# l-tamas/Fiasco

Hardware: AMD Instinct MI355X
Metric: grayscale frames/sec encoded (higher is better)
Workload: dtype f32

## Files before the change

fiasco_amd/__init__.py:

```python
import ctypes
import os
import subprocess

_HERE = os.path.dirname(os.path.abspath(__file__))
LIB_PATH = os.path.join(_HERE, "libfiasco_amd.so")
CSRC = os.path.join(_HERE, "csrc")

FIASCO_NO_VERBOSITY, FIASCO_SOME_VERBOSITY, FIASCO_ULTIMATE_VERBOSITY = 0, 1, 2
FIASCO_TILING_SPIRAL_ASC, FIASCO_TILING_SPIRAL_DSC = 0, 1
FIASCO_TILING_VARIANCE_ASC, FIASCO_TILING_VARIANCE_DSC = 2, 3
FIASCO_RPF_RANGE_0_75, FIASCO_RPF_RANGE_1_00, FIASCO_RPF_RANGE_1_50, FIASCO_RPF_RANGE_2_00 = 0, 1, 2, 3
FIASCO_PROGRESS_NONE, FIASCO_PROGRESS_BAR, FIASCO_PROGRESS_PERCENT = 0, 1, 2

EXPORTED_SYMBOLS = [
    "fiasco_get_error_message", "fiasco_set_verbosity", "fiasco_get_verbosity", "fiasco_coder",
    "fiasco_c_options_new", "fiasco_c_options_delete", "fiasco_c_options_set_smoothing",
    "fiasco_c_options_set_frame_pattern", "fiasco_c_options_set_tiling",
    "fiasco_c_options_set_basisfile", "fiasco_c_options_set_chroma_quality",
    "fiasco_c_options_set_optimizations", "fiasco_c_options_set_prediction",
    "fiasco_c_options_set_video_param", "fiasco_c_options_set_quantization",
    "fiasco_c_options_set_progress_meter", "fiasco_c_options_set_comment",
    "fiasco_c_options_set_title", "fiasco_calloc", "open_file", "fiasco_amd_set_limits",
    "fiasco_amd_get_limits", "fiasco_amd_encode_batch", "fiasco_amd_free",
    "fiasco_amd_get_stats", "fiasco_amd_reset_stats", "fiasco_amd_spec_workgroups", "fiasco_amd_core_name", "fiasco_amd_rccl_gather", "fiasco_amd_set_device",
    "fiasco_amd_batch_stage", "fiasco_amd_batch_encode", "fiasco_amd_batch_free",
    "fiasco_amd_batch_submit", "fiasco_amd_batch_collect", "fiasco_amd_batch_stats", "fiasco_amd_batch_decode_psnr", "fiasco_amd_batch_decode_psnr_all", "fiasco_amd_coop_workgroups", "fiasco_amd_share_of", "fiasco_amd_spec_append_helpers", "fiasco_amd_batch_decode_plane", "fiasco_amd_c_options_set_models",
    "fiasco_amd_release_memory", "fiasco_amd_batch_upload", "fiasco_amd_set_devices", "fiasco_amd_device_count",
    "fiasco_amd_selftest_log2", "fiasco_amd_selftest_log2_patched",
    "fiasco_amd_selftest_log2_max_ulp",
    "fiasco_amd_seq_open", "fiasco_amd_seq_free", "fiasco_amd_seq_gops", "fiasco_amd_seq_frames",
    "fiasco_amd_seq_gop_of", "fiasco_amd_seq_ycol_size", "fiasco_amd_seq_initial_level",
    "fiasco_amd_seq_search", "fiasco_amd_seq_gop_result", "fiasco_amd_seq_ycol", "fiasco_amd_seq_write",
    "fiasco_amd_seq_probe",
    "fiasco_amd_batch_stage_device", "fiasco_amd_batch_upload_device", "fiasco_amd_batch_input_planes",
    "fiasco_amd_batch_decode_device", "fiasco_amd_planes_to_pixels_device",
]

FIASCO_AMD_GRAY8, FIASCO_AMD_RGB8_INTERLEAVED, FIASCO_AMD_RGB8_PLANAR = 0, 1, 2


class DeviceFrame(ctypes.Structure):
    _fields_ = [("data", ctypes.c_void_p), ("pitch", ctypes.c_size_t), ("plane_stride", ctypes.c_size_t),
                ("width", ctypes.c_uint), ("height", ctypes.c_uint), ("layout", ctypes.c_int)]


class DeviceTarget(ctypes.Structure):
    _fields_ = [("data", ctypes.c_void_p), ("pitch", ctypes.c_size_t), ("plane_stride", ctypes.c_size_t),
                ("width", ctypes.c_uint), ("height", ctypes.c_uint), ("layout", ctypes.c_int)]


class Stats(ctypes.Structure):
    _fields_ = [("kernel_ms", ctypes.c_double), ("launches", ctypes.c_ulonglong),
                ("frames", ctypes.c_ulonglong), ("bytes_mp", ctypes.c_ulonglong),
                ("bytes_img", ctypes.c_ulonglong), ("bytes_gram", ctypes.c_ulonglong),
                ("n_mp", ctypes.c_ulonglong), ("n_steps", ctypes.c_ulonglong),
                ("n_blocks", ctypes.c_ulonglong), ("n_appends", ctypes.c_ulonglong),
                ("n_fulleval", ctypes.c_ulonglong), ("t_init", ctypes.c_ulonglong),
                ("t_approx", ctypes.c_ulonglong), ("t_ipis", ctypes.c_ulonglong),
                ("t_append", ctypes.c_ulonglong), ("t_serial", ctypes.c_ulonglong),
                ("t_total", ctypes.c_ulonglong), ("t_mpA", ctypes.c_ulonglong),
                ("t_mpB", ctypes.c_ulonglong), ("n_blockevals", ctypes.c_ulonglong),
                ("dbg", ctypes.c_ulonglong * 8), ("states_sum", ctypes.c_ulonglong),
                ("states_max", ctypes.c_ulonglong), ("reencodes", ctypes.c_ulonglong),
                ("frames_by_build", ctypes.c_ulonglong * 5),
                ("spec_frames", ctypes.c_ulonglong), ("spec_tasks", ctypes.c_ulonglong),
                ("spec_confirmed", ctypes.c_ulonglong), ("spec_wrong", ctypes.c_ulonglong),
                ("spec_timeout", ctypes.c_ulonglong), ("spec_inline", ctypes.c_ulonglong),
                ("spec_wait", ctypes.c_ulonglong), ("spec_tab_used", ctypes.c_ulonglong),
                ("spec_tab_missed", ctypes.c_ulonglong), ("spec_adopted", ctypes.c_ulonglong),
                ("decoder_frames", ctypes.c_ulonglong), ("decoder_bytes", ctypes.c_ulonglong),
                ("decoder_us", ctypes.c_ulonglong), ("coop_frames", ctypes.c_ulonglong),
                ("coop_workgroups", ctypes.c_ulonglong),
                ("spec_app_rows", ctypes.c_ulonglong), ("spec_app_wait", ctypes.c_ulonglong)]


def build(verbose=False):
    out = None if verbose else subprocess.DEVNULL
    subprocess.check_call(["make", "-C", CSRC], stdout=out)
    if not os.path.exists(LIB_PATH):
        raise RuntimeError("build did not produce %s" % LIB_PATH)


class FiascoError(RuntimeError):
    pass


class Library:

    def __init__(self, path=LIB_PATH):
        if not os.path.exists(path):
            raise FiascoError("%s is missing: run fiasco_amd.build() (there is no fallback)" % path)
        self.path = path
        L = self.L = ctypes.CDLL(path)
        c = ctypes
        L.fiasco_get_error_message.restype = c.c_char_p
        L.fiasco_set_verbosity.argtypes = [c.c_int]
        L.fiasco_get_verbosity.restype = c.c_int
        L.fiasco_c_options_new.restype = c.c_void_p
        L.fiasco_c_options_delete.argtypes = [c.c_void_p]
        L.fiasco_coder.argtypes = [c.POINTER(c.c_char_p), c.c_char_p, c.c_float, c.c_void_p]
        L.fiasco_coder.restype = c.c_int
        L.fiasco_amd_c_options_set_models.argtypes = [c.c_void_p, c.c_char_p, c.c_char_p, c.c_char_p, c.c_char_p]
        L.fiasco_amd_c_options_set_models.restype = c.c_int
        for name, args in [
            ("set_smoothing", [c.c_int]), ("set_frame_pattern", [c.c_char_p]),
            ("set_tiling", [c.c_int, c.c_uint]), ("set_basisfile", [c.c_char_p]),
            ("set_chroma_quality", [c.c_float, c.c_uint]),
            ("set_optimizations", [c.c_uint] * 5), ("set_prediction", [c.c_int, c.c_uint, c.c_uint]),
            ("set_video_param", [c.c_uint, c.c_int, c.c_int, c.c_int]),
            ("set_quantization", [c.c_uint, c.c_int, c.c_uint, c.c_int]),
            ("set_progress_meter", [c.c_int]), ("set_comment", [c.c_char_p]),
            ("set_title", [c.c_char_p]),
        ]:
            fn = getattr(L, "fiasco_c_options_" + name)
            fn.argtypes = [c.c_void_p] + args
            fn.restype = c.c_int
        L.fiasco_amd_set_limits.argtypes = [c.c_uint, c.c_uint]
        L.fiasco_amd_set_limits.restype = c.c_int
        L.fiasco_amd_get_limits.argtypes = [c.POINTER(c.c_uint), c.POINTER(c.c_uint)]
        L.fiasco_amd_encode_batch.argtypes = [c.c_uint, c.POINTER(c.c_char_p), c.POINTER(c.c_size_t),
                                              c.c_float, c.c_void_p, c.POINTER(c.c_void_p),
                                              c.POINTER(c.c_size_t)]
        L.fiasco_amd_encode_batch.restype = c.c_int
        L.fiasco_amd_free.argtypes = [c.c_void_p]
        L.fiasco_amd_core_name.restype = c.c_char_p
        if hasattr(L, "fiasco_amd_get_stats"):
            L.fiasco_amd_get_stats.argtypes = [c.POINTER(Stats)]

    def error_message(self):
        return self.L.fiasco_get_error_message().decode("latin-1")

    def core_name(self):
        return self.L.fiasco_amd_core_name().decode()

    def set_verbosity(self, level):
        self.L.fiasco_set_verbosity(level)

    def set_limits(self, max_states, max_level):
        if not self.L.fiasco_amd_set_limits(max_states, max_level):
            raise FiascoError(self.error_message())

    def get_limits(self):
        a, b = ctypes.c_uint(), ctypes.c_uint()
        self.L.fiasco_amd_get_limits(ctypes.byref(a), ctypes.byref(b))
        return a.value, b.value

    def set_devices(self, ids):
        arr = (ctypes.c_int * max(len(ids), 1))(*ids)
        self.L.fiasco_amd_set_devices.argtypes = [ctypes.POINTER(ctypes.c_int), ctypes.c_int]
        if not self.L.fiasco_amd_set_devices(arr, len(ids)):
            raise FiascoError(self.error_message())

    def device_count(self):
        return self.L.fiasco_amd_device_count()

    def set_device(self, device):
# ... 450 lines not shown
```

fiasco_amd/csrc/hip/core_hip.cpp:

```cpp
#include <hip/hip_runtime.h>
#include <stdio.h>
#include <stdlib.h>
#include <string.h>
#include <stddef.h>
#include <pthread.h>
#include <algorithm>
#include <utility>
#include <vector>
#include "fa_host.h"
#include "frame_coder.h"
#include "libfiasco_amd_hip.h"

extern "C" const char *fa_knob(const char *name)
{
    const char *d = getenv("FIASCO_AMD_DEBUG");
    return d && *d && strcmp(d, "0") != 0 ? getenv(name) : nullptr;
}
static long long knob_int(const char *name, long long d)
{
    const char *e = fa_knob(name);
    return e ? atoll(e) : d;
}


// ... 1338 lines not shown
    }
    const char *const host = pinned;
    const int16_t *tree = (const int16_t *) host;
    const int16_t *into = (const int16_t *) (host + (L.into - L.tree));
    const float *weight = (const float *) (host + (L.weight - L.tree));
    const float *fin = (const float *) (host + (L.final_d - L.tree));
    const uint8_t *los = (const uint8_t *) (host + (L.level_of_state - L.tree));
    const uint8_t *dt = (const uint8_t *) (host + (L.domain_type - L.tree));
    const uint16_t *xs = (const uint16_t *) (host + (L.x - L.tree));
    const uint16_t *ys = (const uint16_t *) (host + (L.y - L.tree));
    const uint8_t *ycol = (const uint8_t *) (host + (L.ycol - L.tree));
    const int16_t *mv = (const int16_t *) (host + (L.mv - L.tree));
    const bool inter = job->frame_type != FA_I_FRAME;
    for (unsigned s = 0; s < w->basis_states; s++) w->level_of_state[s] = 0xff;
    fa_wfa_remove_states(w, w->basis_states);
    for (unsigned s = w->basis_states; s < ns; s++) {
        w->final_distribution[s] = fin[s];
        w->domain_type[s] = dt[s];
        w->level_of_state[s] = los[s];
        w->delta_state[s] = 0;
        for (int l = 0; l < 2; l++) {
            FA_TREE(w, s, l) = tree[(size_t) l * P + s];
            w->x[s * 2 + l] = xs[(size_t) l * P + s];
            w->y[s * 2 + l] = ys[(size_t) l * P + s];
            w->y_state[s * 2 + l] = FA_RANGE;
            w->y_column[s * 2 + l] = F.color ? ycol[(size_t) l * P + s] : 0;
            w->prediction[s * 2 + l] = 0;
            if (inter) {
                fa_mv *m = &w->mv[s * 2 + l];
                m->type = mv[(size_t) (0 * 2 + l) * P + s]; m->fx = mv[(size_t) (1 * 2 + l) * P + s];
                m->fy = mv[(size_t) (2 * 2 + l) * P + s]; m->bx = mv[(size_t) (3 * 2 + l) * P + s];
                m->by = mv[(size_t) (4 * 2 + l) * P + s];
            }
            for (int e = 0; e < 6; e++) {
                FA_INTO(w, s, l, e) = into[(size_t) (l * 6 + e) * P + s];
                FA_WEIGHT(w, s, l, e) = weight[(size_t) (l * 6 + e) * P + s];
                if (FA_INTO(w, s, l, e) == FA_NO_EDGE) break;
            }
        }
    }
    if (F.color)
        for (unsigned s = 0; s < w->cap && s < (unsigned) P; s++)
            for (int l = 0; l < 2; l++) w->y_column[s * 2 + l] = ycol[(size_t) l * P + s];
    w->states = ns;
    w->root_state = (unsigned) F.root_state;
    job->stats[0].costs = F.costs; job->stats[0].err = F.err;
    job->stats[0].tree_bits = F.tree_bits; job->stats[0].matrix_bits = F.matrix_bits;
    job->stats[0].weights_bits = F.weights_bits;
    if (F.color) {
        for (int b = 0; b < 2; b++) {
            job->stats[b + 1].costs = F.c_costs[b]; job->stats[b + 1].err = F.c_err[b];
            job->stats[b + 1].tree_bits = F.c_tree_bits[b];
            job->stats[b + 1].matrix_bits = F.c_matrix_bits[b];
            job->stats[b + 1].weights_bits = F.c_weights_bits[b];
        }
        int ycb = FA_TREE(w, ns - 1, 0), crs = FA_TREE(w, ns - 1, 1);
        int roots[2] = { FA_TREE(w, ycb, 1), FA_TREE(w, crs, 0) };
        int yroot = FA_TREE(w, ycb, 0);
        std::vector<std::pair<int, int>> stack;
        for (int b = 0; b < 2; b++) {
            stack.push_back(std::make_pair(roots[b], yroot));
            while (!stack.empty()) {
                std::pair<int, int> t = stack.back();
                stack.pop_back();
                int s = t.first, y = t.second;
                if (s == FA_RANGE || (unsigned) s < w->basis_states) continue;
                for (int l = 0; l < 2; l++) {
                    int ny = y != FA_RANGE ? FA_TREE(w, y, l) : FA_RANGE;
                    w->y_state[s * 2 + l] = (int16_t) ny;
                    stack.push_back(std::make_pair((int) FA_TREE(w, s, l), ny));
                }
            }
        }
    }
    job->lc_min_level_out = (unsigned) F.lc_min_out;
    job->status = 1;
    g_stats.frames += 1;
    g_stats.bytes_mp += F.bytes_mp; g_stats.bytes_img += F.bytes_img; g_stats.bytes_gram += F.bytes_gram;
    g_stats.n_mp += F.n_mp; g_stats.n_steps += F.n_steps; g_stats.n_blocks += F.n_blocks;
    g_stats.n_appends += F.n_appends; g_stats.n_fulleval += F.n_fulleval;
    g_stats.t_init += F.t_init; g_stats.t_approx += F.t_approx; g_stats.t_ipis += F.t_ipis;
    g_stats.t_append += F.t_append; g_stats.t_serial += F.t_serial; g_stats.t_total += F.t_total;
    g_stats.t_mpA += F.t_mpA; g_stats.t_mpB += F.t_mpB; g_stats.n_blockevals += F.n_blockevals;
    for (int k = 0; k < 8; k++) g_stats.dbg[k] += F.dbg[k];
    g_stats.states_sum += ns;
    if (ns > g_stats.states_max) g_stats.states_max = ns;
    cap_hint_put(job, F.ystates_out, F.states);
    if (fa_knob("FIASCO_AMD_CAP_TRACE"))
        fprintf(stderr, "capacity: frame type %d used %d table states of %d, %d states of %d; %.3f s on the device\n", job->frame_type,
                F.ystates_out, fs.P, F.states, fs.PA, (double) F.t_total / 1e8);
    return 1;
}

static bool queue_resources(Staged *S, size_t frames)
{
    if (!grow_buffer(S->d_ring, S->ring_n, 5 * frames)) return false;
    if (!S->d_queue && hipMalloc((void **) &S->d_queue, 2 * 5 * sizeof(unsigned)) != hipSuccess) {
        S->d_queue = nullptr; (void) hipGetLastError(); return false;
    }
    if (!S->ptrmask_ready) {
        const size_t words = FC_DESC_WORDS, mwords = (words + 31) / 32;
        std::vector<unsigned> mask(mwords, 0u);
        FrameSlot a = S->slots[S->lender0], b = S->slots[S->lender0];
        const fa_job *job = &S->jobs[a.job];
        b.base = a.base + (1u << 24);
        fill_frame(a, job); fill_frame(b, job);
        const unsigned long long *wa = (const unsigned long long *) &a.F, *wb = (const unsigned long long *) &b.F;
        for (size_t w = 0; w < sizeof(DevFrame) / 8; w++)
            if (wa[w] != wb[w]) mask[w >> 5] |= 1u << (w & 31);
        const size_t wp = offsetof(DevFrame, pack_src) / 8;
        mask[wp >> 5] |= 1u << (wp & 31);
        if (!S->d_ptrmask && hipMalloc((void **) &S->d_ptrmask, mwords * sizeof(unsigned)) != hipSuccess) {
            S->d_ptrmask = nullptr; (void) hipGetLastError(); return false;
        }
        if (hipMemcpy(S->d_ptrmask, mask.data(), mwords * sizeof(unsigned), hipMemcpyHostToDevice) != hipSuccess) return false;
        S->ptrmask_ready = true;
    }
    return true;
}

struct WaveGroups { size_t n[N_BUILDS], lend[N_BUILDS], borrow[N_BUILDS]; };

static bool order_batch(Staged *S, WaveGroups &g)
{
    std::vector<size_t> &batch = S->batch;
    batch.clear();
    for (size_t k = 0; k < S->slots.size(); k++)
        if (S->slots[k].staged && !S->slots[k].done) batch.push_back(k);
    if (batch.empty()) return false;
    memset(&g, 0, sizeof g);
    const bool few = batch.size() <= (size_t) S->ncu && !fa_knob("FIASCO_AMD_NO_WIDE");
    std::vector<int> key(S->slots.size());
    for (size_t k : batch) {
        const FrameSlot &fs = S->slots[k];
        const Build b = build_of(S, fs, few);
        const int part = fs.borrow ? 1 : S->borrowers && queue_eligible(S, fs) && queue_layout(S, fs) ? 0 : 2;
        key[k] = 3 * b + part;
        g.n[b]++;
        if (part == 0) g.lend[b]++; else if (part == 1) g.borrow[b]++;
        if (k_build[b].stats_slot >= 0) g_stats.frames_by_build[k_build[b].stats_slot]++; else g_stats.spec_frames++;
    }
    std::stable_sort(batch.begin(), batch.end(), [&](size_t a, size_t b) { return key[a] < key[b]; });
    return true;
}

static void place_packs(Staged *S)
{
    const std::vector<size_t> &batch = S->batch;
    std::vector<DevFrame> &hf = S->hf;
    hf.resize(batch.size());
    S->pack_off.assign(batch.size(), 0);
    size_t need = 0;
    for (size_t b = 0; b < batch.size(); b++) {
        const FrameSlot &fs = S->slots[batch[b]];
        hf[b] = fs.F;
        hf[b].pack_src = fs.F.slab_base + fs.L.tree;
        hf[b].pack_bytes = (unsigned) (fs.L.pool_states - fs.L.tree);
        S->pack_off[b] = need;
        need += align_up(fs.L.pool_states - fs.L.tree, 256);
    }
    S->pack_need = need;
    S->parity ^= 1;
    char *&pack = S->d_pack[S->parity];
    (void) grow_buffer(pack, S->d_pack_bytes[S->parity], need);
    if (!S->cstream && hipStreamCreateWithFlags(&S->cstream, hipStreamNonBlocking) != hipSuccess) {
        S->cstream = nullptr; (void) hipGetLastError();
// ... 254 lines not shown
    if (S->packed) {
        need = S->pack_need;
        for (size_t b = 0; b < batch.size(); b++) if (hf[b].status == FC_OK) off[b] = S->pack_off[b];
    } else
        for (size_t b = 0; b < batch.size(); b++)
            if (hf[b].status == FC_OK) {
                const Layout &L = S->slots[batch[b]].L;
                off[b] = need;
                need += align_up(L.pool_states - L.tree, 256);
            }
    if (S->copy_pending) { (void) hipStreamSynchronize(S->cstream); S->copy_pending = false; }
    (void) grow_buffer(S->pinned, S->pinned_bytes, need, true);
    if (S->pinned && S->packed) {
        if (hipMemcpyAsync(S->pinned, S->d_pack[S->parity], need, hipMemcpyDeviceToHost, S->cstream) == hipSuccess)
            S->copy_pending = true;
        else {
            (void) hipGetLastError();
            off.assign(batch.size(), (size_t) -1);
        }
    } else if (S->pinned) {
        for (size_t b = 0; b < batch.size(); b++)
            if (off[b] != (size_t) -1) {
                const FrameSlot &fs = S->slots[batch[b]];
                if (hipMemcpyAsync(S->pinned + off[b], fs.base + fs.L.tree, fs.L.pool_states - fs.L.tree,
                                   hipMemcpyDeviceToHost, S->stream) != hipSuccess)
                    off[b] = (size_t) -1;
            }
        (void) hipStreamSynchronize(S->stream);
    }
    return off;
}

static void frame_outcome(Staged *S, size_t b, size_t off)
{
    FrameSlot &fs = S->slots[S->batch[b]];
    fa_job *job = &S->jobs[fs.job];
    const int st = S->hf[b].status;
    void *tr_keep = fs.F.trace;
    fs.F = S->hf[b];
    fs.F.trace = (FcTrace *) tr_keep; fs.F.trace_cap = 0;
    if (fs.ext_pix) fs.F.pix16 = fs.ext_pix;
    const size_t cap = align_up(job->cp.limit_states, 64);
    if (st == FC_ERR_CAPACITY && ((size_t) fs.P < cap || (size_t) fs.PA < cap || fs.spec)) {
        g_stats.reencodes += 1;
        size_t np = align_up((size_t) fs.P + (size_t) fs.P / 2, 64);
        size_t npa = align_up((size_t) fs.PA + (size_t) fs.PA / 2, 64);
        if ((size_t) fs.P >= cap || np >= cap) fs.spec = false;
        if (np > 3072 && S->specG > 1 && (size_t) S->specG * S->n > (size_t) S->ncu) fs.spec = false;
        if (fs.base) slab_release(fs.base, fs.bytes);
        if (fs.borrow) { fs.borrow = false; S->borrowers--; }
        fs.base = nullptr; fs.staged = false;
        fs.P = (int) (np > cap ? cap : np);
        fs.PA = (int) (npa > cap ? cap : npa);
        if (fs.PA < fs.P) fs.PA = fs.P;
        if (fs.P > 12 * 1024) fs.spec = false;
        if (!stage_slot(S, fs)) fs.done = true;
        return;
    }
    if (st == FC_ERR_COOP && fs.spec && !S->no_app) {
        S->no_app = true;
        return;
    }
    if (st == FC_ERR_COOP && !S->no_coop_done) {
        S->no_coop = true;
        return;
    }
    if (st == FC_ERR_QUEUE && fs.borrow) {
        fs.borrow = false; S->borrowers--;
        fs.base = nullptr; fs.staged = false;
        if (!stage_slot(S, fs)) fs.done = true;
        return;
    }
    fs.done = true;
    if (st == FC_OK) {
        if (S->pinned && off != (size_t) -1) S->to_unpack.push_back(std::make_pair(S->batch[b], off));
        else S->good += collect(S, fs, nullptr);
        return;
    }
    const char *msg = "device coder failed";
    if (st == FC_ERR_STATES || st == FC_ERR_CAPACITY) msg = "Maximum number of states reached!";
    else if (st == FC_ERR_NOROOT) msg = "No root state generated!";
    else if (st == FC_ERR_QUEUE) msg = "device coder: frame queue gave no slab";
    else if (st == FC_ERR_COOP) msg = "device coder: the helper workgroups of the frame did not answer";
    else if (st == FC_ERR_INTERNAL) msg = "device coder: frame exceeds a built-in capacity (recursion depth, snapshot stack or 16384 states)";
    if (st > FC_ERR_QUEUE) snprintf(job->errmsg, sizeof job->errmsg, "%s (status %d)", msg, st);
    else snprintf(job->errmsg, sizeof job->errmsg, "%s", msg);
}

static void complete_wave(Staged *S)
{
    if (!download_wave(S)) {
        const char *why = hipGetErrorString(hipGetLastError());
        for (size_t b = 0; b < S->batch.size(); b++) {
            FrameSlot &fs = S->slots[S->batch[b]];
            snprintf(S->jobs[fs.job].errmsg, sizeof S->jobs[fs.job].errmsg, "HIP error: %s", why);
            fs.done = true;
        }
        S->broken = true;
        return;
    }
    const std::vector<size_t> off = fetch_automata(S);
    for (size_t b = 0; b < S->batch.size(); b++) frame_outcome(S, b, off[b]);
    (void) hipStreamSynchronize(S->stream);
}

static void flush_unpack(Staged *S)
{
    if (S->copy_pending) { (void) hipStreamSynchronize(S->cstream); S->copy_pending = false; }
    for (size_t i = 0; i < S->to_unpack.size(); i++)
        S->good += collect(S, S->slots[S->to_unpack[i].first], S->pinned + S->to_unpack[i].second);
    S->to_unpack.clear();
}

static int core1_submit(void *h)
{
    Staged *S = (Staged *) h;
    if (!S || !S->ok) return 0;
    if (S->inflight) return 1;
    for (size_t k = 0; k < S->slots.size(); k++) {
        S->slots[k].done = false;
        S->slots[k].src = S->jobs[S->slots[k].job].image;
    }
    S->good = 0; S->broken = false;
    if (S->up_pending) {
        (void) hipStreamWaitEvent(S->stream, S->ev_up, 0);
        for (size_t k = 0; k < S->slots.size(); k++) {
            FrameSlot &fs = S->slots[k];
            if (fs.ext_next) { fs.ext_pix = fs.ext_next; fs.F.pix16 = fs.ext_pix; }
        }
        S->up_parity ^= 1;
        S->up_pending = false;
    }
    S->inflight = launch_wave(S);
    return 1;
}

static int core1_finish2(void *h, int resubmit)
{
    Staged *S = (Staged *) h;
    if (!S || !S->ok) return 0;
    if (!S->inflight) { core1_submit(h); }
    for (size_t k = 0; k < S->slots.size(); k++) S->jobs[S->slots[k].job].status = 0;
    for (;;) {
        if (S->inflight) { complete_wave(S); S->inflight = false; if (S->broken) break; }
        {
            bool more = false;
            for (size_t k = 0; k < S->slots.size(); k++) if (!S->slots[k].done) more = true;
            if (more) flush_unpack(S);
        }
        if (launch_wave(S)) { S->inflight = true; continue; }
        bool any = false, pending = false;
        for (size_t k = 0; k < S->slots.size(); k++) {
            FrameSlot &fs = S->slots[k];
            if (!fs.staged && !fs.done && !S->jobs[fs.job].errmsg[0]) pending = true;
        }
        if (!pending) break;
        for (size_t k = 0; k < S->slots.size(); k++) {
            FrameSlot &fs = S->slots[k];
            if (fs.done && fs.base) { slab_release(fs.base, fs.bytes); fs.base = nullptr; fs.staged = false; }
        }
        for (size_t k = 0; k < S->slots.size(); k++) {
            FrameSlot &fs = S->slots[k];
            if (fs.staged || fs.done || S->jobs[fs.job].errmsg[0]) continue;
            if (stage_slot(S, fs)) any = true; else if (!fs.rejected) break;
        }
        if (!any) break;
// ... 511 lines not shown
```

fiasco_amd/csrc/hip/fc_config.inc:

```

#ifndef FC_VARIANT_WIDE
#define FC_VARIANT_WIDE 0
#endif
#if FC_VARIANT_WIDE
#ifndef FC_WIDE_B
#define FC_WIDE_B 512
#endif
#define B       FC_WIDE_B
#if defined(FC_VARIANT_BIG) && FC_VARIANT_BIG
#define FC_KREG 12
#elif !defined(FC_KREG)
#define FC_KREG (9216 / FC_WIDE_B)
#endif
#else
#define B       FC_BLOCK
#define FC_KREG 12
#endif
#ifndef FC_VARIANT_BIG
#define FC_VARIANT_BIG 0
#endif
#if FC_HM && !(FC_VARIANT_BIG && FC_VARIANT_WIDE)
#error "FC_HM is a variant of the 512-thread big build"
#endif
#if FC_GM && !FC_HM
#error "FC_GM is a variant of the FC_HM build"
#endif
#if FC_VARIANT_BIG
#if FC_GM
#define FC_KERNEL    fiasco_frame_kernel_big_gm
#define FC_LAUNCH    fc_launch_big_gm
#define FC_OCCUPANCY fc_occupancy_big_gm
#elif FC_HM
#define FC_KERNEL    fiasco_frame_kernel_big_hm
#define FC_LAUNCH    fc_launch_big_hm
#define FC_OCCUPANCY fc_occupancy_big_hm
#elif FC_VARIANT_WIDE
#define FC_KERNEL    fiasco_frame_kernel_big_wide
#define FC_LAUNCH    fc_launch_big_wide
#define FC_OCCUPANCY fc_occupancy_big_wide
#else
#define FC_KERNEL    fiasco_frame_kernel_big
#define FC_LAUNCH    fc_launch_big
#define FC_OCCUPANCY fc_occupancy_big
#endif
#define FC_PIXELS    4096
#define FC_NIP       4
#define FC_CLMAX     2048
#define FC_WG_PER_CU (FC_VARIANT_WIDE ? 1 : 2)
#else
#if FC_VARIANT_WIDE
#if defined(FC_SPEC) && FC_SPEC
#define FC_KERNEL    fiasco_frame_kernel_spec_wide
#define FC_LAUNCH    fc_launch_spec_wide
#define FC_OCCUPANCY fc_occupancy_spec_wide
#define FC_SPEC_SLOT_BYTES fc_spec_slot_bytes_wide
#elif defined(FC_GRAM_TRI) && FC_GRAM_TRI
#define FC_KERNEL    fiasco_frame_kernel_wide_tri
#define FC_LAUNCH    fc_launch_wide_tri
#define FC_OCCUPANCY fc_occupancy_wide_tri
#else
#define FC_KERNEL    fiasco_frame_kernel_wide
#define FC_LAUNCH    fc_launch_wide
#define FC_OCCUPANCY fc_occupancy_wide
#endif
#elif defined(FC_SPEC) && FC_SPEC
#define FC_KERNEL    fiasco_frame_kernel_spec
#define FC_LAUNCH    fc_launch_spec
#define FC_OCCUPANCY fc_occupancy_spec
#define FC_SPEC_SLOT_BYTES fc_spec_slot_bytes
#else
#define FC_KERNEL    fiasco_frame_kernel
#define FC_LAUNCH    fc_launch
#define FC_OCCUPANCY fc_occupancy
#endif
#define FC_PIXELS    1024
#define FC_NIP       2
#define FC_CLMAX     768
#ifndef FC_WG_PER_CU
#define FC_WG_PER_CU (FC_VARIANT_WIDE ? 1 : 4)
#endif
#endif
#ifndef FC_SPEC
#define FC_SPEC 0
#endif
#define SPEC_THR 1.2f
#define FC_D5T (!FC_VARIANT_BIG)
#if FC_D5T
#define D5_AT(P, NA, a, s) ((unsigned) (s) * (unsigned) (NA) + (unsigned) ((a) & 1) * ((unsigned) (NA) >> 1) + ((unsigned) (a) >> 1))
#else
#define D5_AT(P, NA, a, s) ((unsigned) (a) * (unsigned) (P) + (unsigned) (s))
#endif
#define FC_PRIO_ROTATE (!FC_VARIANT_BIG && !FC_VARIANT_WIDE && !FC_SPEC)
#define FC_PRIO_SHIFT 20
#define MAXED   FC_MAXED
#define FC_MAXE (FC_NIP + 1)
#define NOEDGE  (-1)
#define RANGE_  (-1)
#define MAXCOSTS 1e20f
#define BIGF    3.0e38f
#define MIN_NORM 2e-3f

enum { OP_DONE = 0, OP_INIT_RANGE, OP_APPROX, OP_IPIS_INCR, OP_APPEND, OP_NOP, OP_CHROMA,
       OP_PRED_SETUP, OP_PRED_FINISH, OP_NORMS, OP_MC_SEARCH, OP_SPEC_CKPT };
enum { PH_ENTER = 0, PH_AFTER_INIT, PH_AFTER_LC, PH_CHILD, PH_CHILD2, PH_CHILD_RET, PH_DECIDE,
       PH_AFTER_APPEND, PH_PRED_BEGIN, PH_PRED_RECURSE, PH_PRED_RET, PH_PRED_DONE, PH_PRED_MC2, PH_PRED_GO,
       PH_SPEC_END };
enum { MV_NONE = 0, MV_FORWARD = 1, MV_BACKWARD = 2, MV_INTERPOLATED = 3 };
#ifdef FC_DUP_OP
#define FC_DUP(o, call) do { if ((o) == FC_DUP_OP) { __syncthreads(); call; } } while (0)
#else
#define FC_DUP(o, call) do { } while (0)
#endif
#if FC_VARIANT_BIG
#define FC_DEPTH FC_MAXDEPTH_BIG
#elif FC_VARIANT_WIDE
#define FC_DEPTH FC_MAXDEPTH
#else
#define FC_DEPTH FC_MAXDEPTH_NARROW
#endif
```

fiasco_amd/csrc/hip/fc_lds.inc:

```

#define RANGE_E (FC_MAXE + 1)
struct __attribute__((aligned(16))) Range {
    int   x, y, image, address, level, tree;
    float weight[RANGE_E];
    short into[RANGE_E];
    float err, tree_bits, matrix_bits, weights_bits;
#if FC_VARIANT_BIG
    float nd_tree_bits, nd_weights_bits, mv_tree_bits, mv_coord_bits;
    int   prediction;
    short mv[5];
#endif
};

struct Pool {
    short count[MAXED + 1];
    unsigned short total, n, max_domains, y_index;
    short d0_index;
    unsigned short d0_yindex, d0_n;
};

struct __attribute__((aligned(16))) SFrame {
    Range rg, lrange, rrange, child[2];
    Pool  pool0, pool_lc;
    float max_costs, lincomb, subdiv, ret, price;
// ... 19 lines not shown
    short indices[MAXED + 1], into[MAXED + 1];
    float weight[MAXED];
    unsigned symp;
    float matrix_bits, weights_bits, err, costs, min_costs;
    float sel_ipdo[MAXED][MAXED];
    float norm_ov[MAXED + 1], ipio[MAXED + 1];
    short psorted[MAXED + 1];
    int   np;
    float wb_dc, wb_nd, norm, ab, price;
    int   y_state, ypos;
#if FC_VARIANT_BIG
    const float *numrow;
    short excl[MAXED + 1];
#endif
#if FC_GM
    short kq[MAXED + 1];
#endif
    float s1_pre[MAXED], s1_sfx[MAXED], s1_z0, s1_zy;
    int   s1_last[MAXED], s1_k[MAXED], s1_thr[MAXED];
    unsigned s1_cd, s1_has;
};

struct __attribute__((aligned(16))) CoeffBuf {
    short tot[16];
    short cnt[FC_VARIANT_BIG ? FC_MAXCOEFF_BIG : FC_MAXCOEFF];
};
#if FC_VARIANT_BIG
#define SNAP_POOL16 880
#define SNAP_TM_WORDS 2392
#else
#define SNAP_POOL16 (FC_VARIANT_WIDE ? FC_SNAP16_WIDE : FC_SNAP16_NARROW)
#define SNAP_TM_WORDS (FC_VARIANT_WIDE ? FC_SNAPTM_WIDE : FC_SNAPTM_NARROW)
#endif
#if FC_VARIANT_BIG || FC_VARIANT_WIDE
#define NBLOCKMIN   256
#else
#define NBLOCKMIN   64
#endif
#define TM_WORDS    (4 * 26 + 8)

struct RoundBox {
    float m2[2];
    int   state;
    int   idx;
    float cost, mbits, wbits, err, f[MAXED];
    float num, den, ip[MAXED - 1];
    unsigned evals, blockevals;
    unsigned symp;
};
#define SYMP_NONE 0u
#define SYMP_HAS(p, k) ((k) < 3 && (((p) >> (10 * (k))) & 1023u) != 0u)
#define SYMP_GET(p, k) ((int) (((p) >> (10 * (k))) & 1023u) - 2)
#define SYMP_PUT(sym, k) ((unsigned) ((sym) + 2) << (10 * (k)))

struct Sh {
    RoundBox rb;
    SFrame   st[FC_DEPTH];
    int      sp;
    int      op, a0, a1, a2, a3;
#if FC_VARIANT_BIG
    unsigned coopW, coop_seq;
    int      coopD, coop_minsub;
    unsigned long long coop_ticks;
#endif
    Pool     pool;
    CoeffBuf cb;
#if FC_VARIANT_BIG
    Pool     dpool;
    CoeffBuf dcb;
    struct { int rpf_mant, dc_mant, sy, dcs; float rpf_range, dc_range; int half_nd, half_dc; } dq;
    int      nslot;
    uint4   *snap_tm_p;
    int      pred_active, pred_lo, pred_rec;
    struct { int type, fx, fy, bx, by; float bits, tree_bits; } mc;
    unsigned long long mcred[B / 64];
    unsigned pred_saved[FC_MAXSAVE / 32];
#endif
    uint4    snap_pool[SNAP_POOL16];
    uint4   *snap;
    int      n16;
    __attribute__((aligned(16))) unsigned tm[TM_WORDS];
    __attribute__((aligned(16))) unsigned snap_tm[SNAP_TM_WORDS];
    float    m0tab[12];
    double   lgdc[FC_MAXSYM], lglv[FC_MAXSYM], lglv_m1;
    float    Ltab[MAXED + 1];
    float    Q0, Q1;
    float    tb[2];
    MPState  mp;
#if FC_VARIANT_BIG
    MPState  mp_keep;
    int      apx_stage, apx_it, apx_more;
#endif
    float    blockmin[NBLOCKMIN];
    __attribute__((aligned(16))) float pixels[FC_PIXELS];
    float    norms[FC_PIXELS / 32];
    unsigned long long tk[16];
    struct {
        unsigned long long bytes_mp, bytes_img, bytes_gram, n_mp, n_steps, n_blocks, n_appends,
                           n_fulleval, n_blockevals, t_mpA, t_mpB;
    } cnt;
#ifdef FC_SERIAL_PROFILE
    unsigned long long tk_ph[8], ph_t0, tk_init[2], tk_apx[4];
    int      ph_prev;
#endif
    int      band, lc_min, tree_band[3], ystates, after_chroma;
    short    dl[64];
#if !FC_SPEC
    short    cl[FC_CLMAX];
    int      cln;
#endif
    unsigned long long red[B / 64];
    int      gs_idx[2][MAXED + 1], gs_n[2], gs_c[2], gs_raw_idx[2][MAXED + 1];
    float    gs_raw_w[2][MAXED + 1];
    float    gs_w[2][MAXED + 1];
    struct {
        int lc_max, width, height, limit_states, PA, P, ML; float price, chroma_decrease;
        float *gram, *diag, *ipis; int16_t *pos; unsigned gram_ls;
        float *gcol;
        float *d5, *d4;
        const unsigned *l2_keys; const double *l2_vals; unsigned l2_mask;
        int max_elements, rpf_mant, dc_mant, sy, dcs, gl0, images_level, lc_min_opt, trace_on;
        int snap_b1;
        int16_t *at_tree, *at_into, *at_pool; float *at_weight, *at_final; uint8_t *at_los, *at_dtype, *at_ycol;
        uint16_t *at_x, *at_y; int color;
        float rpf_range, dc_range;
        int half_nd, half_dc;
    } par;
#if FC_GM
    struct { int pk[2], ck[2], qa; float base, kept; double lg1; int16_t *gq; int P; } gm;
#endif
    int      states;
    int      flim;
    int      failed;
#if FC_SPEC
    int      gap_lo, gap_hi, gap_shift;
    unsigned deadmask;
    int      cap;
    int      blk;
    int      tab_shared;
    int      tab_from;
    struct SpecLocal {
        FcSpecCtl *ctl;
        char     *slots;
        int       role, on;
        int       mode;
        int       T;
        int       chroma_tabs;
        char     *tabs;
        unsigned  rb_s[32];
        unsigned  blkof[FC_SPEC_W];
        unsigned  sk[FC_SPEC_W];
        unsigned long long n_tab_used, n_tab_missed, n_adopted;
        int       floor;
        unsigned  head, commit;
        unsigned  spec_mask;
        int       nospec;
        unsigned  epoch;
        int       verdict, abort, busy;
        unsigned  ops;
        float     mlc, lin[FC_SPEC_W];
        unsigned  nlc;
        float     learn;
        unsigned long long n_tasks, n_confirmed, n_wrong, n_timeout, n_inline, t_wait;
        unsigned  app_H, app_min, app_seq, app_off;
        unsigned long long n_app_dealt, t_app_wait;
    } sl;
#endif
};
#if FC_GM
#define GM_QAC(k)   ((k) == FC_PK_ADAPTIVE || (k) == FC_PK_BASIS)
#define GM_RLE(k)   ((k) == FC_PK_RLE || (k) == FC_PK_RLE_NO_CHROMA)
#define GQ_CUR(sh, set)          ((sh).gm.gq + (size_t) ((sh).gm.qa ^ (set)) * (sh).gm.P)
#define GQ_SNAP(sh, depth, slot) ((sh).gm.gq + (size_t) (2 + (depth) * 5 + (slot)) * (sh).gm.P)
#endif
#if FC_SPEC
#define DEAD(sh, s) ((unsigned) ((int) (s) - (sh).gap_lo) < (unsigned) ((sh).gap_hi - (sh).gap_lo))
#else
#define DEAD(sh, s) false
#endif
```

fiasco_amd/csrc/hip/fc_serial.inc:

```


__device__ float tree_bits_dev(const Sh &sh, int ML, int child, int level, int which)
{
    const unsigned *counts = sh.tm + which * 2 * ML;
    float prob = counts[level] / (float) counts[ML + level];
    return child ? (float) -log2((double) prob) : (float) -log2((double) (1 - prob));
}

__device__ void tree_update_dev(Sh &sh, int ML, int child, int level, int which)
{
    unsigned *counts = sh.tm + which * 2 * ML;
    if (child) counts[level]++;
    counts[ML + level]++;
}

__device__ __forceinline__ void copy16(uint4 *dst, const uint4 *src, int n)
{
    int i = 0;
    for (; i + 8 <= n; i += 8) {
        uint4 t0 = src[i], t1 = src[i + 1], t2 = src[i + 2], t3 = src[i + 3];
        uint4 t4 = src[i + 4], t5 = src[i + 5], t6 = src[i + 6], t7 = src[i + 7];
        dst[i] = t0; dst[i + 1] = t1; dst[i + 2] = t2; dst[i + 3] = t3;
        dst[i + 4] = t4; dst[i + 5] = t5; dst[i + 6] = t6; dst[i + 7] = t7;
    }
// ... 405 lines not shown
                snap_save(F, sh, sp, 0);
                tm_save(sh, sp, ML);
#if FC_GM
                fr.rn0 = sh.dpool.n;
                gq_save(sh, 0, sp, 0);
#endif
#if FC_VARIANT_BIG
                if (sh.nslot == 5 && !fr.delta) {
                    fr.dpool0 = sh.dpool; snap_save_d(sh, sp, 2);
#if FC_GM
                    gq_save(sh, 1, sp, 2);
#endif
                }
#endif
            }
            fr.states = sh.states;
            for (int l = 0; l < 2; l++)
                fr.ny[l] = (sh.band && fr.y_state != RANGE_) ? (int) TREE(F, fr.y_state, l) : RANGE_;
            phase = PH_AFTER_LC;
            if (rg.level <= sh.par.lc_max) {
                fr.lrange = rg;
                fr.lrange.tree = RANGE_;
#if FC_VARIANT_BIG
                fr.lrange.tree_bits = tree_bits_dev(sh, ML, 0, rg.level, 0);
#endif
                fr.lrange.matrix_bits = 0;
                fr.lrange.weights_bits = 0;
#if FC_VARIANT_BIG
                fr.lrange.nd_tree_bits = 0; fr.lrange.nd_weights_bits = 0; fr.lrange.prediction = 0;
                fr.lrange.mv_tree_bits = fr.try_pred == 2 ? 1.0f : 0.0f;
                fr.lrange.mv_coord_bits = 0;
#endif
                sh.op = OP_APPROX;
                return 0;
            }
            fr.lincomb = MAXCOSTS;
            break;
        }
        case PH_AFTER_LC: {
            Range &rg = fr.rg;
            if (fr.leaf) {
                fr.subdiv = MAXCOSTS;
                phase = PH_DECIDE;
                break;
            }
            if (!fr.coop) {
#if FC_VARIANT_BIG
                fr.pool_lc = sh.pool;
                snap_save(F, sh, sp, 1);
#if FC_GM
                gq_save(sh, 0, sp, 1);
#endif
                sh.pool = fr.pool0;
                snap_load(F, sh, sp, 0);
#if FC_GM
                gq_load(sh, 0, sp, 0);
                if (fr.delta) sh.dpool.n = (unsigned short) fr.rn0;
#endif
#else
                fr.pool_lc = sh.pool;
#endif
            }
#if FC_SPEC
            if (fr.ckpt == 3) {
                fr.subdiv = MAXCOSTS;
                phase = PH_DECIDE;
                break;
            }
#endif
            if (rg.level > sh.lc_min) {
                Range z;
                z.x = z.y = z.image = z.address = z.level = 0; z.tree = 0;
                for (int i = 0; i < RANGE_E; i++) { z.weight[i] = 0; z.into[i] = 0; }
                z.err = z.tree_bits = z.matrix_bits = z.weights_bits = 0;
#if FC_VARIANT_BIG
                z.nd_tree_bits = z.nd_weights_bits = z.mv_tree_bits = z.mv_coord_bits = 0; z.prediction = 0;
                for (int i = 0; i < 5; i++) z.mv[i] = 0;
#endif
                fr.child[0] = z; fr.child[1] = z;
                fr.rrange = rg;
#if FC_VARIANT_BIG
                fr.rrange.tree_bits = tree_bits_dev(sh, ML, 1, rg.level, 0);
#else
                fr.rrange.tree_bits = rg.level <= sh.par.lc_max ? sh.tb[1] : tree_bits_dev(sh, ML, 1, rg.level, 0);
#endif
                fr.rrange.matrix_bits = 0;
                fr.rrange.weights_bits = 0;
                fr.rrange.err = 0;
#if FC_VARIANT_BIG
                fr.rrange.mv_tree_bits = fr.try_pred == 2 ? 1.0f : 0.0f;
                fr.rrange.mv_coord_bits = 0;
                fr.rrange.nd_tree_bits = fr.try_pred == 1 ? tree_bits_dev(sh, ML, 1, rg.level, 1) : 0.0f;
                fr.rrange.nd_weights_bits = 0;
                fr.rrange.prediction = 0;
                fr.subdiv = (fr.rrange.tree_bits + fr.rrange.weights_bits + fr.rrange.matrix_bits
                             + fr.rrange.mv_tree_bits + fr.rrange.mv_coord_bits + fr.rrange.nd_tree_bits
                             + fr.rrange.nd_weights_bits) * fr.price;
#else
                fr.subdiv = (fr.rrange.tree_bits + fr.rrange.weights_bits + fr.rrange.matrix_bits) * fr.price;
#endif
                fr.label = 0;
                phase = PH_CHILD;
            } else {
                fr.subdiv = MAXCOSTS;
                phase = PH_DECIDE;
            }
            break;
        }
        case PH_CHILD: {
            const Range &rr = fr.rrange;
            const int label = fr.label;
            Range &ch = fr.child[label];
            ch.image = rr.image * 2 + label + 1;
            ch.address = rr.address * 2 + label;
            ch.level = rr.level - 1;
            ch.x = (rr.level & 1) ? rr.x : rr.x + label * (int) width_of_level(rr.level - 1);
            ch.y = (rr.level & 1) ? rr.y + label * (int) height_of_level(rr.level - 1) : rr.y;
            phase = PH_CHILD2;
            if (label && rr.level <= sh.par.lc_max && sh.states > fr.states && !sh.band) {
                sh.op = OP_IPIS_INCR; sh.a0 = ch.image; sh.a1 = ch.address; sh.a2 = ch.level;
                sh.a3 = fr.states;
                return 0;
            }
            break;
        }
        case PH_CHILD2: {
            float lim = fr.lincomb > fr.max_costs ? fr.max_costs : fr.lincomb;
            float remaining = lim - fr.subdiv;
            phase = PH_CHILD_RET;
            fr.ret = 0;
            if (remaining > 0) {
                if (sp + 1 >= FC_DEPTH) { sh.failed = FC_ERR_INTERNAL; break; }
                SFrame &cf = sh.st[sp + 1];
                cf.rg = fr.child[fr.label];
                cf.y_state = fr.ny[fr.label];
                cf.max_costs = remaining;
                cf.phase = PH_ENTER;
#if FC_SPEC
                cf.ckpt = 0;
#endif
#if FC_VARIANT_BIG
                cf.pred = fr.pred; cf.delta = fr.delta;
#endif
                fr.phase = phase; sp++; phase = PH_ENTER;
                break;
            }
            fr.ret = -1;
            break;
        }
        case PH_CHILD_RET: {
            const int label = fr.label;
            float lim = fr.lincomb > fr.max_costs ? fr.max_costs : fr.lincomb;
#if FC_VARIANT_BIG
            if (fr.try_pred == 2 && !fr.norm_done) {
                const Range &c0 = fr.child[label];
                sh.op = OP_NORMS; sh.a0 = fr.rg.level; sh.a1 = fr.norm_first;
                sh.a2 = (fr.ret < 0 && c0.level >= F.p_min) ? c0.level : -1;
                sh.a3 = c0.x | (c0.y << 16);
                fr.norm_first = 0; fr.norm_done = 1;
                return 0;
            }
            fr.norm_done = 0;
#endif
            if (fr.ret >= 0) fr.subdiv += fr.ret;
            if (fr.subdiv >= lim) {
                fr.subdiv = MAXCOSTS;
                phase = PH_DECIDE;
// ... 295 lines not shown
```

fiasco_amd/csrc/hip/frame_coder.h:

```cpp
#ifndef FRAME_CODER_H
#define FRAME_CODER_H
#include <stdint.h>

#define FC_MAXED    5
#define FC_BLOCK    256
#define FC_MAXDEPTH 22
#define FC_MAXDEPTH_BIG 32
#define FC_MAXDEPTH_NARROW 18
#define FC_SNAP16_NARROW 480
#define FC_SNAP16_WIDE   840
#define FC_SNAPTM_NARROW 988
#define FC_SNAPTM_WIDE   1092
#define FC_MAXSAVE  512
#define FC_MAXCOEFF 224
#ifndef FC_HM
#define FC_HM 0
#endif
#ifndef FC_GM
#define FC_GM 0
#endif
enum { FC_PK_ADAPTIVE = 0, FC_PK_CONSTANT = 1, FC_PK_BASIS = 2, FC_PK_UNIFORM = 3, FC_PK_RLE = 4, FC_PK_RLE_NO_CHROMA = 5 };
enum { FC_CK_ADAPTIVE = 0, FC_CK_UNIFORM = 1 };
#define FC_GQ_SLOTS (2 + FC_MAXDEPTH_BIG * 5)
#define FC_MAXCOEFF_BIG_STD 640
#define FC_MAXSYM_STD   64
#define FC_MAXCOEFF_HM  5120
#define FC_MAXSYM_HM    512
#define FC_MAXCOEFF_BIG (FC_HM ? FC_MAXCOEFF_HM : FC_MAXCOEFF_BIG_STD)
#define FC_MAXSYM       (FC_HM ? FC_MAXSYM_HM : FC_MAXSYM_STD)
#define FC_N16(coeffs)  ((32 + 2 * (coeffs) + 15) / 16)
#define FC_N16MAX       FC_N16(FC_MAXCOEFF_BIG)
#define FC_MAXBASIS 16
#define FC_BX_BYTES (64 * 1024)
#ifndef FC_TRI_HOT
#define FC_TRI_HOT  8
#endif

enum { FC_OK = 1, FC_ERR_STATES = 2, FC_ERR_CAPACITY = 3, FC_ERR_NOROOT = 4, FC_ERR_INTERNAL = 5,
       FC_ERR_QUEUE = 6,
       FC_ERR_COOP = 7 };
struct FcCoop {
    unsigned seq;
    unsigned done;
    unsigned quit;
    unsigned depth;
    int      level, from, to;
    int      minsub;
    float   *ipis, *d5, *d4;
    unsigned long long done_ticks;
};
#define FC_COOP_HDR 128
#define FC_COOP_WAIT_TICKS 3000000000ull
#define FC_COOP_DONE_TICKS 500000000ull
#define FC_QUEUE_WAIT_TICKS 60000000000ull

struct FcTrace;
typedef struct DevFrame {
    float    price;
    int      lc_min, lc_max, images_level, max_elements;
    int      maxe_live;
    int      gl0;
    int      second_domain_block;
    int      check_underflow, check_overflow, full_search;
    int      level, width, height;
    int      pool_max, limit_states, ML;
    int      rpf_mant, dc_mant;
    float    rpf_range, dc_range;
    int      P;
    unsigned gram_ls;
    int      PA;
    int      color;
    int      chroma_sparse;
    int      chroma_cl_cap;
    int      chroma_max;
    float    chroma_decrease;
    unsigned long long plane;
    int      NL, NS, NA, NI;
    int      coeff_size, coeff_nt, dcs, sy;
    int      basis_states;
    int16_t  b_tree[FC_MAXBASIS][2];
    int16_t  b_into[FC_MAXBASIS][2][6];
    float    b_weight[FC_MAXBASIS][2][6];
    float    b_final[FC_MAXBASIS];
    uint8_t  b_dtype[FC_MAXBASIS];
    const int *bx;
    int      gm_pool[2], gm_coeff[2];
    int16_t *gq;
    const double *lginv;
    const int16_t *pix16;
    float   *gram, *diag, *ipis, *d5, *img, *imgT, *norms;
    float   *gcol;
    float   *d4, *imgT4;
    float   *num, *den, *est, *ipdo;
    uint8_t *used;
    int16_t *tree, *into;
    float   *weight, *final_d;
    uint8_t *level_of_state, *domain_type;
    uint16_t *x, *y;
    uint8_t *ycol;
    const uint8_t *ycol0;
    void    *snap_hbm;
    int      pred_root;
    int      pred_on;
    int      frame_type;
    int      p_min, p_max;
    int      d_rpf_mant, d_dc_mant;
    float    d_rpf_range, d_dc_range;
    int      d_coeff_size, d_dcs, d_sy;
    float   *ipis_alt, *d5_alt, *d4_alt;
    float   *pix_save;
    float   *sv_gram;
    float   *sv_img;
    struct FcSavedRow *sv_auto;
    int      max_save;
    const int16_t *past, *future;
    float   *mc_fwd, *mc_bwd;
    int16_t *mv;
    int16_t *pix_chroma;
    int      search_range;
    int16_t *pool_states;
    int16_t *pos;
    int     *hits;
    const void *pack_src;
    void    *pack_dst;
    unsigned pack_bytes;
    const unsigned *l2_keys;
    const double   *l2_vals;
    unsigned        l2_mask;
    int      status;
    int      states, root_state;
    FcCoop  *coop;
    int      ystates_out;
    float    costs, err, tree_bits, matrix_bits, weights_bits;
    float    c_costs[2], c_err[2], c_tree_bits[2], c_matrix_bits[2], c_weights_bits[2];
    int      lc_min_out;
    unsigned long long bytes_mp, bytes_img, bytes_gram;
    unsigned long long n_mp, n_steps, n_blocks, n_appends, n_fulleval;
    unsigned long long t_init, t_approx, t_ipis, t_append, t_serial, t_total;
    unsigned long long t_mpA, t_mpB, n_blockevals;
    unsigned long long dbg[8];
    struct FcTrace *trace;
    int      trace_cap, trace_n;
    char    *slab_base;
    unsigned long long slab_bytes;
    struct FcSpecCtl *spec;
    int      spec_role, spec_G;
    int      spec_tb;
    int      spec_cap;
    int      spec_T;
} DevFrame;

#define FC_DESC_WORDS ((sizeof(DevFrame) + 7) / 8)

#define FC_SPEC_W      16
#define FC_SPEC_TEMPS  16
#define FC_SPEC_MAXG   8
#define FC_SPEC_R      24
typedef struct FcSpecCtl {
    unsigned next;
    unsigned epoch;
    unsigned done;
    unsigned committed;
    unsigned adopting;
    unsigned busy;
    unsigned slot_bytes;
    unsigned slot_seq[FC_SPEC_W];
    unsigned verdict[FC_SPEC_W];
    unsigned long long n_tasks, n_confirmed, n_wrong, n_timeout, n_inline, t_wait;
    unsigned long long n_tab_used, n_tab_missed;
    unsigned long long n_adopted;
    unsigned s_pub;
    unsigned tab_free;
    unsigned blk_cur;
    unsigned chroma_ready, tab_next, ystates;
    unsigned n_tabs;
    unsigned n_blocks;
    unsigned tab_stride;
    unsigned tab_wait;
    unsigned long long off_blocks, off_tabs;
    unsigned tab_seq[FC_SPEC_R];
    unsigned tab_s[FC_SPEC_R];
    unsigned tab_epoch[FC_SPEC_R];
    unsigned app_H;
    unsigned app_min;
    unsigned app_wait;
    unsigned app_seq;
    unsigned app_done;
    unsigned app_off;
    unsigned app_dbg;
    int      app_s, app_flim;
    int      app_n[2], app_c[2], app_idx[2][FC_MAXED + 1];
    float    app_w[2][FC_MAXED + 1];
    unsigned long long n_app_dealt, t_app_wait;
} FcSpecCtl;

typedef struct FcSavedRow {
    int16_t  tree[2], into[2][6];
    float    weight[2][6];
    float    final_d;
    uint16_t x[2], y[2];
    int16_t  pos;
    int16_t  mv[2][5];
    uint8_t  level, dtype, ycol[2], tables;
} FcSavedRow;

typedef struct FcTrace {
    int   seq, level, image, D, states, nedges;
    float cost, err, mbits, wbits;
    short into[6];
    float w[5];
} FcTrace;

#endif
```

fiasco_amd/csrc/hip/frame_coder.hip:

```cpp
#include <hip/hip_runtime.h>
#include <stdint.h>
#include <math.h>
#include "frame_coder.h"

#include "fc_config.inc"
#include "fc_lds.inc"
#include "fc_access.inc"
#include "fc_tables.inc"
#include "fc_append.inc"
#include "fc_predict.inc"
#include "fc_models.inc"
#include "mp_device.inc"
#include "fc_serial.inc"
#include "fc_spec.inc"

__device__ void basis_init(DevFrame &F, Sh &sh)
{
    const int nb = F.basis_states, il = F.images_level;
    for (int s = 0; s < nb; s++) {
        F.img[(size_t) s * F.NI] = F.final_d[s];
        if (il == 0) F.imgT[s] = F.final_d[s];
    }
    for (int l = 1; l <= il; l++)
        for (int s = 0; s < nb; s++)
            for (int i = 0; i < (1 << l); i++) {
                float v = image_elem(F, s, l, i);
                F.img[(size_t) s * F.NI + (1 << l) - 1 + i] = v;
                if (l == il) F.imgT[(size_t) i * F.P + s] = v;
#if FC_VARIANT_BIG
                if (l == il - 1 && F.gl0 < il) F.imgT4[(size_t) i * F.P + s] = v;
#endif
            }
    for (int q = 0; q < F.NL; q++)
        for (int s1 = 0; s1 < nb; s1++)
            for (int s2 = 0; s2 <= s1; s2++) {
                if (!F.domain_type[s2]) continue;
#if FC_VARIANT_BIG
                if (F.gl0 < il) {
                    gram_store(F, q, s1, s2, q == 0 ? gram_dot4(F, s1, s2) : q == 1 ? gram_dot(F, s1, s2)
                                                                   : gram_entry(F, q, s1, s2));
                    continue;
                }
#endif
                gram_store(F, q, s1, s2, q == 0 ? gram_dot(F, s1, s2) : gram_entry(F, q, s1, s2));
            }
    sh.states = nb;
}

#if FC_VARIANT_BIG
__device__ void basis_init_bx(DevFrame &F, Sh &sh)
{
    const int tid = threadIdx.x, il = F.images_level;
    const BxView V = bx_view(F);
    const int nb = V.nb;
    for (int s = tid; s < nb; s += B) {
        F.img[(size_t) s * F.NI] = F.final_d[s];
        if (il == 0) F.imgT[s] = F.final_d[s];
    }
    __syncthreads();
    for (int l = 1; l <= il; l++) {
        for (int k = tid; k < (nb << l); k += B) {
            const int s = k >> l, i = k & ((1 << l) - 1);
            const float v = image_elem_bx(F, V, s, l, i);
            F.img[(size_t) s * F.NI + (1 << l) - 1 + i] = v;
            if (l == il) F.imgT[(size_t) i * F.P + s] = v;
            if (l == il - 1 && F.gl0 < il) F.imgT4[(size_t) i * F.P + s] = v;
        }
        __syncthreads();
    }
    for (int q = 0; q < F.NL; q++) {
        for (int k = tid; k < nb * nb; k += B) {
            const int s1 = k / nb, s2 = k - s1 * nb;
            if (s2 > s1 || !F.domain_type[s2]) continue;
            float v;
            if (F.gl0 < il) v = q == 0 ? gram_dot4(F, s1, s2) : q == 1 ? gram_dot(F, s1, s2) : gram_entry_bx(F, V, q, s1, s2);
            else v = q == 0 ? gram_dot(F, s1, s2) : gram_entry_bx(F, V, q, s1, s2);
            gram_store(F, q, s1, s2, v);
        }
        __syncthreads();
    }
}
#endif

#if FC_SPEC
#define SPEC_STRIDE ((unsigned) ((sizeof(Sh) + 255) / 256 * 256))
#define SPEC_SLOTS(ctl) ((char *) (ctl) + (sizeof(FcSpecCtl) + 255) / 256 * 256)
#endif

__global__ void __launch_bounds__(B, FC_WG_PER_CU)
#if FC_SPEC
FC_KERNEL(DevFrame *frames, DevFrame *vframes, unsigned G, unsigned n, unsigned H)
#else
FC_KERNEL(DevFrame *frames, unsigned nlend, unsigned long long *ring, unsigned *ctr, const unsigned *ptrmask,
          unsigned long long queue_wait_ticks, unsigned coopW)
#endif
{
#if FC_SPEC
    constexpr unsigned FC_LDS_EXTRA = sizeof(Sh::SpecLocal) + 64;
#else
    constexpr unsigned FC_LDS_EXTRA = 64;
#endif
    static_assert(sizeof(Sh) + FC_LDS_EXTRA <= (160u * 1024u) / FC_WG_PER_CU, "Sh outgrows the LDS share of a workgroup of this build");
    __shared__ Sh sh;
#if FC_SPEC
    __shared__ Sh::SpecLocal sl_keep;
    __shared__ unsigned task_seq, spec_slot, spec_used, spec_vid;
    __shared__ int task_go, spec_act, spec_bad;
    if (threadIdx.x == 0) spec_bad = 0;
    if (blockIdx.x >= n * G) {
        const unsigned k = blockIdx.x - n * G;
        spec_append_helper(frames[k / H], sh, k % H, H);
        return;
    }
    const unsigned role = blockIdx.x % G;
    DevFrame &F = role ? vframes[(blockIdx.x / G) * (G - 1) + role - 1] : frames[blockIdx.x / G];
    unsigned long long *const ring = nullptr;
#elif FC_VARIANT_BIG
    const unsigned cW = coopW > 1 ? coopW : 1;
    unsigned fidx = blockIdx.x, member = 0;
    if (cW > 1) {
        fidx = (blockIdx.x / (8 * cW)) * 8 + blockIdx.x % 8;
        member = (blockIdx.x / 8) % cW;
        if (fidx >= nlend) return;
    }
    DevFrame &F = frames[fidx];
    if (member) { coop_helper(F, sh, member, cW); return; }
    if (threadIdx.x == 0) {
        sh.coopW = F.coop ? cW : 1; sh.coop_seq = 0;
        sh.coopD = cW > 1 && F.coop ? (int) F.coop->depth : 0; sh.coop_minsub = cW > 1 && F.coop ? F.coop->minsub : 0;
        sh.coop_ticks = cW > 1 && F.coop ? F.coop->done_ticks : 0;
    }
#else
    DevFrame &F = frames[blockIdx.x];
#endif
    const int tid = threadIdx.x;

#if !FC_SPEC
    if (ring && blockIdx.x >= nlend) {
        __shared__ unsigned long long got;
        if (tid == 0) {
            const unsigned t = atomicAdd(&ctr[0], 1u);
            unsigned long long b;
            const unsigned long long t_give_up = wall_clock64() + queue_wait_ticks;
            while ((b = __hip_atomic_load(&ring[t], __ATOMIC_ACQUIRE, __HIP_MEMORY_SCOPE_AGENT)) == 0) {
                if (wall_clock64() > t_give_up) break;
                __builtin_amdgcn_s_sleep(32);
            }
            got = b;
        }
        __syncthreads();
        if (got == 0) {
            if (tid == 0) { F.status = FC_ERR_QUEUE; F.states = 0; }
            return;
        }
        {
            unsigned long long *d = (unsigned long long *) &F;
            const unsigned long long lo = (unsigned long long) F.slab_base, span = F.slab_bytes;
            const unsigned long long delta = got - lo;
            unsigned long long v[(FC_DESC_WORDS + B - 1) / B];
#pragma unroll
            for (unsigned k = 0; k < (FC_DESC_WORDS + B - 1) / B; k++) {
                const unsigned w = k * B + tid;
                v[k] = w < FC_DESC_WORDS ? d[w] : 0;
            }
            __syncthreads();
#pragma unroll
            for (unsigned k = 0; k < (FC_DESC_WORDS + B - 1) / B; k++) {
                const unsigned w = k * B + tid;
                if (w < FC_DESC_WORDS && ((ptrmask[w >> 5] >> (w & 31)) & 1u) && v[k] - lo < span) d[w] = v[k] + delta;
            }
        }
        __threadfence();
        __syncthreads();
        __builtin_amdgcn_s_dcache_inv();
    }
#endif

#if FC_SPEC
    if (tid == 0) {
        Sh::SpecLocal &sl = sh.sl;
        sh.gap_lo = sh.gap_hi = 0; sh.gap_shift = 0; sh.deadmask = 0;
        sh.cap = F.spec ? F.spec_cap : F.P;
        sl.ctl = F.spec; sl.slots = F.spec ? SPEC_SLOTS(F.spec) : nullptr;
        sl.role = (int) role; sl.on = F.spec != nullptr && G > 1;
        sl.mode = role == 0 && sl.on ? 1 : 0;
        sl.T = F.spec_T; sl.tabs = F.spec ? (char *) F.spec + F.spec->off_tabs : nullptr;
        sl.chroma_tabs = 0;
        sl.n_tab_used = sl.n_tab_missed = sl.n_adopted = 0;
        sl.app_H = role == 0 && F.spec && G > 1 ? F.spec->app_H : 0u; sl.app_min = F.spec ? F.spec->app_min : 0u;
        sl.app_seq = 0; sl.app_off = 0; sl.n_app_dealt = sl.t_app_wait = 0;
        for (int k = 0; k < 32; k++) sl.rb_s[k] = 0;
        sh.blk = 0; sh.tab_shared = 0; sh.tab_from = 0;
        sl.floor = 0; sl.head = sl.commit = 0; sl.spec_mask = 0; sl.nospec = 0; sl.epoch = 0;
        sl.verdict = 0; sl.abort = 0; sl.ops = 0; sl.mlc = 0.0f; sl.nlc = 0; sl.learn = 0.0f;
        sl.n_tasks = sl.n_confirmed = sl.n_wrong = sl.n_timeout = sl.n_inline = sl.t_wait = 0;
        sl_keep = sl;
    }
    if (role == 0) {
#endif
    if (tid < 10 && tid >= 1)
        sh.m0tab[tid] = (float) -log2((double) (1 - 1 / (float) (1 << tid)));
    if (tid == 0) {
        const int ML = F.ML;
        static const unsigned c0[22] = {20,17,15,10,5,4,3,2,1,1,1,1,1,1,1,1,1,1,1,1,1,1};
        static const unsigned c1[22] = {1,1,1,1,1,1,1,1,1,2,3,5,10,15,20,25,30,35,60,60,60,60};
        sh.failed = 0;
        sh.cnt.bytes_mp = sh.cnt.bytes_img = sh.cnt.bytes_gram = 0;
        sh.cnt.n_mp = sh.cnt.n_steps = sh.cnt.n_blocks = sh.cnt.n_appends = sh.cnt.n_fulleval = 0;
        sh.cnt.t_mpA = sh.cnt.t_mpB = sh.cnt.n_blockevals = 0;
        F.trace_n = 0;
        for (int k = 0; k < 8; k++) F.dbg[k] = 0;
#ifdef FC_LATENCY_PROBE
        {
            volatile float *a = F.est;
            for (int k = 0; k < 64; k++) a[k] = (float) ((k * 7 + 3) & 63);
            __builtin_amdgcn_s_waitcnt(0);
            unsigned long long c0 = __builtin_readcyclecounter();
            int idx = 0;
            for (int k = 0; k < 64; k++) idx = (int) a[idx];
            unsigned long long c1 = __builtin_readcyclecounter();
            F.dbg[5] = (c1 - c0) / 64 + (idx & 0);
            c0 = __builtin_readcyclecounter();
            for (int k = 0; k < 64; k++) { a[64] = (float) k; idx += (int) a[64]; }
            c1 = __builtin_readcyclecounter();
            F.dbg[6] = (c1 - c0) / 64 + (idx & 0);
        }
#endif
#if FC_VARIANT_BIG
        if (F.bx) {
            const BxView V = bx_view(F);
            for (int s = 0; s < V.nb; s++) {
                F.final_d[s] = V.final_d[s];
                F.domain_type[s] = (uint8_t) V.dtype[s];
                F.level_of_state[s] = 0xff;
                for (int l = 0; l < 2; l++) { TREE(F, s, l) = RANGE_; INTO(F, s, l, 0) = NOEDGE; }
            }
        } else
#endif
        for (int s = 0; s < F.basis_states; s++) {
            F.final_d[s] = F.b_final[s];
            F.domain_type[s] = F.b_dtype[s];
            F.level_of_state[s] = 0xff;
            for (int l = 0; l < 2; l++) {
                TREE(F, s, l) = F.b_tree[s][l];
                for (int e = 0; e < 6; e++) {
                    INTO(F, s, l, e) = F.b_into[s][l][e];
                    WEIGHT(F, s, l, e) = F.b_weight[s][l][e];
                    if (F.b_into[s][l][e] == NOEDGE) break;
                }
            }
        }
        for (int w = 0; w < 2; w++)
            for (int l = 0; l < ML; l++) {
                int k = l < 22 ? l : 21;
                sh.tm[w * 2 * ML + l] = c1[k];
                sh.tm[w * 2 * ML + ML + l] = c0[k] + c1[k];
            }
        for (int i = 4 * ML; i < TM_WORDS; i++) sh.tm[i] = 0;
        Pool &m = sh.pool;
        m.total = 0;
        for (int i = 0; i <= MAXED; i++) { m.count[i] = 1; m.total++; }
        m.n = 0; m.max_domains = (unsigned short) F.pool_max; m.y_index = 0;
        m.d0_index = 0; m.d0_yindex = 0; m.d0_n = 0;
#if FC_GM
        sh.gm.pk[0] = F.gm_pool[0]; sh.gm.pk[1] = F.pred_on ? F.gm_pool[1] : FC_PK_CONSTANT;
        sh.gm.ck[0] = F.gm_coeff[0]; sh.gm.ck[1] = F.gm_coeff[1];
        sh.gm.qa = 0; sh.gm.gq = F.gq; sh.gm.P = F.P;
        sh.gm.base = sh.gm.kept = 0.0f; sh.gm.lg1 = 0.0;
        sh.dpool = m;
        for (int set = 0; set < 2; set++) {
            Pool &pm = set ? sh.dpool : sh.pool;
            const int k = sh.gm.pk[set];
            int maxd = F.pool_max ? F.pool_max : 1;
            if (k == FC_PK_BASIS) maxd = F.basis_states;
            if (k == FC_PK_UNIFORM || k == FC_PK_CONSTANT) maxd = 0xffff;
            pm.max_domains = (unsigned short) maxd;
            if (!GM_RLE(k)) { pm.total = 0; for (int i = 0; i <= MAXED; i++) pm.count[i] = 0; }
        }
        for (int s = 0; s < F.basis_states; s++) {
            F.pos[s] = -1;
            if (F.domain_type[s] & 2) gm_offer(F, sh, s);
        }
        if ((F.domain_type[0] & 2) && F.pos[0] < 0) { F.pos[0] = 0; F.pool_states[0] = 0; }
        if (sh.gm.pk[0] == FC_PK_CONSTANT) sh.pool.n = 1;
        if (sh.gm.pk[1] == FC_PK_CONSTANT) sh.dpool.n = 0;
#else
        for (int s = 0; s < F.basis_states; s++) {
            F.pos[s] = -1;
            if ((F.domain_type[s] & 2) && m.n < m.max_domains) {
                F.pos[s] = (short) m.n;
                F.pool_states[m.n++] = (short) s;
                if (s == 0) m.d0_n = 1;
            }
        }
#endif
        sh.n16 = (32 + 2 * F.coeff_size + 15) / 16;
#if FC_VARIANT_BIG
        if (F.pred_on && (32 + 2 * F.d_coeff_size + 15) / 16 > sh.n16) sh.n16 = (32 + 2 * F.d_coeff_size + 15) / 16;
        sh.nslot = F.pred_on ? 5 : 2;
        sh.snap = (F.pred_on || (F.level - F.lc_min + 3) * 2 * sh.n16 > SNAP_POOL16) && F.snap_hbm
                  ? (uint4 *) F.snap_hbm : sh.snap_pool;
        sh.snap_tm_p = F.pred_on && F.snap_hbm ? (uint4 *) F.snap_hbm + FC_DEPTH * 5 * FC_N16MAX : (uint4 *) sh.snap_tm;
        sh.pred_active = 0; sh.pred_lo = sh.pred_rec = 0;
#endif
        {
            const int depth_need = F.level - F.lc_min + 2
#if FC_VARIANT_BIG
                                   + (F.pred_on ? F.p_max - F.lc_min + 2 : 0)
#endif
                                   ;
#if FC_VARIANT_BIG
            const bool snap_lds = sh.snap == &sh.snap_pool[0];
            const bool tm_lds = (const void *) sh.snap_tm_p == (const void *) &sh.snap_tm[0];
#else
            const bool snap_lds = true, tm_lds = true;
#endif
#if FC_VARIANT_BIG
            const int snap_need = (F.level - F.lc_min + 3) * 2 * sh.n16;
#else
            const int snap_need = (F.level - F.lc_min + 3 + F.lc_max - F.lc_min) * sh.n16;
            sh.par.snap_b1 = (F.level - F.lc_min + 3) - (F.level - F.lc_max);
#endif
            if ((snap_lds && snap_need > SNAP_POOL16)
                || (tm_lds && (F.level - F.lc_min + 3) * 4 * TM_N16(ML) > SNAP_TM_WORDS) || F.coeff_nt > 16
                || (F.P + 63) / 64 > NBLOCKMIN
                || depth_need > FC_DEPTH
                || F.max_elements > FC_MAXE
                || (!FC_VARIANT_BIG && F.pred_on))
                sh.failed = FC_ERR_INTERNAL;
        }
        for (int i = 0; i < (FC_VARIANT_BIG ? FC_MAXCOEFF_BIG : FC_MAXCOEFF); i++) sh.cb.cnt[i] = 0;
        for (int i = 0; i < 16; i++) sh.cb.tot[i] = 0;
        for (int i = 0; i < F.coeff_size; i++) sh.cb.cnt[i] = 1;
        sh.cb.tot[0] = (short) F.dcs;
        for (int i = 1; i < F.coeff_nt; i++) sh.cb.tot[i] = (short) F.sy;
#if FC_VARIANT_BIG
        for (int i = 0; i < FC_MAXCOEFF_BIG; i++) sh.dcb.cnt[i] = 0;
        for (int i = 0; i < 16; i++) sh.dcb.tot[i] = 0;
        for (int i = 0; i < F.d_coeff_size; i++) sh.dcb.cnt[i] = 1;
        sh.dcb.tot[0] = (short) F.d_dcs;
        for (int i = 1; i < F.coeff_nt; i++) sh.dcb.tot[i] = (short) F.d_sy;
#if !FC_GM
        sh.dpool = sh.pool;
#endif
        sh.dq.rpf_mant = F.d_rpf_mant; sh.dq.dc_mant = F.d_dc_mant; sh.dq.sy = F.d_sy; sh.dq.dcs = F.d_dcs;
        sh.dq.rpf_range = F.d_rpf_range; sh.dq.dc_range = F.d_dc_range;
        sh.dq.half_nd = rtob_dev(0.5f, F.d_rpf_mant, F.d_rpf_range); sh.dq.half_dc = rtob_dev(0.5f, F.d_dc_mant, F.d_dc_range);
        if (F.pred_on && F.d_coeff_size > FC_MAXCOEFF_BIG) sh.failed = FC_ERR_INTERNAL;
#endif
#if FC_VARIANT_BIG
        if (F.bx) sh.states = F.basis_states;
        else
#else
        if (F.bx) sh.failed = FC_ERR_INTERNAL;
#endif
        basis_init(F, sh);
        sh.flim = 0;
        sh.par.lc_max = F.lc_max; sh.par.width = F.width; sh.par.height = F.height;
        sh.par.limit_states = F.limit_states; sh.par.PA = F.PA; sh.par.P = F.P; sh.par.ML = F.ML;
        sh.par.price = F.price; sh.par.chroma_decrease = F.chroma_decrease;
        sh.par.gram = F.gram; sh.par.gram_ls = F.gram_ls; sh.par.diag = F.diag; sh.par.ipis = F.ipis; sh.par.pos = F.pos;
        sh.par.gcol = F.gcol;
        sh.par.d5 = F.d5; sh.par.d4 = F.d4;
        sh.par.at_tree = F.tree; sh.par.at_into = F.into; sh.par.at_pool = F.pool_states; sh.par.at_weight = F.weight;
        sh.par.at_final = F.final_d; sh.par.at_los = F.level_of_state; sh.par.at_dtype = F.domain_type;
        sh.par.at_ycol = F.ycol; sh.par.at_x = F.x; sh.par.at_y = F.y; sh.par.color = F.color;
        sh.par.l2_keys = F.l2_keys; sh.par.l2_vals = F.l2_vals; sh.par.l2_mask = F.l2_mask;
        sh.par.max_elements = F.max_elements; sh.par.rpf_mant = F.rpf_mant; sh.par.dc_mant = F.dc_mant;
        sh.par.sy = F.sy; sh.par.dcs = F.dcs; sh.par.gl0 = F.gl0; sh.par.images_level = F.images_level;
        sh.par.lc_min_opt = F.lc_min; sh.par.trace_on = F.trace != nullptr;
        sh.par.rpf_range = F.rpf_range; sh.par.dc_range = F.dc_range;
        sh.par.half_nd = rtob_dev(0.5f, F.rpf_mant, F.rpf_range); sh.par.half_dc = rtob_dev(0.5f, F.dc_mant, F.dc_range);
        sh.band = 0; sh.lc_min = F.lc_min; sh.after_chroma = 0; sh.ystates = 0;
        push_root(F, sh, RANGE_);
        sh.op = OP_NOP;
    }
    if (F.color)
        for (int i = tid; i < 2 * F.PA; i += B) F.ycol[i] = F.ycol0 ? F.ycol0[i] : (uint8_t) 0;
#if FC_VARIANT_BIG
    if (F.bx) { __syncthreads(); basis_init_bx(F, sh); }
#endif
#if FC_SPEC
    }
#endif
    unsigned long long *tk = sh.tk;
    if (tid == 0) for (int k = 0; k < 16; k++) tk[k] = 0;
#ifdef FC_SERIAL_PROFILE
    if (tid == 0) { for (int k = 0; k < 8; k++) sh.tk_ph[k] = 0; sh.ph_prev = 0; sh.ph_t0 = 0; sh.tk_init[0] = sh.tk_init[1] = 0; for (int k = 0; k < 4; k++) sh.tk_apx[k] = 0; }
#endif
    unsigned long long t_begin = wall_clock64();
#if FC_SPEC
    const unsigned T = F.spec ? (unsigned) F.spec_T : 0u;
    if (role == 0 && F.spec && G > 1) {
        __threadfence();
        __syncthreads();
        if (tid == 0) __hip_atomic_store(&F.spec->s_pub, (unsigned) sh.states, __ATOMIC_RELEASE, __HIP_MEMORY_SCOPE_AGENT);
    }
    if (role >= 1 && role <= T) { spec_worker(F, sh, role, T, false); return; }
    for (;;) {
    if (role) {
        FcSpecCtl *const c = F.spec;
        __syncthreads();
        if (tid == 0) {
            unsigned t = atomicAdd(&c->next, 1u);
            int go = 1;
            for (;;) {
                const unsigned q = __hip_atomic_load(&c->slot_seq[t % FC_SPEC_W], __ATOMIC_RELAXED, __HIP_MEMORY_SCOPE_AGENT);
                if (q == t + 1) { take_acquire(); break; }
                if (q > t + 1) { t = atomicAdd(&c->next, 1u); continue; }
                if (__hip_atomic_load(&c->done, __ATOMIC_RELAXED, __HIP_MEMORY_SCOPE_AGENT)) { go = 0; break; }
                if (__hip_atomic_load(&c->chroma_ready, __ATOMIC_RELAXED, __HIP_MEMORY_SCOPE_AGENT)) { take_acquire(); go = 2; break; }
                __builtin_amdgcn_s_sleep(32);
            }
            task_seq = t; task_go = go;
        }
        __syncthreads();
        if (task_go != 1) break;
        {
            const uint4 *src = (const uint4 *) (SPEC_SLOTS(c) + (size_t) (task_seq % FC_SPEC_W) * SPEC_STRIDE);
            for (unsigned i = tid; i < sizeof(Sh) / 16; i += B) ((uint4 *) &sh)[i] = src[i];
        }
        __syncthreads();
        if (tid == 0) {
            const unsigned task_epoch = sh.sl.epoch;
            bool valid = __hip_atomic_load(&c->slot_seq[task_seq % FC_SPEC_W], __ATOMIC_ACQUIRE, __HIP_MEMORY_SCOPE_AGENT) == task_seq + 1
                         && __hip_atomic_load(&c->epoch, __ATOMIC_ACQUIRE, __HIP_MEMORY_SCOPE_AGENT) == task_epoch;
            sh.sl = sl_keep;
            sh.sl.epoch = task_epoch;
            const int S0 = sh.states, TB = F.spec_tb;
            if (valid && (S0 > TB || sh.sp < 0 || sh.sp >= FC_DEPTH)) valid = false;
            sh.sl.floor = sh.sp; sh.sl.verdict = 2; sh.sl.abort = valid ? 0 : 1; sh.sl.ops = 0; sh.sl.busy = 0;
            sh.sl.mode = 2 + sh.sp;
            if (sh.sp > 0) sh.st[sh.sp - 1].phase = PH_SPEC_END;
            sh.gap_lo = S0; sh.gap_hi = TB; sh.gap_shift = TB - S0; sh.states = TB; sh.cap = TB + FC_SPEC_TEMPS;
            unsigned dm = 0;
            for (int k = 0; k < 32; k++) if (k * B >= S0 && (k + 1) * B <= TB) dm |= 1u << k;
            sh.deadmask = dm;
            sh.par.at_pool = F.pool_states;
            sh.par.trace_on = 0;
            sh.par.color = 0;
            for (int k = 0; k < FC_SPEC_TEMPS; k++) F.level_of_state[TB + k] = 0;
            sh.op = valid ? OP_NOP : OP_DONE;
            if (valid) {
                atomicAdd(&c->busy, 1u);
                SPEC_DEKKER_FENCE();
                if (__hip_atomic_load(&c->epoch, __ATOMIC_ACQUIRE, __HIP_MEMORY_SCOPE_AGENT) != task_epoch) {
                    atomicSub(&c->busy, 1u); valid = false; sh.sl.abort = 1; sh.op = OP_DONE;
                } else sh.sl.busy = 1;
            }
            if (valid && !sh.tab_shared) {
                const Range &rg = sh.st[sh.sp].rg;
                sh.par.ipis = F.ipis; sh.par.d5 = F.d5;
                sh.op = OP_INIT_RANGE; sh.a0 = rg.x; sh.a1 = rg.y; sh.a2 = -1;
            }
        }
    }
#endif
    for (;;) {
        __syncthreads();
        const int op = sh.op;
        if (op == OP_DONE) break;
        unsigned long long t0 = wall_clock64();
#if FC_PRIO_ROTATE
        {
            const unsigned pr = ((unsigned) (t0 >> FC_PRIO_SHIFT) + (blockIdx.x >> 8)) & 3u;
            if (pr == 0) __builtin_amdgcn_s_setprio(0);
            else if (pr == 1) __builtin_amdgcn_s_setprio(1);
            else if (pr == 2) __builtin_amdgcn_s_setprio(2);
            else __builtin_amdgcn_s_setprio(3);
        }
#endif
        switch (op) {
#if FC_SPEC
        case OP_SPEC_CKPT: {
            FcSpecCtl *const c = sh.sl.ctl;
            if (tid == 0) {
                int act = 0;
                const int back = spec_poll(sh, sh.a0 == 2);
                if (back) {
                    act = (back & 0x100) ? 3 : 2; spec_slot = (unsigned) ((back & 0xff) - 1);
                    spec_used = (unsigned) (back >> 16) & 63u; spec_vid = (unsigned) (back >> 24) & 7u;
                    if (act == 3) {
                        __builtin_amdgcn_fence(__ATOMIC_ACQUIRE, "agent");
                        const Sh *im = (const Sh *) (sh.sl.slots + (size_t) (FC_SPEC_W + spec_vid) * SPEC_STRIDE);
                        const int TB = im->gap_hi, S0 = im->gap_lo, m = im->states - TB;
                        int bad = 0;
                        if (S0 != (int) sh.sl.sk[spec_slot]) bad |= 1;
                        if (TB < F.spec_cap || TB + FC_SPEC_TEMPS > F.P || ((TB - F.spec_cap) % FC_SPEC_TEMPS)) bad |= 2;
                        if (m < 0 || m > FC_SPEC_TEMPS || m > (int) spec_used) bad |= 4;
                        if (im->sp < 1 || im->sp >= FC_DEPTH) bad |= 8;
                        if (im->sl.epoch != sh.sl.epoch) bad |= 16;
                        if (S0 + m > F.spec_cap) bad |= 32;
                        if (im->sl.verdict != 3 || im->failed) bad |= 64;
                        if (bad) { spec_bad |= bad; act = 2; }
                    }
                }
                else if (sh.a0 == 1) {
                    SFrame &fr = sh.st[sh.sp];
                    if (!sh.sl.nospec && fr.rg.level > sh.lc_min) { fr.ckpt = 2; act = 1; }
                } else if (sh.par.color && !sh.band && !sh.after_chroma) spec_luminance_done(sh);
                else { sh.sl.on = 0; sh.sl.mode = 0; }
                spec_act = act;
            }
            __syncthreads();
            if (spec_act == 1) {
                const unsigned seq = sh.sl.head, slot = seq % FC_SPEC_W;
                if (tid == 0) __hip_atomic_store(&c->slot_seq[slot], 0u, __ATOMIC_RELAXED, __HIP_MEMORY_SCOPE_AGENT);
                WAVE_DRAIN();
                __syncthreads();
                uint4 *dst = (uint4 *) (sh.sl.slots + (size_t) slot * SPEC_STRIDE);
                for (unsigned i = tid; i < sizeof(Sh) / 16; i += B) dst[i] = ((const uint4 *) &sh)[i];
                WAVE_DRAIN();
                __syncthreads();
                if (tid == 0) {
                    publish_release();
                    __hip_atomic_store(&c->s_pub, (unsigned) sh.states, __ATOMIC_RELAXED, __HIP_MEMORY_SCOPE_AGENT);
                    __hip_atomic_store(&c->slot_seq[slot], seq + 1, __ATOMIC_RELAXED, __HIP_MEMORY_SCOPE_AGENT);
                    sh.sl.head = seq + 1; sh.sl.spec_mask &= ~(1u << slot); sh.sl.n_tasks++;
                    sh.sl.blkof[slot] = (unsigned) (sh.blk - 1);
                    sh.sl.sk[slot] = (unsigned) sh.states;
                }
            } else if (spec_act == 3) {
                if (tid == 0) sl_keep = sh.sl;
                __builtin_amdgcn_fence(__ATOMIC_ACQUIRE, "agent");
                __syncthreads();
                const uint4 *src = (const uint4 *) (sl_keep.slots + (size_t) (FC_SPEC_W + spec_vid) * SPEC_STRIDE);
                for (unsigned i = tid; i < sizeof(Sh) / 16; i += B) ((uint4 *) &sh)[i] = src[i];
                __syncthreads();
                const int TB = sh.gap_hi, S0 = sh.gap_lo, m = sh.states - TB, shift = TB - S0;
                __syncthreads();
                if (tid == 0) {
                    sh.sl = sl_keep;
                    sh.sl.nospec = 0;
                    sh.sl.commit = sh.sl.head;
                    sh.sl.rb_s[sh.sl.epoch % 32u] = (unsigned) S0;
                    __hip_atomic_store(&c->s_pub, (unsigned) S0, __ATOMIC_RELEASE, __HIP_MEMORY_SCOPE_AGENT);
                    __hip_atomic_store(&c->adopting, 1u, __ATOMIC_RELEASE, __HIP_MEMORY_SCOPE_AGENT);
                    sh.sl.epoch++;
                    __hip_atomic_store(&c->epoch, sh.sl.epoch, __ATOMIC_RELEASE, __HIP_MEMORY_SCOPE_AGENT);
                    SPEC_DEKKER_FENCE();
                    while (__hip_atomic_load(&c->busy, __ATOMIC_ACQUIRE, __HIP_MEMORY_SCOPE_AGENT)) __builtin_amdgcn_s_sleep(8);
                    sh.sl.n_adopted++;
                    sh.gap_lo = sh.gap_hi = sh.gap_shift = 0; sh.deadmask = 0;
                    sh.cap = F.spec_cap;
                    sh.states = S0 + m;
                    sh.par.at_pool = F.pool_states; sh.par.color = F.color; sh.par.trace_on = 0;
                    if (!sh.tab_shared) { sh.par.ipis = F.ipis; sh.par.d5 = F.d5; }
                    sh.st[sh.sp - 1].phase = PH_CHILD_RET;
                    SFrame &fr = sh.st[sh.sp];
                    fr.states = S0;
                    for (int l = 0; l < 2; l++) {
                        Range &ch = fr.child[l];
                        if (ch.tree >= TB) ch.tree -= shift;
                        for (int e = 0; e < RANGE_E; e++) if (ch.into[e] >= TB) ch.into[e] = (short) (ch.into[e] - shift);
                    }
                    if (F.color) {
                        GLOBAL_AS uint8_t *yc = (GLOBAL_AS uint8_t *) F.ycol;
                        for (unsigned j = 0; j < spec_used; j++) { yc[S0 + j] = 0; yc[(unsigned) F.PA + S0 + j] = 0; }
                    }
                }
                __syncthreads();
                __builtin_amdgcn_fence(__ATOMIC_ACQUIRE, "agent");
                for (int j = 0; j < m; j++) {
                    const int sid = TB + j, did = S0 + j;
                    if (tid < 2) {
                        const int l = tid;
                        const int t = TREE(F, sid, l);
                        TREE(F, did, l) = (short) (t >= TB ? t - shift : t);
                        for (int e = 0; e < 6; e++) {
                            const int d = INTO(F, sid, l, e);
                            INTO(F, did, l, e) = (short) (d >= TB ? d - shift : d);
                            WEIGHT(F, did, l, e) = WEIGHT(F, sid, l, e);
                        }
                        F.x[l * F.PA + did] = F.x[l * F.PA + sid]; F.y[l * F.PA + did] = F.y[l * F.PA + sid];
                    } else if (tid == 2) {
                        F.final_d[did] = F.final_d[sid]; F.level_of_state[did] = F.level_of_state[sid];
                        F.domain_type[did] = F.domain_type[sid];
                        const short p = F.pos[sid];
                        F.pos[did] = p;
                        if (p >= 0) F.pool_states[p] = (short) did;
                    }
                    if (!F.domain_type[sid]) continue;
                    for (int i = tid; i < F.NI; i += B) F.img[(size_t) did * F.NI + i] = F.img[(size_t) sid * F.NI + i];
                    if (tid < 32) F.imgT[(size_t) tid * F.P + did] = F.imgT[(size_t) tid * F.P + sid];
                    for (int q = 0; q < F.NL; q++) {
                        const float *Gs = GRAM(F, q) + GROW(sid, F.P);
                        float *Gd = GRAM(F, q) + GROW(did, F.P);
                        for (int t = tid; t < S0; t += B) Gd[t] = Gs[t];
                        if (tid <= j) Gd[S0 + tid] = Gs[TB + tid];
                        if (tid == 0) F.diag[(size_t) q * F.P + did] = F.diag[(size_t) q * F.P + sid];
                    }
                }
                __threadfence();
                __syncthreads();
                if (tid == 0)
                    __hip_atomic_store(&c->adopting, 0u, __ATOMIC_RELEASE, __HIP_MEMORY_SCOPE_AGENT);
            } else if (spec_act == 2) {
                const unsigned slot = spec_slot;
                if (tid == 0) sl_keep = sh.sl;
                __builtin_amdgcn_fence(__ATOMIC_ACQUIRE, "agent");
                __syncthreads();
                const uint4 *src = (const uint4 *) (sl_keep.slots + (size_t) slot * SPEC_STRIDE);
                for (unsigned i = tid; i < sizeof(Sh) / 16; i += B) ((uint4 *) &sh)[i] = src[i];
                __syncthreads();
                if (tid == 0) {
                    sh.sl = sl_keep;
                    sh.sl.nospec = 1;
                    sh.sl.commit = sh.sl.head;
                    sh.sl.rb_s[sh.sl.epoch % 32u] = (unsigned) sh.states;
                    __hip_atomic_store(&c->s_pub, (unsigned) sh.states, __ATOMIC_RELEASE, __HIP_MEMORY_SCOPE_AGENT);
                    sh.sl.epoch++;
                    __hip_atomic_store(&c->epoch, sh.sl.epoch, __ATOMIC_RELEASE, __HIP_MEMORY_SCOPE_AGENT);
                    SPEC_DEKKER_FENCE();
                    while (__hip_atomic_load(&c->busy, __ATOMIC_ACQUIRE, __HIP_MEMORY_SCOPE_AGENT)) __builtin_amdgcn_s_sleep(8);
                }
                __syncthreads();
                if (!sh.tab_shared) op_init_range(F, sh, sh.st[sh.sp].rg.x, sh.st[sh.sp].rg.y, 0);
                if (tid == 0 && sh.sl.n_timeout >= 3) { sh.sl.on = 0; sh.sl.mode = 0; }
            }
            break;
        }
#endif
#if FC_SPEC
        case OP_INIT_RANGE:
            if (((sh.sl.on && sh.sl.T > 0) || sh.sl.chroma_tabs) && sh.sl.role == 0 && sh.a2 >= 0) spec_tables(F, sh, sh.a2);
            else if (tid == 0) { sh.tab_from = 0; if (sh.sl.role == 0) { sh.par.ipis = F.ipis; sh.par.d5 = F.d5; sh.tab_shared = 0; } }
            __syncthreads();
            op_init_range(F, sh, sh.a0, sh.a1, sh.tab_from);
            break;
#else
        case OP_INIT_RANGE: op_init_range(F, sh, sh.a0, sh.a1, 0); FC_DUP(OP_INIT_RANGE, op_init_range(F, sh, sh.a0, sh.a1, 0)); break;
#endif
        case OP_APPROX:     op_approx(F, sh); break;
        case OP_IPIS_INCR:  op_ipis(F, sh, sh.a0, sh.a1, sh.a2, sh.a3); FC_DUP(OP_IPIS_INCR, op_ipis(F, sh, sh.a0, sh.a1, sh.a2, sh.a3)); break;
        case OP_APPEND:     op_append(F, sh, sh.a0); FC_DUP(OP_APPEND, op_append(F, sh, sh.a0)); break;
        case OP_CHROMA:
            op_chroma_pool(F, sh);
#if FC_SPEC
            if (sh.sl.chroma_tabs) {
                __threadfence();
                __syncthreads();
                if (tid == 0) {
                    FcSpecCtl *c = sh.sl.ctl;
                    c->ystates = (unsigned) sh.ystates;
                    __hip_atomic_store(&c->chroma_ready, 1u, __ATOMIC_RELEASE, __HIP_MEMORY_SCOPE_AGENT);
                }
            }
#endif
            break;
#if FC_VARIANT_BIG
        case OP_PRED_SETUP:  op_pred_setup(F, sh, sh.a0, sh.a1); break;
        case OP_PRED_FINISH: op_pred_finish(F, sh, sh.a0); break;
        case OP_NORMS:       op_norms(F, sh, sh.a0, sh.a1, sh.a2, sh.a3); break;
        case OP_MC_SEARCH:   op_mc_search(F, sh, sh.a0, sh.a1, sh.a2); break;
#endif
        default: break;
        }
        __syncthreads();
#if FC_SPEC
        if (tid == 0 && role && (++sh.sl.ops & 1u) == 0
            && __hip_atomic_load(&F.spec->epoch, __ATOMIC_RELAXED, __HIP_MEMORY_SCOPE_AGENT) != sh.sl.epoch) {
            sh.sl.abort = 1; sh.op = OP_DONE;
        } else
#endif
        if (tid == 0) {
            unsigned long long t1 = wall_clock64();
            tk[op] += t1 - t0;
#ifdef FC_SERIAL_PROFILE
            sh.ph_t0 = t1;
#endif
            serial_advance(F, sh);
#ifdef FC_SERIAL_PROFILE
            { unsigned long long t = wall_clock64(); sh.tk_ph[sh.ph_prev] += t - sh.ph_t0; }
#endif
            tk[0] += wall_clock64() - t1;
        }
    }
#if FC_SPEC
    if (!role) break;
    __syncthreads();
    if (tid == 0 && !sh.sl.abort
        && __hip_atomic_load(&F.spec->epoch, __ATOMIC_ACQUIRE, __HIP_MEMORY_SCOPE_AGENT) != sh.sl.epoch) sh.sl.abort = 1;
    __syncthreads();
    if (!sh.sl.abort && sh.sl.verdict == 3) {
        uint4 *dst = (uint4 *) (SPEC_SLOTS(F.spec) + (size_t) (FC_SPEC_W + (role - T - 1)) * SPEC_STRIDE);
        for (unsigned i = tid; i < sizeof(Sh) / 16; i += B) dst[i] = ((const uint4 *) &sh)[i];
        __threadfence();
        __syncthreads();
    }
    if (tid == 0) {
        if (!sh.sl.abort) {
            unsigned used = 0;
            while (used < FC_SPEC_TEMPS && F.level_of_state[sh.gap_hi + (int) used] != 0) used++;
            __hip_atomic_store(&F.spec->verdict[task_seq % FC_SPEC_W],
                               ((task_seq + 1) << 11) | ((role - T - 1) << 8) | (used << 2) | (unsigned) sh.sl.verdict,
                               __ATOMIC_RELEASE, __HIP_MEMORY_SCOPE_AGENT);
        }
        if (sh.sl.busy) { __threadfence(); atomicSub(&F.spec->busy, 1u); }
        if (!sh.sl.abort && sh.sl.verdict == 3) {
            while (__hip_atomic_load(&F.spec->epoch, __ATOMIC_ACQUIRE, __HIP_MEMORY_SCOPE_AGENT) == sh.sl.epoch
                   && __hip_atomic_load(&F.spec->committed, __ATOMIC_ACQUIRE, __HIP_MEMORY_SCOPE_AGENT) <= task_seq
                   && !__hip_atomic_load(&F.spec->done, __ATOMIC_ACQUIRE, __HIP_MEMORY_SCOPE_AGENT))
                __builtin_amdgcn_s_sleep(16);
            while (__hip_atomic_load(&F.spec->adopting, __ATOMIC_ACQUIRE, __HIP_MEMORY_SCOPE_AGENT)) __builtin_amdgcn_s_sleep(16);
        }
    }
    }
    if (role) {
        if (task_go == 2) spec_worker(F, sh, role, T, true);
        return;
    }
    if (tid == 0 && sh.sl.ctl && G > 1) {
        FcSpecCtl *const c = sh.sl.ctl;
        __hip_atomic_store(&c->epoch, sh.sl.epoch + 1, __ATOMIC_RELEASE, __HIP_MEMORY_SCOPE_AGENT);
        __hip_atomic_store(&c->done, 1u, __ATOMIC_RELEASE, __HIP_MEMORY_SCOPE_AGENT);
        c->n_tasks = sh.sl.n_tasks; c->n_confirmed = sh.sl.n_confirmed; c->n_wrong = sh.sl.n_wrong;
        c->n_timeout = sh.sl.n_timeout; c->n_inline = sh.sl.n_inline; c->t_wait = sh.sl.t_wait;
        c->n_tab_used = sh.sl.n_tab_used; c->n_tab_missed = sh.sl.n_tab_missed; c->n_adopted = sh.sl.n_adopted;
        c->n_app_dealt = sh.sl.n_app_dealt; c->t_app_wait = sh.sl.t_app_wait;
    }
#endif
    if (tid == 0) {
        F.t_serial = tk[0]; F.t_init = tk[OP_INIT_RANGE]; F.t_approx = tk[OP_APPROX];
        F.t_ipis = tk[OP_IPIS_INCR]; F.t_append = tk[OP_APPEND];
        F.t_total = wall_clock64() - t_begin;
        F.bytes_mp = sh.cnt.bytes_mp; F.bytes_img = sh.cnt.bytes_img; F.bytes_gram = sh.cnt.bytes_gram;
        F.n_mp = sh.cnt.n_mp; F.n_steps = sh.cnt.n_steps; F.n_blocks = sh.cnt.n_blocks;
        F.n_appends = sh.cnt.n_appends; F.n_fulleval = sh.cnt.n_fulleval;
        F.n_blockevals = sh.cnt.n_blockevals; F.t_mpA = sh.cnt.t_mpA; F.t_mpB = sh.cnt.t_mpB;
#if FC_VARIANT_BIG && !defined(FC_SERIAL_PROFILE)
        F.dbg[2] = tk[OP_CHROMA]; F.dbg[3] = tk[OP_PRED_SETUP]; F.dbg[4] = tk[OP_PRED_FINISH];
        F.dbg[5] = tk[OP_NORMS]; F.dbg[6] = tk[OP_MC_SEARCH];
#endif
#ifdef FC_SERIAL_PROFILE
        for (int k = 0; k < 8; k++) F.dbg[k] = sh.tk_ph[k];
        F.dbg[0] = sh.tk_init[0]; F.dbg[7] = sh.tk_init[1];
        F.dbg[3] = sh.tk_apx[0]; F.dbg[4] = sh.tk_apx[1]; F.dbg[5] = sh.tk_apx[2]; F.dbg[2] = sh.tk_apx[3];
#endif
    }
#if FC_SPEC && !defined(FC_SERIAL_PROFILE)
    if (tid == 0) { F.dbg[0] = tk[OP_SPEC_CKPT]; F.dbg[1] = 0; }
#endif
    if (tid == 0) {
#if FC_VARIANT_BIG && !FC_SPEC
        if (sh.coopW > 1 && F.coop) __hip_atomic_store(&F.coop->quit, 1u, __ATOMIC_RELAXED, __HIP_MEMORY_SCOPE_AGENT);
#endif
        F.states = sh.states;
        F.ystates_out = sh.band ? sh.ystates : sh.states;
        F.lc_min_out = sh.lc_min;
        F.status = sh.failed ? sh.failed : FC_OK;
#if FC_SPEC
        if (spec_bad) F.status = 128 + spec_bad;
#endif
    }
    if (F.pack_dst) {
        const uint4 *src = (const uint4 *) F.pack_src;
        uint4 *dst = (uint4 *) F.pack_dst;
        const unsigned n16 = F.pack_bytes / 16;
        for (unsigned i = tid; i < n16; i += B) dst[i] = src[i];
    }
#if !FC_SPEC
    if (ring) {
        __threadfence();
        __syncthreads();
        if (tid == 0) {
            const unsigned i = atomicAdd(&ctr[1], 1u);
            __hip_atomic_store(&ring[i], (unsigned long long) F.slab_base, __ATOMIC_RELEASE, __HIP_MEMORY_SCOPE_AGENT);
        }
    }
#endif
}

extern "C" int FC_OCCUPANCY(void)
{
    const int by_lds = (int) (163840 / sizeof(Sh));
    return by_lds < FC_WG_PER_CU ? (by_lds < 1 ? 1 : by_lds) : FC_WG_PER_CU;
}

#if FC_SPEC
extern "C" void FC_LAUNCH(DevFrame *d_frames, DevFrame *d_vframes, unsigned n, unsigned G, unsigned H, hipStream_t stream)
{
    hipLaunchKernelGGL(FC_KERNEL, dim3(n * (G + H)), dim3(B), 0, stream, d_frames, d_vframes, G, n, H);
}
extern "C" unsigned FC_SPEC_SLOT_BYTES(void) { return SPEC_STRIDE; }
#if !FC_VARIANT_WIDE
extern "C" unsigned fc_spec_ctl_bytes(void) { return (unsigned) ((sizeof(FcSpecCtl) + 255) / 256 * 256); }
#endif
#else
extern "C" void FC_LAUNCH(DevFrame *d_frames, unsigned n, unsigned nlend, unsigned long long *ring, unsigned *ctr,
                          const unsigned *ptrmask, unsigned long long queue_wait_ticks, unsigned coopW, hipStream_t stream)
{
    const unsigned grid = coopW > 1 ? (n + 7) / 8 * 8 * coopW : n;
    hipLaunchKernelGGL(FC_KERNEL, dim3(grid), dim3(B), 0, stream, d_frames, nlend, ring, ctr, ptrmask, queue_wait_ticks, coopW);
}
#endif
```

fiasco_amd/csrc/hip/mp_device.inc:

```

struct StepCtx {
    int      np;
    int      p[MAXED - 1];
    float    pre[MAXED];
    int      last[MAXED], k[MAXED], thr[MAXED];
    unsigned cd, has;
    float    sfx[MAXED - 1];
    float    z0, zy;
    int      ypos;
    float    wb_dc, wb_nd;
    float    ab, price, err;
    unsigned N;
};

__device__ __forceinline__ int   uni(int v)      { return __builtin_amdgcn_readfirstlane(v); }
__device__ __forceinline__ float unif(float v)   { return __int_as_float(__builtin_amdgcn_readfirstlane(__float_as_int(v))); }

__device__ __forceinline__ void load_step_ctx(const MPState &mp, StepCtx &c)
{
    c.np = uni(mp.np);
#pragma unroll
    for (int i = 0; i < MAXED - 1; i++) { c.p[i] = uni(mp.psorted[i]); c.sfx[i] = unif(mp.s1_sfx[i]); }
#pragma unroll
    for (int i = 0; i < MAXED; i++) {
// ... 194 lines not shown
#endif
        ev.m_bits = bits;
    }
    nov[NN] = den; ipio[NN] = num;
#pragma unroll
    for (int k = 0; k <= NN; k++)
#pragma unroll
        for (int l = 0; l <= NN; l++)
            if (l > k) r[k] += ipd[l][k] * r[l] / nov[k];
    float m_err = mp.norm;
#pragma unroll
    for (int k = 0; k <= NN; k++) m_err += r[k] * r[k] * nov[k] - 2 * r[k] * ipio[k];
    ev.m_err = m_err;
    ev.costs = (ev.m_bits + ev.w_bits + mp.ab) * mp.price + m_err;
#pragma unroll
    for (int k = 0; k < MAXED; k++) ev.f[k] = k <= NN ? f[k] : 0.0f;
}

template <int MAXN>
__device__ __forceinline__ void full_eval(const DevFrame &F, const Sh &sh, const MPState &mp, const double *lglv,
                                          int n, int d, int state,
                                          float num, float den, float ip0, float ip1, float ip2,
                                          float ip3, Eval &ev)
{
    if (n == 0) full_eval_n<0>(F, sh, mp, lglv, d, state, num, den, ip0, ip1, ip2, ip3, ev);
    else if (n == 1 && MAXN >= 1) full_eval_n<(MAXN >= 1 ? 1 : 0)>(F, sh, mp, lglv, d, state, num, den, ip0, ip1, ip2, ip3, ev);
    else if (n == 2 && MAXN >= 2) full_eval_n<(MAXN >= 2 ? 2 : 0)>(F, sh, mp, lglv, d, state, num, den, ip0, ip1, ip2, ip3, ev);
    else if (n == 3 && MAXN >= 3) full_eval_n<(MAXN >= 3 ? 3 : 0)>(F, sh, mp, lglv, d, state, num, den, ip0, ip1, ip2, ip3, ev);
    else if (MAXN >= 4) full_eval_n<(MAXN >= 4 ? 4 : 0)>(F, sh, mp, lglv, d, state, num, den, ip0, ip1, ip2, ip3, ev);
}

#if FC_HM
__device__ __noinline__ void mp_tables(const DevFrame &F, Sh &sh, int level, int y)
{
    const int tid = threadIdx.x;
    const int ctx = level - sh.par.lc_min_opt, dcs = sh.par.dcs, sy = sh.par.sy;
    const int nrole = dcs + sy + MAXED + 2;
    for (int t = tid; t < nrole; t += B) {
        const int r = t - dcs - sy;
        int ci, ti = 0;
        const bool coeff = r <= 0;
        if (t < dcs) ci = t;
        else if (r < 0) { ci = dcs + ctx * sy + t - dcs; ti = ctx + 1; }
        else if (r == 0) { ci = dcs + ctx * sy - 1; ti = ctx + 1; }
        else ci = r - 1;
        const float num = coeff ? (float) sh.cb.cnt[ci] : (float) sh.pool.count[ci];
        const float den = coeff ? (float) sh.cb.tot[ti] : (float) sh.pool.total;
        const double lg = log2((double) (num / den));
        if (t < dcs) sh.lgdc[t] = lg;
        else if (r < 0) sh.lglv[t - dcs] = lg;
        else if (r == 0) sh.lglv_m1 = lg;
        else sh.Ltab[ci] = (float) -lg;
    }
    __syncthreads();
    if (tid == 0) {
        const Pool &m = sh.pool;
        float q0 = 0, q1;
        if (m.d0_n && y != 0) q0 += sh.m0tab[qac_shift(m.d0_index)];
        if (y >= 0) q0 += sh.m0tab[qac_shift(m.d0_yindex)];
        q1 = q0;
        if (y == 0) { q1 -= sh.m0tab[qac_shift(m.d0_yindex)]; q1 += (float) qac_shift(m.d0_yindex); }
        else        { q1 -= sh.m0tab[qac_shift(m.d0_index)];  q1 += (float) qac_shift(m.d0_index); }
        sh.Q0 = q0; sh.Q1 = q1;
#if FC_GM
        {
            const int k = sh.gm.pk[0];
            sh.gm.base = 0.0f;
            if (GM_QAC(k)) {
                const int16_t *q = GQ_CUR(sh, 0), *list = F.pool_states;
                float bits = 0;
                for (int e = 0; e < (int) m.n; e++)
                    if (list[e] != y) bits += gm_m0(sh, q[e]);
                if (y >= 0) bits += gm_m0(sh, m.y_index);
                sh.gm.base = bits;
            } else if (k == FC_PK_UNIFORM) {
                const unsigned nn = m.n;
                sh.gm.base = (float) ((double) (0u - nn) * log2_host(sh, (float) (nn - 1) / (float) nn));
                sh.gm.lg1 = F.lginv[nn];
            }
        }
#endif
    }
}
#else
__device__ __noinline__ void mp_tables(const DevFrame &F, Sh &sh, int level, int y)
{
    const int tid = threadIdx.x;
    const int ctx = level - sh.par.lc_min_opt, dcs = sh.par.dcs, sy = sh.par.sy;
    const int om = 64 + sy + 12 <= 128 ? 64 + sy : 128;
    const int sl = (om + 12 <= 128 && B > 128) ? 128 : om + 11;
    if (tid == sl) {
        const Pool &m = sh.pool;
        float q0 = 0, q1;
        if (m.d0_n && y != 0) q0 += sh.m0tab[qac_shift(m.d0_index)];
        if (y >= 0) q0 += sh.m0tab[qac_shift(m.d0_yindex)];
        q1 = q0;
        if (y == 0) { q1 -= sh.m0tab[qac_shift(m.d0_yindex)]; q1 += (float) qac_shift(m.d0_yindex); }
        else        { q1 -= sh.m0tab[qac_shift(m.d0_index)];  q1 += (float) qac_shift(m.d0_index); }
        sh.Q0 = q0; sh.Q1 = q1;
#if !FC_VARIANT_BIG
        if (!sh.band) {
            MPState &mp = sh.mp;
            const unsigned N = (unsigned) sh.pool.n;
            mp.s1_last[0] = 1;
            const unsigned mv = N - 2u;
            if (mv != 0) {
                const unsigned kk = 31u - (unsigned) __clz((int) (mv + 1));
                const unsigned r = (mv + 1) - (1u << kk);
                mp.s1_cd = 1u; mp.s1_k[0] = (int) kk; mp.s1_thr[0] = (int) (mv + 1 - 2 * r);
            } else {
                mp.s1_cd = 0u; mp.s1_k[0] = 0; mp.s1_thr[0] = 0;
            }
            mp.s1_has = 0u;
            mp.np = 0;
        }
#endif
    }
    if (tid < om + 12) {
        int ci = 0, ti = 0, role = 0;
        const int r = tid - om;
        if (tid < dcs) { role = 1; ci = tid; ti = 0; }
        else if (tid >= 64 && tid < 64 + sy) { role = 1; ci = dcs + ctx * sy + tid - 64; ti = ctx + 1; }
        else if (r == 6) {
            role = 1; ci = dcs + ctx * sy - 1; ti = ctx + 1;
        }
        else if (r >= 0 && r < MAXED + 1) { role = 2; ci = r; }
#if !FC_VARIANT_BIG
        else if (r == 7 || r == 8) role = 3;
        else if (r == 9 && !sh.band) {
            role = 1; ci = dcs + ctx * sy + sh.par.half_nd; ti = ctx + 1;
        } else if (r == 10 && !sh.band) {
            role = 1; ci = sh.par.half_dc; ti = 0;
        }
#endif
        float num = 1.0f, den = 1.0f;
        if (role == 1)      { num = (float) sh.cb.cnt[ci]; den = (float) sh.cb.tot[ti]; }
        else if (role == 2) { num = (float) sh.pool.count[ci]; den = (float) sh.pool.total; }
#if !FC_VARIANT_BIG
        else if (role == 3) {
            const unsigned *counts = sh.tm;
            num = (float) counts[level]; den = (float) counts[sh.par.ML + level];
        }
#endif
        float p = num / den;
#if !FC_VARIANT_BIG
        if (r == 7) p = 1 - p;
#endif
        const double lg = log2((double) p);
        if (role == 1) {
            if (tid < dcs) sh.lgdc[tid] = lg;
            else if (r == 6) sh.lglv_m1 = lg;
#if !FC_VARIANT_BIG
            else if (r == 9) sh.mp.wb_nd = sub_log2(sh, 0.0f, lg, ci, ti);
            else if (r == 10) sh.mp.wb_dc = sub_log2(sh, 0.0f, lg, ci, ti);
#endif
            else sh.lglv[tid - 64] = lg;
        } else if (role == 2) sh.Ltab[ci] = (float) -lg;
#if !FC_VARIANT_BIG
        else if (role == 3) sh.tb[r - 7] = (float) -lg;
#endif
    }
}

#endif

__device__ void mp_step_prepare(const DevFrame &F, Sh &sh, MPState &mp, const double *lglv, double lglv_m1)
{
    float wb = 0;
    int np = 0;
    for (int k = 0; k < mp.n; k++)
        if (mp.weight[k] != 0) {
            const bool have = SYMP_HAS(mp.symp, k);
            if (mp.into[k]) {
                const int sym = have ? SYMP_GET(mp.symp, k) : rtob_dev(mp.weight[k], sh.par.rpf_mant, sh.par.rpf_range);
                {
                    const int ctx = mp.level - sh.par.lc_min_opt;
                    wb = sub_log2(sh, wb, sym >= 0 ? lglv[sym] : lglv_m1, sh.par.dcs + ctx * sh.par.sy + sym, ctx + 1);
                }
            }
            else {
                const int sym = have ? SYMP_GET(mp.symp, k) : rtob_dev(mp.weight[k], sh.par.dc_mant, sh.par.dc_range);
                wb = sym >= 0 ? sub_log2(sh, wb, sh.lgdc[sym], sym, 0)
                              : (float) ((double) wb + (double) INFINITY);
            }
            if (mp.indices[k] == mp.ypos) continue;
            int j = np++;
            while (j > 0 && mp.psorted[j - 1] > mp.indices[k]) { mp.psorted[j] = mp.psorted[j - 1]; j--; }
            mp.psorted[j] = mp.indices[k];
        }
    mp.np = np;
    {
        const unsigned N = (unsigned) mp.N;
        const short *p = mp.psorted;
        const bool p0zero = np > 0 && p[0] == 0;
        float e[MAXED];
        bool  ev[MAXED];
        for (int j = 0; j < np; j++) {
            if (j == 0) {
                ev[0] = p[0] != 0 && (N - 2) != 0;
                e[0] = ev[0] ? (float) bits_bin_code((unsigned) p[0] - 1, N - 2) : 0.0f;
            } else {
                ev[j] = (unsigned) p[j - 1] != N - 2;
                e[j] = ev[j] ? (float) bits_bin_code((unsigned) (p[j] - p[j - 1] - 1), N - 2 - (unsigned) p[j - 1]) : 0.0f;
            }
        }
        float b = sh.Ltab[np + 1];
        b += p0zero ? sh.Q1 : sh.Q0;
        unsigned cd = 0, has = 0;
        for (int i = 0; i <= np; i++) {
            mp.s1_pre[i] = b;
            unsigned last = i == 0 ? 1u : (unsigned) p[i - 1] + 1;
            unsigned mv = N - 1 - last;
            mp.s1_last[i] = (int) last;
            if (mv != 0) {
                unsigned kk = 31u - (unsigned) __clz((int) (mv + 1));
                unsigned r = (mv + 1) - (1u << kk);
                cd |= 1u << i;
                mp.s1_k[i] = (int) kk; mp.s1_thr[i] = (int) (mv + 1 - 2 * r);
            } else {
                mp.s1_k[i] = 0; mp.s1_thr[i] = 0;
            }
            if (i < np && ev[i]) b += e[i];
        }
        for (int j = 1; j < np; j++) { mp.s1_sfx[j] = e[j]; if (ev[j]) has |= 1u << j; }
        mp.s1_cd = cd; mp.s1_has = has;
        b = sh.Ltab[np + 1]; b += sh.Q1;
        for (int j = 0; j < np; j++) if (ev[j]) b += e[j];
        mp.s1_z0 = b;
        b = sh.Ltab[np]; b += p0zero ? sh.Q1 : sh.Q0;
        for (int j = 0; j < np; j++) if (ev[j]) b += e[j];
        mp.s1_zy = b;
    }
    {
        const int ctx = mp.level - sh.par.lc_min_opt;
        const int s_nd = sh.par.half_nd, s_dc = sh.par.half_dc;
        mp.wb_nd = sub_log2(sh, wb, lglv[s_nd], sh.par.dcs + ctx * sh.par.sy + s_nd, ctx + 1);
        mp.wb_dc = sub_log2(sh, wb, sh.lgdc[s_dc], s_dc, 0);
    }
#if FC_GM
    {
        const int k = sh.gm.pk[0];
        float b = sh.gm.base;
        if (GM_QAC(k)) {
// ... 15 lines not shown
            mp.wb_dc = w; mp.wb_dc += (float) (sh.par.dc_mant + 1);
        }
    }
#endif
#if FC_VARIANT_BIG
    mp.min_costs = F.full_search ? MAXCOSTS : mp.costs;
#else
    mp.min_costs = mp.costs;
#endif
}

__device__ void models_update(const DevFrame &F, Sh &sh, const short *indices, const short *into,
                              const float *weight, int level, int y, unsigned symp = SYMP_NONE)
{
    Pool &m = sh.pool;
    int state_0 = 0, state_y = 0, edge = 0;
#if FC_GM
    if (GM_QAC(sh.gm.pk[0])) {
        int16_t *q = GQ_CUR(sh, 0);
        const int16_t *list = F.pool_states;
        int used_y = 0, y_is_domain = y >= 0 && F.pos[y] >= 0 && F.pos[y] < (int) m.n;
        short nv[MAXED + 1], np_[MAXED + 1];
        int nu = 0;
        for (int e = 0; indices[e] != NOEDGE; e++) {
            const int p = indices[e];
            if (into[e] == y && y >= 0) {
                if (y_is_domain) { np_[nu] = (short) p; nv[nu] = q[p]; nu++; }
                m.y_index >>= 1;
                used_y = 1;
            } else { np_[nu] = (short) p; nv[nu] = (short) (q[p] >> 1); nu++; }
        }
        (void) list;
        for (int i = 0; i < ((int) m.n + 7) / 8; i++) {
            uint4 v = ((uint4 *) q)[i];
            unsigned *w = (unsigned *) &v;
            for (int j = 0; j < 4; j++) {
                unsigned lo = (w[j] & 0xffffu) + 1, hi = (w[j] >> 16) + 1;
                if (lo > 1020) lo = 1020;
                if (hi > 1020) hi = 1020;
                w[j] = lo | (hi << 16);
            }
            ((uint4 *) q)[i] = v;
        }
        for (int i = 0; i < nu; i++) q[np_[i]] = nv[i] > 1020 ? (short) 1020 : nv[i];
        if (y >= 0 && !used_y) m.y_index++;
        if (m.y_index > 1020) m.y_index = 1020;
    } else if (!GM_RLE(sh.gm.pk[0])) {
    } else {
#endif
    for (; indices[edge] != NOEDGE; edge++) {
        if (into[edge] == 0) state_0 = 1;
        else if (into[edge] == y) state_y = 1;
    }
    m.count[edge]++;
    m.total++;
    {
        int used_y = 0, y_is_domain = 0;
        if (m.d0_n) { m.d0_index++; if (y == 0) y_is_domain = 1; }
        if (state_0) {
            if (y == 0) { if (y_is_domain) m.d0_index--; m.d0_yindex >>= 1; used_y = 1; }
            else { m.d0_index--; m.d0_index >>= 1; }
        }
        if (y >= 0 && !used_y) m.d0_yindex++;
        if (m.d0_n && m.d0_index > 1020) m.d0_index = 1020;
        if (m.d0_yindex > 1020) m.d0_yindex = 1020;
    }
    if (state_y) m.y_index >>= 1; else m.y_index++;
    if (m.y_index > 1020) m.y_index = 1020;
#if FC_GM
    }
    if (sh.gm.ck[0] == FC_CK_UNIFORM) return;
#endif
    int ctx = level - sh.par.lc_min_opt;
    for (int e = 0; into[e] != NOEDGE; e++) {
        const bool have = SYMP_HAS(symp, e);
        if (into[e]) {
            sh.cb.cnt[sh.par.dcs + ctx * sh.par.sy + (have ? SYMP_GET(symp, e) : rtob_dev(weight[e], sh.par.rpf_mant, sh.par.rpf_range))]++;
            sh.cb.tot[ctx + 1]++;
        } else {
            sh.cb.cnt[have ? SYMP_GET(symp, e) : rtob_dev(weight[e], sh.par.dc_mant, sh.par.dc_range)]++;
            sh.cb.tot[0]++;
        }
    }
}

__device__ __forceinline__ float wave_min_l63(float v)
{
    asm volatile(
        "s_nop 1\n\t"
        "v_min_f32_dpp %0, %0, %0 row_shr:1 row_mask:0xf bank_mask:0xf\n\t"
        "s_nop 1\n\t"
        "v_min_f32_dpp %0, %0, %0 row_shr:2 row_mask:0xf bank_mask:0xf\n\t"
        "s_nop 1\n\t"
        "v_min_f32_dpp %0, %0, %0 row_shr:4 row_mask:0xf bank_mask:0xf\n\t"
        "s_nop 1\n\t"
        "v_min_f32_dpp %0, %0, %0 row_shr:8 row_mask:0xf bank_mask:0xf\n\t"
        "s_nop 1\n\t"
        "v_min_f32_dpp %0, %0, %0 row_bcast:15 row_mask:0xa bank_mask:0xf\n\t"
        "s_nop 1\n\t"
        "v_min_f32_dpp %0, %0, %0 row_bcast:31 row_mask:0xc bank_mask:0xf\n\t"
        "s_nop 1"
        : "+v"(v));
    return v;
}

__device__ __forceinline__ void wave_min4_l63(float &a, float &b, float &c, float &d)
{
#define MIN4_STEP(ctl)                                                     \
        "v_min_f32_dpp %0, %0, %0 " ctl "\n\t"                             \
        "v_min_f32_dpp %1, %1, %1 " ctl "\n\t"                             \
        "v_min_f32_dpp %2, %2, %2 " ctl "\n\t"                             \
        "v_min_f32_dpp %3, %3, %3 " ctl "\n\t"
    asm volatile(
        "s_nop 1\n\t"
        MIN4_STEP("row_shr:1 row_mask:0xf bank_mask:0xf")
        MIN4_STEP("row_shr:2 row_mask:0xf bank_mask:0xf")
        MIN4_STEP("row_shr:4 row_mask:0xf bank_mask:0xf")
        MIN4_STEP("row_shr:8 row_mask:0xf bank_mask:0xf")
        MIN4_STEP("row_bcast:15 row_mask:0xa bank_mask:0xf")
        MIN4_STEP("row_bcast:31 row_mask:0xc bank_mask:0xf")
        "s_nop 1"
        : "+v"(a), "+v"(b), "+v"(c), "+v"(d));
#undef MIN4_STEP
}

__device__ __forceinline__ float wave_min(float v)
{
    return __int_as_float(__builtin_amdgcn_readlane(__float_as_int(wave_min_l63(v)), 63));
}

#if FC_VARIANT_BIG
#define MP_NUMROW(F, mp)    ((mp).numrow)
__device__ __forceinline__ bool mp_excluded(const MPState &mp, int pos)
{
    bool x = false;
    bool live = true;
#pragma unroll
    for (int i = 0; i < MAXED; i++) {
        live = live && mp.excl[i] != NOEDGE;
        x = x || (live && mp.excl[i] == pos);
    }
    return x;
}
#define MP_EXCLUDED(mp, pos) mp_excluded(mp, pos)
#else
#define MP_NUMROW(F, mp)    (sh.par.ipis + (size_t) (mp).image * sh.par.P)
#define MP_EXCLUDED(mp, pos) false
#endif

__device__ __forceinline__ void lds_barrier()
{
    asm volatile("s_waitcnt lgkmcnt(0)\n\ts_barrier" ::: "memory");
}

#include "mp_reg.inc"

__device__ __noinline__ void mp_steps_global(DevFrame &F, Sh &sh, int q, float size)
{
    const int tid = threadIdx.x, lane = tid & 63, wave = tid >> 6, P = F.P;
    MPState &mp = sh.mp;
    const int S = sh.states;
    const int nblk = (S + 63) >> 6;
    constexpr int U = 4;
    unsigned long long tA = 0, tB = 0, tmark = wall_clock64();
    unsigned blockevals = 0;
    for (;;) {
// ... 22 lines not shown
                    dd[u] = base + u * B + tid;
                    ps[u] = dd[u] < S && !DEAD(sh, dd[u]) ? (int) F.pos[dd[u]] : -1;
                    in[u] = ps[u] >= 0;
                    us[u] = (in[u] && n) ? F.used[dd[u]] != 0 : !in[u];
                }
                if (n == 0) {
#pragma unroll
                    for (int u = 0; u < U; u++) {
                        den[u] = in[u] ? diag[dd[u]] : 1.0f;
                        num[u] = in[u] ? numrow[dd[u]] : 0.0f;
                    }
#pragma unroll
                    for (int u = 0; u < U; u++) {
                        if (!in[u]) continue;
                        bool uu = den[u] / size < MIN_NORM;
                        if (!uu) uu = fabsf(num[u]) < MIN_NORM;
                        if (MP_EXCLUDED(mp, ps[u])) uu = true;
                        us[u] = uu;
                        F.num[dd[u]] = num[u]; F.den[dd[u]] = den[u]; F.used[dd[u]] = uu;
                    }
                } else {
#pragma unroll
                    for (int u = 0; u < U; u++) {
                        bool on = !us[u];
                        num[u] = on ? F.num[dd[u]] : 0.0f;
                        den[u] = on ? F.den[dd[u]] : 1.0f;
                        g[u] = on ? gram_load(Gq, P, mp.row_state, dd[u], flim) : 0.0f;
#pragma unroll
                        for (int k = 0; k < MAXED - 1; k++)
                            ip[u][k] = (on && k < nv) ? F.ipdo[(size_t) k * P + dd[u]] : 0.0f;
                    }
#pragma unroll
                    for (int u = 0; u < U; u++) {
                        if (us[u]) continue;
                        float t = g[u];
#pragma unroll
                        for (int k = 0; k < MAXED - 1; k++)
                            if (k < nv) t -= ip[u][k] / novk[k] * selk[k];
                        F.ipdo[(size_t) nv * P + dd[u]] = t;
                        den[u] -= t * t / nov_nv;
                        num[u] -= ipio_nv / nov_nv * t;
                        if (den[u] / size < MIN_NORM) { us[u] = true; F.used[dd[u]] = 1; }
                        F.num[dd[u]] = num[u]; F.den[dd[u]] = den[u];
                    }
                }
#pragma unroll
                for (int u = 0; u < U; u++) {
                    e[u] = BIGF;
                    if (in[u] && !us[u]) e[u] = stage1<MAXED - 1>(ctx, ps[u], dd[u], num[u], den[u]);
                    if (dd[u] < S) F.est[dd[u]] = e[u];
                    float bm = wave_min(e[u]);
                    int blk = ((base + u * B) >> 6) + wave;
                    if (lane == 0 && blk < NBLOCKMIN) sh.blockmin[blk] = bm;
                }
            }
        }
        __syncthreads();
        if (tid == 0) { unsigned long long t = wall_clock64(); tA += t - tmark; tmark = t; }
        if (wave == 0) {
            float m = mp.min_costs;
            unsigned evals = 0;
            int b_state = -1;
            float b_cost = 0, b_mbits = 0, b_wbits = 0, b_err = 0, b_f[MAXED];
#pragma unroll
            for (int k = 0; k < MAXED; k++) b_f[k] = 0;
            for (int bb = 0; bb < nblk; bb += 64) {
                float bm = (bb + lane < nblk) ? sh.blockmin[bb + lane] : BIGF;
                int lastb = -1;
                for (;;) {
                    unsigned long long mask = __ballot(bm < m && lane > lastb);
                    if (!mask) break;
                    int jb = __ffsll((long long) mask) - 1;
                    lastb = jb;
                    int d = ((bb + jb) << 6) + lane;
                    float e = (d < S) ? F.est[d] : BIGF;
                    bool pass = e < m;
                    Eval ev;
                    ev.costs = BIGF; ev.m_bits = ev.w_bits = ev.m_err = 0;
#pragma unroll
                    for (int k = 0; k < MAXED; k++) ev.f[k] = 0;
                    if (pass) {
                        float i0 = n > 0 ? F.ipdo[d] : 0.0f, i1 = n > 1 ? F.ipdo[(size_t) P + d] : 0.0f;
                        float i2 = n > 2 ? F.ipdo[(size_t) 2 * P + d] : 0.0f, i3 = n > 3 ? F.ipdo[(size_t) 3 * P + d] : 0.0f;
                        full_eval<MAXED - 1>(F, sh, mp, sh.lglv, n, F.pos[d], d, F.num[d], F.den[d], i0, i1, i2, i3, ev);
                    }
                    evals += (unsigned) __popcll(__ballot(pass));
                    blockevals++;
                    int last = -1, win = -1;
                    for (;;) {
                        unsigned long long ok = __ballot(pass && lane > last && e < m && ev.costs < m);
                        if (!ok) break;
                        int j = __ffsll((long long) ok) - 1;
                        last = j; win = j;
                        m = __shfl(ev.costs, j);
                    }
                    if (win >= 0) {
                        b_state = ((bb + jb) << 6) + win;
                        b_cost = __shfl(ev.costs, win); b_mbits = __shfl(ev.m_bits, win);
                        b_wbits = __shfl(ev.w_bits, win); b_err = __shfl(ev.m_err, win);
#pragma unroll
                        for (int k = 0; k < MAXED; k++) b_f[k] = __shfl(ev.f[k], win);
                    }
                }
            }
            if (lane == 0) {
                sh.cnt.n_fulleval += evals;
                int index = b_state >= 0 ? (int) F.pos[b_state] : -1;
                if (index >= 0) {
                    if (b_cost < mp.costs) {
                        mp.costs = b_cost; mp.err = b_err;
                        mp.matrix_bits = b_mbits; mp.weights_bits = b_wbits;
#pragma unroll
                        for (int k = 0; k < MAXED; k++) if (k <= n) mp.weight[k] = b_f[k];
                        mp.symp = SYMP_NONE;
                        mp.best_n = n + 1;
                    }
                    mp.indices[n] = (short) index;
                    mp.into[n] = (short) b_state;
                    F.used[b_state] = 1;
                    mp.norm_ov[n] = F.den[b_state];
                    mp.ipio[n] = F.num[b_state];
#pragma unroll
                    for (int k = 0; k < MAXED - 1; k++)
                        if (k < n) mp.sel_ipdo[n][k] = F.ipdo[(size_t) k * P + b_state];
                    mp.row_state = b_state;
                    mp.n = n + 1;
                    if (mp.n < F.max_elements) mp_step_prepare(F, sh, mp, sh.lglv, sh.lglv_m1);
                }
                mp.index = index;
            }
        }
        __syncthreads();
        if (tid == 0) { unsigned long long t = wall_clock64(); tB += t - tmark; tmark = t; }
        if (!(mp.n < F.max_elements && mp.index >= 0)) break;
    }
    if (tid == 0) { sh.cnt.t_mpA += tA; sh.cnt.t_mpB += tB; sh.cnt.n_blockevals += blockevals; }
}

#if FC_VARIANT_BIG
__device__ __noinline__ void mp_steps_list_global(DevFrame &F, Sh &sh, int q, float size, int D)
{
    const int tid = threadIdx.x, lane = tid & 63, wave = tid >> 6, P = F.P;
    MPState &mp = sh.mp;
    const int16_t *const list = F.pool_states;
    const int nblk = (D + 63) >> 6;
    unsigned blockevals = 0;
    for (;;) {
        const int n = mp.n;
        {
            const float *Gq = GRAM(F, q);
            const int flim = sh.flim;
            const float *diag = F.diag + (size_t) q * P;
            const float *numrow = MP_NUMROW(F, mp);
            const int nv = n - 1;
            StepCtx ctx;
            load_step_ctx(mp, ctx);
            for (int base = 0; base < nblk * 64; base += B) {
                const int c = base + tid;
                const bool in = c < D;
                const int st = in ? (int) list[c] : 0;
                bool us = in ? (n ? F.used[c] != 0 : false) : true;
                float num = 0.0f, den = 1.0f;
                if (in && n == 0) {
                    den = diag[st]; num = numrow[st];
                    bool uu = den / size < MIN_NORM;
                    if (!uu) uu = fabsf(num) < MIN_NORM;
                    if (MP_EXCLUDED(mp, c)) uu = true;
                    us = uu;
                    F.num[c] = num; F.den[c] = den; F.used[c] = uu;
                } else if (!us) {
                    num = F.num[c]; den = F.den[c];
                    float t = gram_load(Gq, P, mp.row_state, st, flim);
                    for (int k = 0; k < MAXED - 1; k++)
                        if (k < nv) t -= F.ipdo[(size_t) k * P + c] / mp.norm_ov[k] * mp.sel_ipdo[nv][k];
                    F.ipdo[(size_t) nv * P + c] = t;
                    den -= t * t / mp.norm_ov[nv];
                    num -= mp.ipio[nv] / mp.norm_ov[nv] * t;
                    if (den / size < MIN_NORM) { us = true; F.used[c] = 1; }
                    F.num[c] = num; F.den[c] = den;
                }
                float e = BIGF;
#if FC_GM
                if (in && !us && !GM_RLE(sh.gm.pk[0])) {
                    const int pk = sh.gm.pk[0];
                    float bits = sh.gm.kept;
                    if (GM_QAC(pk)) {
                        const int qi = c == mp.ypos ? (int) sh.pool.y_index : (int) GQ_CUR(sh, 0)[c < (int) sh.pool.n ? c : 0];
                        bits -= gm_m0(sh, qi); bits += gm_m1(qi);
                    } else if (pk == FC_PK_UNIFORM) bits = (float) ((double) bits - sh.gm.lg1);
                    else bits = 0;
                    const float wbits = st ? ctx.wb_nd : ctx.wb_dc;
                    e = (bits + wbits + ctx.ab) * ctx.price + ctx.err - num * num / den;
                } else
#endif
                if (in && !us) e = stage1<MAXED - 1>(ctx, c, st, num, den);
                if (in) F.est[c] = e;
                const float bm = wave_min(e);
                const int blk = (base >> 6) + wave;
                if (lane == 0 && blk < NBLOCKMIN) sh.blockmin[blk] = bm;
            }
        }
        __syncthreads();
        if (wave == 0) {
            float m = mp.min_costs;
            unsigned evals = 0;
            int b_idx = -1;
            float b_cost = 0, b_mbits = 0, b_wbits = 0, b_err = 0, b_f[MAXED];
#pragma unroll
            for (int k = 0; k < MAXED; k++) b_f[k] = 0;
            for (int bb = 0; bb < nblk; bb += 64) {
                float bm = (bb + lane < nblk) ? sh.blockmin[bb + lane] : BIGF;
                int lastb = -1;
                for (;;) {
                    unsigned long long mask = __ballot(bm < m && lane > lastb);
                    if (!mask) break;
                    int jb = __ffsll((long long) mask) - 1;
                    lastb = jb;
                    const int c = ((bb + jb) << 6) + lane;
                    float e = (c < D) ? F.est[c] : BIGF;
                    bool pass = e < m;
                    Eval ev;
                    ev.costs = BIGF; ev.m_bits = ev.w_bits = ev.m_err = 0;
#pragma unroll
                    for (int k = 0; k < MAXED; k++) ev.f[k] = 0;
                    if (pass) {
                        float i0 = n > 0 ? F.ipdo[c] : 0.0f, i1 = n > 1 ? F.ipdo[(size_t) P + c] : 0.0f;
                        float i2 = n > 2 ? F.ipdo[(size_t) 2 * P + c] : 0.0f, i3 = n > 3 ? F.ipdo[(size_t) 3 * P + c] : 0.0f;
#if FC_GM
                        ev.qc = GM_QAC(sh.gm.pk[0]) && c < (int) sh.pool.n ? (int) GQ_CUR(sh, 0)[c] : 0;
#endif
                        full_eval<MAXED - 1>(F, sh, mp, sh.lglv, n, c, list[c], F.num[c], F.den[c], i0, i1, i2, i3, ev);
                    }
                    evals += (unsigned) __popcll(__ballot(pass));
                    blockevals++;
                    int last = -1, win = -1;
                    for (;;) {
                        unsigned long long ok = __ballot(pass && lane > last && e < m && ev.costs < m);
                        if (!ok) break;
                        int j = __ffsll((long long) ok) - 1;
                        last = j; win = j;
                        m = __shfl(ev.costs, j);
                    }
                    if (win >= 0) {
                        b_idx = ((bb + jb) << 6) + win;
                        b_cost = __shfl(ev.costs, win); b_mbits = __shfl(ev.m_bits, win);
                        b_wbits = __shfl(ev.w_bits, win); b_err = __shfl(ev.m_err, win);
#pragma unroll
                        for (int k = 0; k < MAXED; k++) b_f[k] = __shfl(ev.f[k], win);
                    }
                }
            }
            if (lane == 0) {
                sh.cnt.n_fulleval += evals;
                const int index = b_idx;
                if (index >= 0) {
                    const int b_state = list[index];
                    if (b_cost < mp.costs) {
                        mp.costs = b_cost; mp.err = b_err;
                        mp.matrix_bits = b_mbits; mp.weights_bits = b_wbits;
#pragma unroll
                        for (int k = 0; k < MAXED; k++) if (k <= n) mp.weight[k] = b_f[k];
                        mp.symp = SYMP_NONE;
                        mp.best_n = n + 1;
                    }
                    mp.indices[n] = (short) index;
                    mp.into[n] = (short) b_state;
#if FC_GM
                    mp.kq[n] = GM_QAC(sh.gm.pk[0]) && index < (int) sh.pool.n ? GQ_CUR(sh, 0)[index] : (short) 0;
#endif
                    F.used[index] = 1;
                    mp.norm_ov[n] = F.den[index];
                    mp.ipio[n] = F.num[index];
#pragma unroll
                    for (int k = 0; k < MAXED - 1; k++)
                        if (k < n) mp.sel_ipdo[n][k] = F.ipdo[(size_t) k * P + index];
                    mp.row_state = b_state;
                    mp.n = n + 1;
                    if (mp.n < F.max_elements) mp_step_prepare(F, sh, mp, sh.lglv, sh.lglv_m1);
                }
                mp.index = index;
            }
        }
        __syncthreads();
        if (!(mp.n < F.max_elements && mp.index >= 0)) break;
    }
    if (tid == 0) sh.cnt.n_blockevals += blockevals;
}
#endif

__device__ __noinline__ void mp_steps_chroma(DevFrame &F, Sh &sh, int q, float size, int D)
{
#if FC_VARIANT_BIG
    if (F.chroma_max > 63) { mp_steps_list_global(F, sh, q, size, D); return; }
#endif
    mp_steps_list<MAXED - 1>(F, sh, q, size, D);
}

__device__ __forceinline__ void op_approx(DevFrame &F, Sh &sh)
{
    const int tid = threadIdx.x, lane = tid & 63, wave = tid >> 6, P = sh.par.P;
    SFrame &fr = sh.st[sh.sp];
    MPState &mp = sh.mp;
    const int level = fr.lrange.level;
    const float size = (float) (1u << level);
    const int q = level - sh.par.gl0;
    const int D = sh.pool.n;
    int y = fr.y_state;
    if (y >= 0 && !(F.domain_type[y] & 2)) y = -1;

#ifdef FC_SERIAL_PROFILE
    unsigned long long tp = wall_clock64();
#define APX_MARK(i) do { if (tid == 0) { unsigned long long t_ = wall_clock64(); sh.tk_apx[i] += t_ - tp; tp = t_; } } while (0)
#else
#define APX_MARK(i) do { } while (0)
#endif
    if (fr.coop) snap_coop_before(sh, fr, sh.sp, sh.par.ML);
    mp_tables(F, sh, level, y);
    __syncthreads();
    APX_MARK(0);
    const int S = sh.states;
    const bool regscan = !sh.band && S <= KREG * B && sh.par.max_elements <= FC_NIP + 1;
    Step0 pre;
#if !FC_VARIANT_BIG
    if (regscan) mp_step0_issue(sh, q, sh.par.ipis + (size_t) fr.lrange.image * P, pre);
#endif
#if FC_VARIANT_BIG
    const bool retries = F.second_domain_block || F.check_underflow || F.check_overflow;
    if (tid == 0) {
        sh.apx_stage = 0; sh.apx_it = -1;
        mp.excl[0] = NOEDGE;
        for (int k = 0; k < MAXED; k++) mp.weight[k] = 0;
    }
#else
    const bool retries = false;
#endif
    for (;;) {
    if (tid == 0) {
        mp.n = 0; mp.best_n = 0; mp.symp = SYMP_NONE;
        mp.D = D; mp.N = D;
        mp.y_state = y; mp.ypos = -1;
        if (sh.band) {
            int ypos = -1;
#if FC_VARIANT_BIG
#if FC_GM
            if (sh.gm.pk[0] == FC_PK_UNIFORM || sh.gm.pk[0] == FC_PK_CONSTANT) {
            } else
#endif
            if (FC_GM || F.chroma_max > 63) {
                if (y >= 0) {
                    ypos = F.pos[y];
                    if (ypos < 0 || ypos >= D) { F.pool_states[D] = (short) y; ypos = D; mp.D = D + 1; }
                }
            } else
#endif
            if (y >= 0) {
                for (int i = 0; i < D; i++) if (sh.dl[i] == y) ypos = i;
                if (ypos < 0) { sh.dl[D] = (short) y; ypos = D; mp.D = D + 1; }
            }
            mp.ypos = ypos;
        }
        mp.level = level; mp.image = fr.lrange.image; mp.address = fr.lrange.address;
#if FC_VARIANT_BIG
        if (level > sh.par.images_level) {
            mp.norm = sh.norms[mp.image];
            mp.numrow = sh.par.ipis + (size_t) mp.image * P;
        } else {
            const int npx = 1 << level;
            const float *px = sh.pixels + mp.address * npx;
            float nrm = 0;
            for (int k = 0; k < npx; k++) nrm += px[k] * px[k];
            mp.norm = nrm;
            mp.numrow = (level == sh.par.images_level ? ACT_D5(F, sh) : ACT_D4(F, sh)) + (size_t) mp.address * P;
        }
#else
        mp.norm = sh.norms[mp.image];
#endif
#if FC_VARIANT_BIG
        mp.ab = fr.lrange.tree_bits + fr.lrange.mv_tree_bits + fr.lrange.mv_coord_bits + fr.lrange.nd_tree_bits
                + fr.lrange.nd_weights_bits;
#else
        fr.lrange.tree_bits = sh.tb[0];
        mp.ab = sh.tb[0];
#endif
        mp.price = fr.price;
        mp.err = mp.norm;
        mp.weights_bits = 0;
        mp.matrix_bits = sh.Ltab[0] + sh.Q0;
#if FC_GM
        if (!GM_RLE(sh.gm.pk[0])) mp.matrix_bits = sh.gm.pk[0] == FC_PK_CONSTANT ? 0.0f : sh.gm.base;
#endif
        mp.costs = (mp.matrix_bits + mp.weights_bits + mp.ab) * mp.price + mp.err;
        mp.index = -1;
#if FC_VARIANT_BIG
        mp_step_prepare(F, sh, mp, sh.lglv, sh.lglv_m1);
#else
        if (sh.band) mp_step_prepare(F, sh, mp, sh.lglv, sh.lglv_m1);
        else {
            const float L0 = sh.Ltab[0], L1 = sh.Ltab[1], q0 = sh.Q0, q1 = sh.Q1;
            float b = L1; b += q0; mp.s1_pre[0] = b;
            b = L1; b += q1; mp.s1_z0 = b;
            b = L0; b += q0; mp.s1_zy = b;
            mp.min_costs = mp.costs;
        }
#endif
    }
    lds_barrier();

    APX_MARK(1);
#if FC_GM
    if (true) {
        mp_steps_list_global(F, sh, q, size, mp.D);
    } else
#endif
    if (sh.band) {
        mp_steps_chroma(F, sh, q, size, mp.D);
    } else if (regscan) {
#if FC_VARIANT_BIG
        mp_step0_issue(sh, q, MP_NUMROW(F, mp), pre);
#endif
#if FC_VARIANT_BIG
        const int kslots = (sh.states + B - 1) / B;
        if (sh.par.max_elements <= 3) {
            if (kslots <= KREG / 4) mp_steps_reg<2, KREG / 4>(F, sh, q, size, pre);
            else if (kslots <= KREG / 2) mp_steps_reg<2, KREG / 2>(F, sh, q, size, pre);
            else mp_steps_reg<2>(F, sh, q, size, pre);
        } else if (kslots <= KREG / 4) mp_steps_reg<FC_NIP, KREG / 4>(F, sh, q, size, pre);
        else if (kslots <= KREG / 2) mp_steps_reg<FC_NIP, KREG / 2>(F, sh, q, size, pre);
        else
#endif
        mp_steps_reg<FC_NIP>(F, sh, q, size, pre);
    } else {
        mp_steps_global(F, sh, q, size);
    }
    APX_MARK(2);
    if (!retries) break;
#if FC_VARIANT_BIG
    __syncthreads();
    if (tid == 0) {
        MPState &best = sh.mp_keep;
        mp.indices[mp.best_n] = NOEDGE;
        mp.costs = (mp.matrix_bits + mp.weights_bits + mp.ab) * mp.price + mp.err;
        if (sh.apx_stage == 0) best = mp;
        else if (mp.costs < best.costs) best = mp;
        int more = 0;
        while (!more && sh.apx_stage < 4) {
            if (sh.apx_stage == 0) {
                sh.apx_stage = 1;
                if (F.second_domain_block && (best.indices[0] != NOEDGE || F.full_search)) {
                    mp.excl[0] = best.indices[0]; mp.excl[1] = NOEDGE;
                    more = 1;
                }
            } else if (sh.apx_stage == 1 || sh.apx_stage == 2) {
                const bool on = sh.apx_stage == 1 ? F.check_underflow != 0 : F.check_overflow != 0;
                if (!on) { sh.apx_stage++; sh.apx_it = -1; continue; }
                if (sh.apx_it < 0) mp = best;
                else if (!(sh.apx_it < MAXED - 1)) { sh.apx_stage++; sh.apx_it = -1; continue; }
                const int it = ++sh.apx_it;
                mp.excl[it] = NOEDGE;
                for (int i = 0; mp.indices[i] != NOEDGE; i++) {
                    bool hit;
                    if (sh.apx_stage == 1) hit = mp.weight[i] == 0;
                    else {
                        const int mant = mp.indices[i] ? sh.par.rpf_mant : sh.par.dc_mant;
                        const float range = mp.indices[i] ? sh.par.rpf_range : sh.par.dc_range;
                        hit = mp.weight[i] == btor_fast(rtob_dev(200.0f, mant, range), mant, range)
                              || mp.weight[i] == btor_fast(rtob_dev(-200.0f, mant, range), mant, range);
                    }
                    if (hit) { mp.excl[it] = mp.indices[i]; break; }
                }
                if (mp.excl[it] != NOEDGE) { mp.excl[it + 1] = NOEDGE; more = 1; }
                else { sh.apx_stage++; sh.apx_it = -1; }
            } else sh.apx_stage = 4;
        }
        if (!more) mp = best;
        sh.apx_more = more;
    }
    __syncthreads();
    if (!sh.apx_more) break;
#endif
    }

    if (tid == 0) {
        Range &lr = fr.lrange;
        mp.indices[mp.best_n] = NOEDGE;
        float costs = (mp.matrix_bits + mp.weights_bits + mp.ab) * mp.price + mp.err;
        if (costs < fr.max_costs) {
            int ni = 0;
            unsigned sp = 0;
            for (int oi = 0; mp.indices[oi] != NOEDGE; oi++)
                if (mp.weight[oi] != 0) {
                    mp.indices[ni] = mp.indices[oi]; mp.into[ni] = mp.into[oi];
                    mp.weight[ni] = mp.weight[oi];
                    if (oi < 3) sp |= ((mp.symp >> (10 * oi)) & 1023u) << (10 * ni);
                    ni++;
                }
            mp.indices[ni] = NOEDGE; mp.into[ni] = NOEDGE;
            models_update(F, sh, mp.indices, mp.into, mp.weight, level, mp.y_state, sp);
            int e = 0;
            for (; mp.indices[e] != NOEDGE; e++) { lr.into[e] = mp.into[e]; lr.weight[e] = mp.weight[e]; }
            lr.into[e] = NOEDGE;
            lr.matrix_bits = mp.matrix_bits; lr.weights_bits = mp.weights_bits; lr.err = mp.err;
        } else {
            lr.into[0] = NOEDGE;
            costs = MAXCOSTS;
        }
        fr.lincomb = costs;
#if FC_SPEC
        if (fr.ckpt == 2 && sh.sl.role == 0) {
            Sh::SpecLocal &sl = sh.sl;
            const unsigned slot = (sl.head - 1) % FC_SPEC_W;
            if (sl.nospec) { sl.nospec = 0; sl.n_inline++; }
            else if (costs < (sl.nlc >= 8 ? SPEC_THR * sl.mlc : MAXCOSTS) && !sh.failed) {
                sl.spec_mask |= 1u << slot;
                sl.lin[slot] = costs;
                fr.ckpt = 3;
            } else sl.n_inline++;
        }
#endif
        if (sh.par.trace_on && F.trace_n < F.trace_cap) {
            FcTrace &t = F.trace[F.trace_n];
            t.seq = F.trace_n; t.level = level; t.image = mp.image; t.D = D; t.states = sh.states;
            t.cost = costs; t.err = mp.err; t.mbits = mp.matrix_bits; t.wbits = mp.weights_bits;
            int e = 0;
            for (; e < 6; e++) { t.into[e] = -1; if (e < 5) t.w[e] = 0; }
            for (e = 0; costs < MAXCOSTS && lr.into[e] != NOEDGE; e++) { t.into[e] = lr.into[e]; t.w[e] = lr.weight[e]; }
            t.nedges = e;
            F.trace_n++;
        }
#if FC_VARIANT_BIG
        sh.cnt.bytes_mp += 4ull * D * (2 + mp.n) + 4ull * (1u << level);
        sh.cnt.n_mp++; sh.cnt.n_steps += mp.n;
#endif
    }
#if !FC_VARIANT_BIG
    else if (tid == 64) {
        sh.cnt.bytes_mp += 4ull * D * (2 + mp.n) + 4ull * (1u << level);
        sh.cnt.n_mp++; sh.cnt.n_steps += mp.n;
    }
#endif
    if (fr.coop) {
        __syncthreads();
        snap_coop_after(sh, fr, sh.sp);
    }
    APX_MARK(3);
#undef APX_MARK
}
```

fiasco_amd/csrc/hip/mp_reg.inc:

```

#define KREG FC_KREG
#define NWAVES (B / 64)

struct Step0 { unsigned praw[KREG]; float draw[KREG], nraw[KREG]; };

#if FC_SPEC
#define SPEC_DEADMASK(sh) const unsigned deadmask_ = (unsigned) __builtin_amdgcn_readfirstlane((int) (sh).deadmask);
#define SLOT_LIVE(k)      (!((deadmask_ >> (k)) & 1u))
#else
#define SPEC_DEADMASK(sh)
#define SLOT_LIVE(k)      true
#endif

__device__ __forceinline__ void mp_step0_issue(const Sh &sh, int q, const float *numrow, Step0 &o)
{
    unsigned utid = threadIdx.x;
    asm volatile("" : "+v"(utid));
    const int P = sh.par.P, S = sh.states, K = (S + B - 1) / B;
    const float *diag = sh.par.diag + (size_t) q * P;
    const unsigned short *pos = (const unsigned short *) sh.par.pos;
    SPEC_DEADMASK(sh)
#pragma unroll
    for (int k = 0; k < KREG; k++) {
        o.praw[k] = 0xffffu; o.draw[k] = 1.0f; o.nraw[k] = 0.0f;
// ... 129 lines not shown
                if (den[k] * rsize < MIN_NORM) usmask |= 1u << k;
            }
        }
#define EST_ONE(NPV, k, ek)                                                                      \
        float ek = BIGF;                                                                         \
        if ((k) < K && !((usmask >> (k)) & 1u))                                                  \
            ek = stage1<NIP, NPV, true>(ctx, PS(k), (k) * B + tid, num[k], den[k]);
#define EST_PASS(NPV)                                                                            \
        _Pragma("unroll")                                                                        \
        for (int k4 = 0; k4 + 4 <= KR; k4 += 4) {                                              \
            if (k4 < K) {                                       \
                EST_ONE(NPV, k4, e0) EST_ONE(NPV, k4 + 1, e1) EST_ONE(NPV, k4 + 2, e2) EST_ONE(NPV, k4 + 3, e3) \
                wave_min4_l63(e0, e1, e2, e3);                                                   \
                if (lane == 63) {                                                                \
                    sh.blockmin[NWAVES * k4 + wave] = e0;                                        \
                    if (k4 + 1 < K) sh.blockmin[NWAVES * (k4 + 1) + wave] = e1;                  \
                    if (k4 + 2 < K) sh.blockmin[NWAVES * (k4 + 2) + wave] = e2;                  \
                    if (k4 + 3 < K) sh.blockmin[NWAVES * (k4 + 3) + wave] = e3;                  \
                }                                                                                \
            }                                                                                    \
        }                                                                                        \
        _Pragma("unroll")                                                                        \
        for (int k = KR / 4 * 4; k < KR; k++) {                                              \
            if (k < K) {                                                                         \
                EST_ONE(NPV, k, ek)                                                              \
                ek = wave_min_l63(ek);                                                           \
                if (lane == 63) sh.blockmin[NWAVES * k + wave] = ek;                             \
            }                                                                                    \
        }
        if (ctx.np == 0)      { EST_PASS(0) }
        else if (ctx.np == 1) { EST_PASS(1) }
        else                  { EST_PASS(-1) }
#undef EST_PASS
#undef EST_ONE
        if (tid == 0) { rb.m2[1] = mp.min_costs; rb.state = -1; }
        __syncthreads();
        if (tid == 0) { unsigned long long t = wall_clock64(); tA += t - tmark; tmark = t; }

        float m = rb.m2[1];
        int round = 0;
        int cursor = -1;
        for (;;) {
            int jb = -1;
            for (int bb = 0; bb < nblk && jb < 0; bb += 64) {
                float bmv = (bb + lane < nblk) ? sh.blockmin[bb + lane] : BIGF;
                unsigned long long mask = __ballot(bmv < m && bb + lane > cursor);
                if (mask) jb = bb + __ffsll((long long) mask) - 1;
            }
            if (jb < 0) break;
            cursor = jb;
            if (jb % NWAVES == wave) {
                const int kk = jb / NWAVES;
                float numk = 0, denk = 1, ipk[NIP];
                int psk = -1;
#pragma unroll
                for (int j = 0; j < NIP; j++) ipk[j] = 0;
#pragma unroll
                for (int k = 0; k < KR; k++)
                    if (k == kk) {
                        numk = num[k]; denk = den[k]; psk = PS(k);
#pragma unroll
                        for (int j = 0; j < NIP - 1; j++) ipk[j] = ip[k][j];
                    }
                const int state = kk * B + tid;
                if (n == NIP) {
                    const int nv = NIP - 1;
                    float t = 0.0f;
                    if (!((usmask >> kk) & 1u)) {
                        t = gram_load(PGRAM(sh, q), P, mp.row_state, state, sh.flim);
#pragma unroll
                        for (int j = 0; j < NIP - 1; j++)
                            if (j < nv) t -= ipk[j] / mp.norm_ov[j] * mp.sel_ipdo[nv][j];
                    }
                    ipk[NIP - 1] = t;
                }
                const float ek = ((usmask >> kk) & 1u) ? BIGF : stage1<NIP>(ctx, psk, state, numk, denk);
                bool pass = ek < m;
                Eval ev;
                ev.costs = BIGF; ev.m_bits = ev.w_bits = ev.m_err = 0; ev.symp = SYMP_NONE;
#pragma unroll
                for (int k = 0; k < MAXED; k++) ev.f[k] = 0;
                const float i0 = ipk[0], i1 = NIP > 1 ? ipk[1 % NIP] : 0.0f;
                const float i2 = NIP > 2 ? ipk[2 % NIP] : 0.0f, i3 = NIP > 3 ? ipk[3 % NIP] : 0.0f;
                if (pass) full_eval<NIP>(F, sh, mp, sh.lglv, n, psk, state, numk, denk, i0, i1, i2, i3, ev);
                unsigned npass = (unsigned) __popcll(__ballot(pass));
                int last = -1, win = -1;
                for (;;) {
                    unsigned long long ok = __ballot(pass && lane > last && ek < m && ev.costs < m);
                    if (!ok) break;
                    int j = __ffsll((long long) ok) - 1;
                    last = j; win = j;
                    m = __shfl(ev.costs, j);
                }
                if (lane == win) {
                    rb.state = state; rb.idx = psk;
                    rb.cost = ev.costs; rb.mbits = ev.m_bits; rb.wbits = ev.w_bits;
                    rb.err = ev.m_err; rb.symp = ev.symp;
#pragma unroll
                    for (int k = 0; k < MAXED; k++) rb.f[k] = ev.f[k];
                    rb.num = numk; rb.den = denk;
#pragma unroll
                    for (int j = 0; j < MAXED - 1; j++) rb.ip[j] = j < NIP ? ipk[j % NIP] : 0.0f;
                }
                if (lane == 0) { rb.m2[round & 1] = m; rb.evals += npass; rb.blockevals++; }
            }
            __syncthreads();
            m = rb.m2[round & 1];
            round++;
        }
        if (tid == 0) {
            const int bstate = rb.state;
            int index = bstate >= 0 ? rb.idx : -1;
            if (index >= 0) {
                if (rb.cost < mp.costs) {
                    mp.costs = rb.cost; mp.err = rb.err;
                    mp.matrix_bits = rb.mbits; mp.weights_bits = rb.wbits;
#pragma unroll
                    for (int k = 0; k < MAXED; k++) if (k <= n) mp.weight[k] = rb.f[k];
                    mp.symp = rb.symp;
                    mp.best_n = n + 1;
                }
                mp.indices[n] = (short) index;
                mp.into[n] = (short) bstate;
                mp.norm_ov[n] = rb.den;
                mp.ipio[n] = rb.num;
#pragma unroll
                for (int k = 0; k < MAXED - 1; k++) if (k < n) mp.sel_ipdo[n][k] = rb.ip[k];
                mp.row_state = bstate;
                mp.n = n + 1;
                if (mp.n < sh.par.max_elements) mp_step_prepare(F, sh, mp, sh.lglv, sh.lglv_m1);
            }
            mp.index = index;
        }
        __syncthreads();
        if (tid == 0) { unsigned long long t = wall_clock64(); tB += t - tmark; tmark = t; }
        if (!(mp.n < sh.par.max_elements && mp.index >= 0)) break;
    }
    if (tid == 0) {
        sh.cnt.n_fulleval += rb.evals; sh.cnt.n_blockevals += rb.blockevals;
        sh.cnt.t_mpA += tA; sh.cnt.t_mpB += tB;
    }
}
#undef PS

template <int NIP>
__device__ __forceinline__ void mp_steps_list(DevFrame &F, Sh &sh, int q, float size, int D)
{
    const int tid = threadIdx.x, P = sh.par.P;
    MPState &mp = sh.mp;
    RoundBox &rb = sh.rb;
    const bool ok = tid < D;
    const int st = ok ? (int) sh.dl[tid] : 0;
    float den = ok ? sh.par.diag[(size_t) q * P + st] : 1.0f;
    float num = ok ? MP_NUMROW(F, mp)[st] : 0.0f;
    float ip[NIP];
#pragma unroll
    for (int j = 0; j < NIP; j++) ip[j] = 0.0f;
    bool used = !ok;
    unsigned evals = 0, steps = 0;

    for (;;) {
        const int n = mp.n;
        StepCtx ctx;
        load_step_ctx(mp, ctx);
        if (n == 0) {
            if (ok) {
                bool uu = den / size < MIN_NORM;
                if (!uu) uu = fabsf(num) < MIN_NORM;
                used = uu || MP_EXCLUDED(mp, tid);
            }
        } else {
            const int nv = n - 1;
            if (tid == (int) mp.indices[nv]) used = true;
            if (!used) {
                float t = gram_load(PGRAM(sh, q), P, mp.row_state, st, sh.flim);
#pragma unroll
                for (int j = 0; j < NIP; j++)
                    if (j < nv) t -= ip[j] / mp.norm_ov[j] * mp.sel_ipdo[nv][j];
#pragma unroll
                for (int j = 0; j < NIP; j++)
                    if (j == nv) ip[j] = t;
                den -= t * t / mp.norm_ov[nv];
                num -= mp.ipio[nv] / mp.norm_ov[nv] * t;
                if (den / size < MIN_NORM) used = true;
            }
        }
        if (tid < 64) {
            const int lane = tid;
            float e = used ? BIGF : stage1<NIP>(ctx, tid, st, num, den);
            float m = mp.min_costs;
            bool pass = e < m;
            Eval ev;
            ev.costs = BIGF; ev.m_bits = ev.w_bits = ev.m_err = 0; ev.symp = SYMP_NONE;
#pragma unroll
            for (int k = 0; k < MAXED; k++) ev.f[k] = 0;
            if (pass)
                full_eval<NIP>(F, sh, mp, sh.lglv, n, tid, st, num, den, ip[0], NIP > 1 ? ip[1 % NIP] : 0.0f,
                          NIP > 2 ? ip[2 % NIP] : 0.0f, NIP > 3 ? ip[3 % NIP] : 0.0f, ev);
            evals += (unsigned) __popcll(__ballot(pass));
            int last = -1, win = -1;
            for (;;) {
                unsigned long long okm = __ballot(pass && lane > last && e < m && ev.costs < m);
                if (!okm) break;
                int j = __ffsll((long long) okm) - 1;
                last = j; win = j;
                m = __shfl(ev.costs, j);
            }
            if (lane == 0) rb.state = -1;
            if (lane == win) {
                rb.state = st; rb.idx = tid;
                rb.cost = ev.costs; rb.mbits = ev.m_bits; rb.wbits = ev.w_bits; rb.err = ev.m_err; rb.symp = ev.symp;
#pragma unroll
                for (int k = 0; k < MAXED; k++) rb.f[k] = ev.f[k];
                rb.num = num; rb.den = den;
#pragma unroll
                for (int j = 0; j < MAXED - 1; j++) rb.ip[j] = j < NIP ? ip[j % NIP] : 0.0f;
            }
        }
        __syncthreads();
        if (tid == 0) {
            const int bstate = rb.state;
            const int index = bstate >= 0 ? rb.idx : -1;
            if (index >= 0) {
                if (rb.cost < mp.costs) {
                    mp.costs = rb.cost; mp.err = rb.err;
                    mp.matrix_bits = rb.mbits; mp.weights_bits = rb.wbits;
#pragma unroll
                    for (int k = 0; k < MAXED; k++) if (k <= n) mp.weight[k] = rb.f[k];
                    mp.symp = rb.symp;
                    mp.best_n = n + 1;
                }
                mp.indices[n] = (short) index;
                mp.into[n] = (short) bstate;
                mp.norm_ov[n] = rb.den;
                mp.ipio[n] = rb.num;
#pragma unroll
                for (int k = 0; k < MAXED - 1; k++) if (k < n) mp.sel_ipdo[n][k] = rb.ip[k];
                mp.row_state = bstate;
                mp.n = n + 1;
                if (mp.n < sh.par.max_elements) mp_step_prepare(F, sh, mp, sh.lglv, sh.lglv_m1);
            }
            mp.index = index;
        }
        steps++;
        __syncthreads();
        if (!(mp.n < sh.par.max_elements && mp.index >= 0)) break;
    }
    if (tid == 0) { sh.cnt.n_fulleval += evals; sh.cnt.n_blockevals += steps; }
}
```

include/libfiasco_amd_hip.h:

```cpp
#ifndef LIBFIASCO_AMD_HIP_H
#define LIBFIASCO_AMD_HIP_H 1
#include <stddef.h>
#include <stdint.h>
#include "libfiasco_amd.h"
#ifdef __cplusplus
extern "C" {
#endif

typedef struct fiasco_amd_stats {
    double             kernel_ms;
    unsigned long long launches;
    unsigned long long frames;
    unsigned long long bytes_mp, bytes_img, bytes_gram;
    unsigned long long n_mp, n_steps, n_blocks, n_appends, n_fulleval;
    unsigned long long t_init, t_approx, t_ipis, t_append, t_serial, t_total;
    unsigned long long t_mpA, t_mpB, n_blockevals;
    unsigned long long dbg[8];
    unsigned long long states_sum, states_max, reencodes;
    unsigned long long frames_by_build[5];
    unsigned long long spec_frames, spec_tasks, spec_confirmed, spec_wrong, spec_timeout, spec_inline, spec_wait;
    unsigned long long spec_tab_used, spec_tab_missed;
    unsigned long long spec_adopted;
    unsigned long long decoder_frames, decoder_bytes, decoder_us;
    unsigned long long coop_frames, coop_workgroups;
    unsigned long long spec_app_rows, spec_app_wait;
} fiasco_amd_stats;

void fiasco_amd_get_stats(fiasco_amd_stats *out);
void fiasco_amd_reset_stats(void);

int fiasco_amd_spec_workgroups(unsigned frames, int cus, int big_frames, int narrow_only, int occupancy);

const char *fiasco_amd_core_name(void);

int fiasco_amd_rccl_gather(void *comm, void *stream, int rank, int world, int root,
                           unsigned n_local, const unsigned char *const *data, const size_t *len,
                           unsigned char ***all, size_t **all_len, unsigned *n_all);

unsigned fiasco_amd_coop_workgroups(unsigned frames, int cus);
int fiasco_amd_spec_append_helpers(unsigned frames, int cus, int G, int wide_build);
unsigned fiasco_amd_share_of(unsigned share_key, unsigned index, unsigned shares);
int fiasco_amd_set_device(int device);
int fiasco_amd_set_devices(const int *ids, int n);
int fiasco_amd_device_count(void);

enum { FIASCO_AMD_GRAY8 = 0, FIASCO_AMD_RGB8_INTERLEAVED = 1, FIASCO_AMD_RGB8_PLANAR = 2 };
typedef struct fiasco_amd_device_frame {
    const void *data;
    size_t pitch;
    size_t plane_stride;
    unsigned width, height;
    int layout;
} fiasco_amd_device_frame;

fiasco_amd_batch_t *fiasco_amd_batch_stage_device(unsigned n, const fiasco_amd_device_frame *frames,
                                                  void *stream, float quality, const fiasco_c_options_t *options);
int fiasco_amd_batch_upload_device(fiasco_amd_batch_t *b, const fiasco_amd_device_frame *frames, void *stream);
int fiasco_amd_batch_input_planes(const fiasco_amd_batch_t *b, unsigned i, int16_t *out);

typedef struct fiasco_amd_device_target {
    void *data;
    size_t pitch;
    size_t plane_stride;
    unsigned width, height;
    int layout;
} fiasco_amd_device_target;

int fiasco_amd_batch_decode_device(const fiasco_amd_batch_t *b, const fiasco_amd_device_target *targets, void *stream);
int fiasco_amd_planes_to_pixels_device(const int16_t *planes, int color, const fiasco_amd_device_target *target, void *stream);

void fiasco_amd_release_memory(void);

int fiasco_amd_selftest_log2(unsigned exp_lo, unsigned exp_hi, unsigned long long *n_checked,
                             unsigned long long *n_double, unsigned long long *n_float,
                             float *first_bad);

unsigned long long fiasco_amd_selftest_log2_max_ulp(void);
int fiasco_amd_selftest_log2_patched(unsigned exp_lo, unsigned exp_hi, unsigned long long *n_checked,
                                     unsigned long long *n_double, unsigned long long *n_entries);

#ifdef __cplusplus
}
#endif
#endif
```

Before: 599.6.

## Cache rate-model log tables across matching-pursuit calls with generation tags

Builds the log-probability tables for all level contexts at once and tags them with a coefficient-model generation counter, the pool counts and the tree-model counts. When a later matching-pursuit call finds the tags unchanged, it reuses the tables and skips the per-call log2 recomputation. The table build grows to cover several contexts, and speculative tasks invalidate the tags when they reload state. An optional check mode recomputes the tables and flags any mismatch. The cost is extra LDS for the per-context tables and tags, plus a tag comparison on every call.

Result: no change. 602.3, median of 3 (+0.5%).

```diff
diff --git a/fiasco_amd/__init__.py b/fiasco_amd/__init__.py
--- a/fiasco_amd/__init__.py
+++ b/fiasco_amd/__init__.py
@@ -71,7 +71,8 @@
                 ("decoder_frames", ctypes.c_ulonglong), ("decoder_bytes", ctypes.c_ulonglong),
                 ("decoder_us", ctypes.c_ulonglong), ("coop_frames", ctypes.c_ulonglong),
                 ("coop_workgroups", ctypes.c_ulonglong),
-                ("spec_app_rows", ctypes.c_ulonglong), ("spec_app_wait", ctypes.c_ulonglong)]
+                ("spec_app_rows", ctypes.c_ulonglong), ("spec_app_wait", ctypes.c_ulonglong),
+                ("tab_builds", ctypes.c_ulonglong), ("tab_hits", ctypes.c_ulonglong)]
 
 
 def build(verbose=False):
diff --git a/fiasco_amd/csrc/hip/core_hip.cpp b/fiasco_amd/csrc/hip/core_hip.cpp
--- a/fiasco_amd/csrc/hip/core_hip.cpp
+++ b/fiasco_amd/csrc/hip/core_hip.cpp
@@ -1444,6 +1444,7 @@
     g_stats.t_init += F.t_init; g_stats.t_approx += F.t_approx; g_stats.t_ipis += F.t_ipis;
     g_stats.t_append += F.t_append; g_stats.t_serial += F.t_serial; g_stats.t_total += F.t_total;
     g_stats.t_mpA += F.t_mpA; g_stats.t_mpB += F.t_mpB; g_stats.n_blockevals += F.n_blockevals;
+    g_stats.tab_builds += F.n_tab_build; g_stats.tab_hits += F.n_tab_hit;
     for (int k = 0; k < 8; k++) g_stats.dbg[k] += F.dbg[k];
     g_stats.states_sum += ns;
     if (ns > g_stats.states_max) g_stats.states_max = ns;
@@ -1864,6 +1865,7 @@
     else if (st == FC_ERR_NOROOT) msg = "No root state generated!";
     else if (st == FC_ERR_QUEUE) msg = "device coder: frame queue gave no slab";
     else if (st == FC_ERR_COOP) msg = "device coder: the helper workgroups of the frame did not answer";
+    else if (st == FC_ERR_TABCHECK) msg = "device coder: a reused rate-model table differs from its recomputation";
     else if (st == FC_ERR_INTERNAL) msg = "device coder: frame exceeds a built-in capacity (recursion depth, snapshot stack or 16384 states)";
     if (st > FC_ERR_QUEUE) snprintf(job->errmsg, sizeof job->errmsg, "%s (status %d)", msg, st);
     else snprintf(job->errmsg, sizeof job->errmsg, "%s", msg);
diff --git a/fiasco_amd/csrc/hip/fc_config.inc b/fiasco_amd/csrc/hip/fc_config.inc
--- a/fiasco_amd/csrc/hip/fc_config.inc
+++ b/fiasco_amd/csrc/hip/fc_config.inc
@@ -92,6 +92,12 @@
 #endif
 #define FC_PRIO_ROTATE (!FC_VARIANT_BIG && !FC_VARIANT_WIDE && !FC_SPEC)
 #define FC_PRIO_SHIFT 20
+#define FC_TABREUSE (!FC_VARIANT_BIG)
+#define FC_TAB_CTX  8
+#define FC_TAB_LV   128
+#ifndef FC_TABCHECK
+#define FC_TABCHECK 0
+#endif
 #define MAXED   FC_MAXED
 #define FC_MAXE (FC_NIP + 1)
 #define NOEDGE  (-1)
diff --git a/fiasco_amd/csrc/hip/fc_lds.inc b/fiasco_amd/csrc/hip/fc_lds.inc
--- a/fiasco_amd/csrc/hip/fc_lds.inc
+++ b/fiasco_amd/csrc/hip/fc_lds.inc
@@ -125,10 +125,22 @@
     __attribute__((aligned(16))) unsigned tm[TM_WORDS];
     __attribute__((aligned(16))) unsigned snap_tm[SNAP_TM_WORDS];
     float    m0tab[12];
+#if FC_TABREUSE
+    double   lgdc[FC_MAXSYM], lglv[FC_TAB_LV], lglv_m1[FC_TAB_CTX];
+    float    Ltab[MAXED + 1];
+    float    Q0, Q1;
+    float    tb[FC_TAB_CTX][2], wb_nd[FC_TAB_CTX], wb_dc;
+    float    tbc[2];
+    int      tab_slot, tab_off;
+    int      tab_nctx;
+    struct { unsigned cb; short pool[MAXED + 2]; unsigned tm[FC_TAB_CTX][2]; } tag;
+    unsigned gen_ctr;
+#else
     double   lgdc[FC_MAXSYM], lglv[FC_MAXSYM], lglv_m1;
     float    Ltab[MAXED + 1];
     float    Q0, Q1;
     float    tb[2];
+#endif
     MPState  mp;
 #if FC_VARIANT_BIG
     MPState  mp_keep;
@@ -140,7 +152,7 @@
     unsigned long long tk[16];
     struct {
         unsigned long long bytes_mp, bytes_img, bytes_gram, n_mp, n_steps, n_blocks, n_appends,
-                           n_fulleval, n_blockevals, t_mpA, t_mpB;
+                           n_fulleval, n_blockevals, t_mpA, t_mpB, n_tab_build, n_tab_hit;
     } cnt;
 #ifdef FC_SERIAL_PROFILE
     unsigned long long tk_ph[8], ph_t0, tk_init[2], tk_apx[4];
@@ -210,6 +222,14 @@
     } sl;
 #endif
 };
+#if FC_TABREUSE
+#define CB_GEN(sh)       (*(unsigned *) &(sh).cb.tot[14])
+#define MP_LGLV(sh)      ((sh).lglv + (sh).tab_off)
+#define MP_LGLV_M1(sh)   ((sh).lglv_m1[(sh).tab_slot])
+#else
+#define MP_LGLV(sh)      ((sh).lglv)
+#define MP_LGLV_M1(sh)   ((sh).lglv_m1)
+#endif
 #if FC_GM
 #define GM_QAC(k)   ((k) == FC_PK_ADAPTIVE || (k) == FC_PK_BASIS)
 #define GM_RLE(k)   ((k) == FC_PK_RLE || (k) == FC_PK_RLE_NO_CHROMA)
diff --git a/fiasco_amd/csrc/hip/fc_serial.inc b/fiasco_amd/csrc/hip/fc_serial.inc
--- a/fiasco_amd/csrc/hip/fc_serial.inc
+++ b/fiasco_amd/csrc/hip/fc_serial.inc
@@ -511,7 +511,7 @@
 #if FC_VARIANT_BIG
                 fr.rrange.tree_bits = tree_bits_dev(sh, ML, 1, rg.level, 0);
 #else
-                fr.rrange.tree_bits = rg.level <= sh.par.lc_max ? sh.tb[1] : tree_bits_dev(sh, ML, 1, rg.level, 0);
+                fr.rrange.tree_bits = rg.level <= sh.par.lc_max ? sh.tbc[1] : tree_bits_dev(sh, ML, 1, rg.level, 0);
 #endif
                 fr.rrange.matrix_bits = 0;
                 fr.rrange.weights_bits = 0;
diff --git a/fiasco_amd/csrc/hip/frame_coder.h b/fiasco_amd/csrc/hip/frame_coder.h
--- a/fiasco_amd/csrc/hip/frame_coder.h
+++ b/fiasco_amd/csrc/hip/frame_coder.h
@@ -38,7 +38,8 @@
 
 enum { FC_OK = 1, FC_ERR_STATES = 2, FC_ERR_CAPACITY = 3, FC_ERR_NOROOT = 4, FC_ERR_INTERNAL = 5,
        FC_ERR_QUEUE = 6,
-       FC_ERR_COOP = 7 };
+       FC_ERR_COOP = 7,
+       FC_ERR_TABCHECK = 8 };
 struct FcCoop {
     unsigned seq;
     unsigned done;
@@ -138,6 +139,7 @@
     unsigned long long n_mp, n_steps, n_blocks, n_appends, n_fulleval;
     unsigned long long t_init, t_approx, t_ipis, t_append, t_serial, t_total;
     unsigned long long t_mpA, t_mpB, n_blockevals;
+    unsigned long long n_tab_build, n_tab_hit;
     unsigned long long dbg[8];
     struct FcTrace *trace;
     int      trace_cap, trace_n;
diff --git a/fiasco_amd/csrc/hip/frame_coder.hip b/fiasco_amd/csrc/hip/frame_coder.hip
--- a/fiasco_amd/csrc/hip/frame_coder.hip
+++ b/fiasco_amd/csrc/hip/frame_coder.hip
@@ -106,6 +106,8 @@
     __shared__ Sh::SpecLocal sl_keep;
     __shared__ unsigned task_seq, spec_slot, spec_used, spec_vid;
     __shared__ int task_go, spec_act, spec_bad;
+    __shared__ unsigned gen_keep;
+#define SPEC_TAB_LOADED(sh, keep) do { (sh).tag.cb = 0; (sh).gen_ctr = ((keep) > (sh).gen_ctr ? (keep) : (sh).gen_ctr) + 1; } while (0)
     if (threadIdx.x == 0) spec_bad = 0;
     if (blockIdx.x >= n * G) {
         const unsigned k = blockIdx.x - n * G;
@@ -195,6 +197,7 @@
         sl.verdict = 0; sl.abort = 0; sl.ops = 0; sl.mlc = 0.0f; sl.nlc = 0; sl.learn = 0.0f;
         sl.n_tasks = sl.n_confirmed = sl.n_wrong = sl.n_timeout = sl.n_inline = sl.t_wait = 0;
         sl_keep = sl;
+        gen_keep = 0;
     }
     if (role == 0) {
 #endif
@@ -208,6 +211,7 @@
         sh.cnt.bytes_mp = sh.cnt.bytes_img = sh.cnt.bytes_gram = 0;
         sh.cnt.n_mp = sh.cnt.n_steps = sh.cnt.n_blocks = sh.cnt.n_appends = sh.cnt.n_fulleval = 0;
         sh.cnt.t_mpA = sh.cnt.t_mpB = sh.cnt.n_blockevals = 0;
+        sh.cnt.n_tab_build = sh.cnt.n_tab_hit = 0;
         F.trace_n = 0;
         for (int k = 0; k < 8; k++) F.dbg[k] = 0;
 #ifdef FC_LATENCY_PROBE
@@ -334,6 +338,11 @@
         for (int i = 0; i < F.coeff_size; i++) sh.cb.cnt[i] = 1;
         sh.cb.tot[0] = (short) F.dcs;
         for (int i = 1; i < F.coeff_nt; i++) sh.cb.tot[i] = (short) F.sy;
+#if FC_TABREUSE
+        sh.tab_nctx = mp_tab_levels(F);
+        sh.tag.cb = 0; sh.gen_ctr = 1;
+        if (sh.tab_nctx) CB_GEN(sh) = 1;
+#endif
 #if FC_VARIANT_BIG
         for (int i = 0; i < FC_MAXCOEFF_BIG; i++) sh.dcb.cnt[i] = 0;
         for (int i = 0; i < 16; i++) sh.dcb.tot[i] = 0;
@@ -427,6 +436,7 @@
                          && __hip_atomic_load(&c->epoch, __ATOMIC_ACQUIRE, __HIP_MEMORY_SCOPE_AGENT) == task_epoch;
             sh.sl = sl_keep;
             sh.sl.epoch = task_epoch;
+            SPEC_TAB_LOADED(sh, gen_keep);
             const int S0 = sh.states, TB = F.spec_tb;
             if (valid && (S0 > TB || sh.sp < 0 || sh.sp >= FC_DEPTH)) valid = false;
             sh.sl.floor = sh.sp; sh.sl.verdict = 2; sh.sl.abort = valid ? 0 : 1; sh.sl.ops = 0; sh.sl.busy = 0;
@@ -521,7 +531,7 @@
                     sh.sl.sk[slot] = (unsigned) sh.states;
                 }
             } else if (spec_act == 3) {
-                if (tid == 0) sl_keep = sh.sl;
+                if (tid == 0) { sl_keep = sh.sl; gen_keep = sh.gen_ctr; }
                 __builtin_amdgcn_fence(__ATOMIC_ACQUIRE, "agent");
                 __syncthreads();
                 const uint4 *src = (const uint4 *) (sl_keep.slots + (size_t) (FC_SPEC_W + spec_vid) * SPEC_STRIDE);
@@ -531,6 +541,7 @@
                 __syncthreads();
                 if (tid == 0) {
                     sh.sl = sl_keep;
+                    SPEC_TAB_LOADED(sh, gen_keep);
                     sh.sl.nospec = 0;
                     sh.sl.commit = sh.sl.head;
                     sh.sl.rb_s[sh.sl.epoch % 32u] = (unsigned) S0;
@@ -597,7 +608,7 @@
                     __hip_atomic_store(&c->adopting, 0u, __ATOMIC_RELEASE, __HIP_MEMORY_SCOPE_AGENT);
             } else if (spec_act == 2) {
                 const unsigned slot = spec_slot;
-                if (tid == 0) sl_keep = sh.sl;
+                if (tid == 0) { sl_keep = sh.sl; gen_keep = sh.gen_ctr; }
                 __builtin_amdgcn_fence(__ATOMIC_ACQUIRE, "agent");
                 __syncthreads();
                 const uint4 *src = (const uint4 *) (sl_keep.slots + (size_t) slot * SPEC_STRIDE);
@@ -605,6 +616,7 @@
                 __syncthreads();
                 if (tid == 0) {
                     sh.sl = sl_keep;
+                    SPEC_TAB_LOADED(sh, gen_keep);
                     sh.sl.nospec = 1;
                     sh.sl.commit = sh.sl.head;
                     sh.sl.rb_s[sh.sl.epoch % 32u] = (unsigned) sh.states;
@@ -689,6 +701,7 @@
         __syncthreads();
     }
     if (tid == 0) {
+        gen_keep = sh.gen_ctr;
         if (!sh.sl.abort) {
             unsigned used = 0;
             while (used < FC_SPEC_TEMPS && F.level_of_state[sh.gap_hi + (int) used] != 0) used++;
@@ -728,6 +741,7 @@
         F.n_mp = sh.cnt.n_mp; F.n_steps = sh.cnt.n_steps; F.n_blocks = sh.cnt.n_blocks;
         F.n_appends = sh.cnt.n_appends; F.n_fulleval = sh.cnt.n_fulleval;
         F.n_blockevals = sh.cnt.n_blockevals; F.t_mpA = sh.cnt.t_mpA; F.t_mpB = sh.cnt.t_mpB;
+        F.n_tab_build = sh.cnt.n_tab_build; F.n_tab_hit = sh.cnt.n_tab_hit;
 #if FC_VARIANT_BIG && !defined(FC_SERIAL_PROFILE)
         F.dbg[2] = tk[OP_CHROMA]; F.dbg[3] = tk[OP_PRED_SETUP]; F.dbg[4] = tk[OP_PRED_FINISH];
         F.dbg[5] = tk[OP_NORMS]; F.dbg[6] = tk[OP_MC_SEARCH];
diff --git a/fiasco_amd/csrc/hip/mp_device.inc b/fiasco_amd/csrc/hip/mp_device.inc
--- a/fiasco_amd/csrc/hip/mp_device.inc
+++ b/fiasco_amd/csrc/hip/mp_device.inc
@@ -300,14 +300,13 @@
 #endif
     }
 }
-#else
+#elif FC_VARIANT_BIG
 __device__ __noinline__ void mp_tables(const DevFrame &F, Sh &sh, int level, int y)
 {
     const int tid = threadIdx.x;
     const int ctx = level - sh.par.lc_min_opt, dcs = sh.par.dcs, sy = sh.par.sy;
     const int om = 64 + sy + 12 <= 128 ? 64 + sy : 128;
-    const int sl = (om + 12 <= 128 && B > 128) ? 128 : om + 11;
-    if (tid == sl) {
+    if (tid == om + 11) {
         const Pool &m = sh.pool;
         float q0 = 0, q1;
         if (m.d0_n && y != 0) q0 += sh.m0tab[qac_shift(m.d0_index)];
@@ -316,23 +315,6 @@
         if (y == 0) { q1 -= sh.m0tab[qac_shift(m.d0_yindex)]; q1 += (float) qac_shift(m.d0_yindex); }
         else        { q1 -= sh.m0tab[qac_shift(m.d0_index)];  q1 += (float) qac_shift(m.d0_index); }
         sh.Q0 = q0; sh.Q1 = q1;
-#if !FC_VARIANT_BIG
-        if (!sh.band) {
-            MPState &mp = sh.mp;
-            const unsigned N = (unsigned) sh.pool.n;
-            mp.s1_last[0] = 1;
-            const unsigned mv = N - 2u;
-            if (mv != 0) {
-                const unsigned kk = 31u - (unsigned) __clz((int) (mv + 1));
-                const unsigned r = (mv + 1) - (1u << kk);
-                mp.s1_cd = 1u; mp.s1_k[0] = (int) kk; mp.s1_thr[0] = (int) (mv + 1 - 2 * r);
-            } else {
-                mp.s1_cd = 0u; mp.s1_k[0] = 0; mp.s1_thr[0] = 0;
-            }
-            mp.s1_has = 0u;
-            mp.np = 0;
-        }
-#endif
     }
     if (tid < om + 12) {
         int ci = 0, ti = 0, role = 0;
@@ -343,40 +325,165 @@
             role = 1; ci = dcs + ctx * sy - 1; ti = ctx + 1;
         }
         else if (r >= 0 && r < MAXED + 1) { role = 2; ci = r; }
-#if !FC_VARIANT_BIG
-        else if (r == 7 || r == 8) role = 3;
-        else if (r == 9 && !sh.band) {
-            role = 1; ci = dcs + ctx * sy + sh.par.half_nd; ti = ctx + 1;
-        } else if (r == 10 && !sh.band) {
-            role = 1; ci = sh.par.half_dc; ti = 0;
-        }
-#endif
         float num = 1.0f, den = 1.0f;
         if (role == 1)      { num = (float) sh.cb.cnt[ci]; den = (float) sh.cb.tot[ti]; }
         else if (role == 2) { num = (float) sh.pool.count[ci]; den = (float) sh.pool.total; }
-#if !FC_VARIANT_BIG
-        else if (role == 3) {
-            const unsigned *counts = sh.tm;
-            num = (float) counts[level]; den = (float) counts[sh.par.ML + level];
-        }
-#endif
         float p = num / den;
-#if !FC_VARIANT_BIG
-        if (r == 7) p = 1 - p;
-#endif
         const double lg = log2((double) p);
         if (role == 1) {
             if (tid < dcs) sh.lgdc[tid] = lg;
             else if (r == 6) sh.lglv_m1 = lg;
-#if !FC_VARIANT_BIG
-            else if (r == 9) sh.mp.wb_nd = sub_log2(sh, 0.0f, lg, ci, ti);
-            else if (r == 10) sh.mp.wb_dc = sub_log2(sh, 0.0f, lg, ci, ti);
-#endif
             else sh.lglv[tid - 64] = lg;
         } else if (role == 2) sh.Ltab[ci] = (float) -lg;
-#if !FC_VARIANT_BIG
-        else if (role == 3) sh.tb[r - 7] = (float) -lg;
-#endif
+    }
+}
+#else
+
+__device__ __forceinline__ void mp_call_setup(Sh &sh, int y, int slot)
+{
+    const Pool &m = sh.pool;
+    float q0 = 0, q1;
+    if (m.d0_n && y != 0) q0 += sh.m0tab[qac_shift(m.d0_index)];
+    if (y >= 0) q0 += sh.m0tab[qac_shift(m.d0_yindex)];
+    q1 = q0;
+    if (y == 0) { q1 -= sh.m0tab[qac_shift(m.d0_yindex)]; q1 += (float) qac_shift(m.d0_yindex); }
+    else        { q1 -= sh.m0tab[qac_shift(m.d0_index)];  q1 += (float) qac_shift(m.d0_index); }
+    sh.Q0 = q0; sh.Q1 = q1;
+    sh.tab_slot = slot; sh.tab_off = slot * sh.par.sy;
+    if (!sh.band) {
+        MPState &mp = sh.mp;
+        const unsigned N = (unsigned) sh.pool.n;
+        mp.s1_last[0] = 1;
+        const unsigned mv = N - 2u;
+        if (mv != 0) {
+            const unsigned kk = 31u - (unsigned) __clz((int) (mv + 1));
+            const unsigned r = (mv + 1) - (1u << kk);
+            mp.s1_cd = 1u; mp.s1_k[0] = (int) kk; mp.s1_thr[0] = (int) (mv + 1 - 2 * r);
+        } else {
+            mp.s1_cd = 0u; mp.s1_k[0] = 0; mp.s1_thr[0] = 0;
+        }
+        mp.s1_has = 0u;
+        mp.np = 0;
+    }
+}
+
+__device__ int mp_tab_levels(const DevFrame &F)
+{
+    const int nc = F.lc_max - F.lc_min + 1;
+    if (nc < 1 || nc > FC_TAB_CTX || nc * F.sy > FC_TAB_LV || F.coeff_nt > 14) return 0;
+    if (64 + nc * F.sy + MAXED + 1 + 4 * nc + 1 + 1 > B) return 0;
+    return nc;
+}
+
+__device__ __forceinline__ bool mp_tables_hit(const Sh &sh, int level, int ctx)
+{
+    if (!sh.tab_nctx || sh.band || sh.tag.cb != CB_GEN(sh)) return false;
+    bool same = sh.tag.tm[ctx][0] == sh.tm[level] && sh.tag.tm[ctx][1] == sh.tm[sh.par.ML + level];
+#pragma unroll
+    for (int i = 0; i <= MAXED; i++) same = same && sh.tag.pool[i] == sh.pool.count[i];
+    return same && sh.tag.pool[MAXED + 1] == (short) sh.pool.total;
+}
+
+template <bool CHECK>
+__device__ __noinline__ void mp_tables(const DevFrame &F, Sh &sh, int level, int y)
+{
+    const int tid = threadIdx.x;
+    const int ctx = level - sh.par.lc_min_opt, dcs = sh.par.dcs, sy = sh.par.sy;
+    const bool all = sh.tab_nctx != 0 && !sh.band;
+    const int nc = all ? sh.tab_nctx : 1, c0 = all ? 0 : ctx;
+    const int cur = ctx - c0;
+    const int om = 64 + nc * sy, end = om + MAXED + 1 + 4 * nc + 1;
+    const int sl = ((end + 63) & ~63) < B ? ((end + 63) & ~63) : end;
+    if (tid == sl && !CHECK) mp_call_setup(sh, y, cur);
+    unsigned tag0 = 0, tag1 = 0;
+    int kind = 0, slot = 0, ci = 0;
+    if (tid < end) {
+        int ti = 0;
+        const int r = tid - om;
+        if (tid < dcs) { kind = 1; ci = tid; }
+        else if (tid >= 64 && tid < om) {
+            int t = tid - 64;
+#pragma unroll
+            for (int k = 1; k < FC_TAB_CTX; k++) if (k < nc && t >= sy) { t -= sy; slot++; }
+            kind = 2; ci = dcs + (c0 + slot) * sy + t; ti = c0 + slot + 1;
+        }
+        else if (r >= 0 && r < MAXED + 1) { kind = 3; ci = r; }
+        else if (r >= MAXED + 1 && r < MAXED + 1 + nc) {
+            kind = 4; slot = r - (MAXED + 1); ci = dcs + (c0 + slot) * sy - 1; ti = c0 + slot + 1;
+        }
+        else if (r >= MAXED + 1 + nc && r < MAXED + 1 + 3 * nc) {
+            const int u = r - (MAXED + 1 + nc);
+            slot = u >> 1; kind = 5 + (u & 1);
+        }
+        else if (r >= MAXED + 1 + 3 * nc && !sh.band) {
+            const int u = r - (MAXED + 1 + 3 * nc);
+            if (u < nc) { kind = 7; slot = u; ci = dcs + (c0 + slot) * sy + sh.par.half_nd; ti = c0 + slot + 1; }
+            else { kind = 8; ci = sh.par.half_dc; }
+        }
+        float num = 1.0f, den = 1.0f;
+        if (kind == 3) {
+            const short cn = sh.pool.count[ci], ct = (short) sh.pool.total;
+            num = (float) cn; den = (float) sh.pool.total;
+            tag0 = (unsigned short) cn; tag1 = (unsigned short) ct;
+        } else if (kind == 5 || kind == 6) {
+            const int lv = sh.par.lc_min_opt + c0 + slot;
+            tag0 = sh.tm[lv]; tag1 = sh.tm[sh.par.ML + lv];
+            num = (float) tag0; den = (float) tag1;
+        } else if (kind) { num = (float) sh.cb.cnt[ci]; den = (float) sh.cb.tot[ti]; }
+        if (kind == 1 && tid == 0) tag0 = CB_GEN(sh);
+        float p = num / den;
+        if (kind == 5) p = 1 - p;
+        const double lg = log2((double) p);
+        const float nlg = (float) -lg;
+        const float wbv = (kind == 7 || kind == 8) ? sub_log2(sh, 0.0f, lg, ci, ti) : 0.0f;
+        if (CHECK) {
+#if FC_TABCHECK
+            bool bad = false;
+            if (kind == 1) bad = __double_as_longlong(sh.lgdc[tid]) != __double_as_longlong(lg);
+            else if (kind == 2) bad = __double_as_longlong(sh.lglv[tid - 64]) != __double_as_longlong(lg);
+            else if (kind == 3) bad = __float_as_uint(sh.Ltab[ci]) != __float_as_uint(nlg);
+            else if (kind == 4) bad = __double_as_longlong(sh.lglv_m1[slot]) != __double_as_longlong(lg);
+            else if (kind == 5 || kind == 6) {
+                if (slot == cur) bad = __float_as_uint(sh.tb[slot][kind - 5]) != __float_as_uint(nlg)
+                                       || __float_as_uint(sh.tbc[kind - 5]) != __float_as_uint(nlg);
+            }
+            else if (kind == 7) bad = __float_as_uint(sh.wb_nd[slot]) != __float_as_uint(wbv)
+                                      || (slot == cur && __float_as_uint(sh.mp.wb_nd) != __float_as_uint(wbv));
+            else if (kind == 8) bad = __float_as_uint(sh.wb_dc) != __float_as_uint(wbv)
+                                      || __float_as_uint(sh.mp.wb_dc) != __float_as_uint(wbv);
+            if (bad) sh.failed = FC_ERR_TABCHECK;
+#endif
+        } else {
+            if (kind == 1) sh.lgdc[tid] = lg;
+            else if (kind == 2) sh.lglv[tid - 64] = lg;
+            else if (kind == 3) sh.Ltab[ci] = nlg;
+            else if (kind == 4) sh.lglv_m1[slot] = lg;
+            else if (kind == 5 || kind == 6) {
+                sh.tb[slot][kind - 5] = nlg;
+                if (slot == cur) sh.tbc[kind - 5] = nlg;
+            }
+            else if (kind == 7) { sh.wb_nd[slot] = wbv; if (slot == cur) sh.mp.wb_nd = wbv; }
+            else if (kind == 8) { sh.wb_dc = wbv; sh.mp.wb_dc = wbv; }
+        }
+    }
+    __syncthreads();
+    if (!CHECK && all) {
+        if (kind == 3) { sh.tag.pool[ci] = (short) tag0; if (ci == 0) sh.tag.pool[MAXED + 1] = (short) tag1; }
+        else if (kind == 5) { sh.tag.tm[slot][0] = tag0; sh.tag.tm[slot][1] = tag1; }
+        else if (kind == 1 && tid == 0) sh.tag.cb = tag0;
+    }
+    if (!CHECK && !all && tid == 0) sh.tag.cb = 0;
+}
+
+__device__ __forceinline__ void mp_tables_reuse(Sh &sh, int ctx, int y)
+{
+    const int nc = sh.tab_nctx;
+    const int end = 64 + nc * sh.par.sy + MAXED + 1 + 4 * nc + 1;
+    const int sl = ((end + 63) & ~63) < B ? ((end + 63) & ~63) : end;
+    if ((int) threadIdx.x == sl) {
+        mp_call_setup(sh, y, ctx);
+        sh.tbc[0] = sh.tb[ctx][0]; sh.tbc[1] = sh.tb[ctx][1];
+        sh.mp.wb_nd = sh.wb_nd[ctx]; sh.mp.wb_dc = sh.wb_dc;
     }
 }
 
@@ -558,6 +665,9 @@
             sh.cb.tot[0]++;
         }
     }
+#if FC_TABREUSE
+    if (sh.tab_nctx) CB_GEN(sh) = ++sh.gen_ctr;
+#endif
 }
 
 __device__ __forceinline__ float wave_min_l63(float v)
@@ -746,7 +856,7 @@
                     if (pass) {
                         float i0 = n > 0 ? F.ipdo[d] : 0.0f, i1 = n > 1 ? F.ipdo[(size_t) P + d] : 0.0f;
                         float i2 = n > 2 ? F.ipdo[(size_t) 2 * P + d] : 0.0f, i3 = n > 3 ? F.ipdo[(size_t) 3 * P + d] : 0.0f;
-                        full_eval<MAXED - 1>(F, sh, mp, sh.lglv, n, F.pos[d], d, F.num[d], F.den[d], i0, i1, i2, i3, ev);
+                        full_eval<MAXED - 1>(F, sh, mp, MP_LGLV(sh), n, F.pos[d], d, F.num[d], F.den[d], i0, i1, i2, i3, ev);
                     }
                     evals += (unsigned) __popcll(__ballot(pass));
                     blockevals++;
@@ -789,7 +899,7 @@
                         if (k < n) mp.sel_ipdo[n][k] = F.ipdo[(size_t) k * P + b_state];
                     mp.row_state = b_state;
                     mp.n = n + 1;
-                    if (mp.n < F.max_elements) mp_step_prepare(F, sh, mp, sh.lglv, sh.lglv_m1);
+                    if (mp.n < F.max_elements) mp_step_prepare(F, sh, mp, MP_LGLV(sh), MP_LGLV_M1(sh));
                 }
                 mp.index = index;
             }
@@ -893,7 +1003,7 @@
 #if FC_GM
                         ev.qc = GM_QAC(sh.gm.pk[0]) && c < (int) sh.pool.n ? (int) GQ_CUR(sh, 0)[c] : 0;
 #endif
-                        full_eval<MAXED - 1>(F, sh, mp, sh.lglv, n, c, list[c], F.num[c], F.den[c], i0, i1, i2, i3, ev);
+                        full_eval<MAXED - 1>(F, sh, mp, MP_LGLV(sh), n, c, list[c], F.num[c], F.den[c], i0, i1, i2, i3, ev);
                     }
                     evals += (unsigned) __popcll(__ballot(pass));
                     blockevals++;
@@ -940,7 +1050,7 @@
                         if (k < n) mp.sel_ipdo[n][k] = F.ipdo[(size_t) k * P + index];
                     mp.row_state = b_state;
                     mp.n = n + 1;
-                    if (mp.n < F.max_elements) mp_step_prepare(F, sh, mp, sh.lglv, sh.lglv_m1);
+                    if (mp.n < F.max_elements) mp_step_prepare(F, sh, mp, MP_LGLV(sh), MP_LGLV_M1(sh));
                 }
                 mp.index = index;
             }
@@ -979,8 +1089,19 @@
 #define APX_MARK(i) do { } while (0)
 #endif
     if (fr.coop) snap_coop_before(sh, fr, sh.sp, sh.par.ML);
+#if FC_TABREUSE
+    const bool tab_hit = uni((int) mp_tables_hit(sh, level, level - sh.par.lc_min_opt)) != 0;
+    if (tab_hit) {
+        mp_tables_reuse(sh, level - sh.par.lc_min_opt, y);
+        __syncthreads();
+#if FC_TABCHECK
+        mp_tables<true>(F, sh, level, y);
+#endif
+    } else mp_tables<false>(F, sh, level, y);
+#else
     mp_tables(F, sh, level, y);
     __syncthreads();
+#endif
     APX_MARK(0);
     const int S = sh.states;
     const bool regscan = !sh.band && S <= KREG * B && sh.par.max_elements <= FC_NIP + 1;
@@ -1043,8 +1164,8 @@
         mp.ab = fr.lrange.tree_bits + fr.lrange.mv_tree_bits + fr.lrange.mv_coord_bits + fr.lrange.nd_tree_bits
                 + fr.lrange.nd_weights_bits;
 #else
-        fr.lrange.tree_bits = sh.tb[0];
-        mp.ab = sh.tb[0];
+        fr.lrange.tree_bits = sh.tbc[0];
+        mp.ab = sh.tbc[0];
 #endif
         mp.price = fr.price;
         mp.err = mp.norm;
@@ -1056,9 +1177,9 @@
         mp.costs = (mp.matrix_bits + mp.weights_bits + mp.ab) * mp.price + mp.err;
         mp.index = -1;
 #if FC_VARIANT_BIG
-        mp_step_prepare(F, sh, mp, sh.lglv, sh.lglv_m1);
+        mp_step_prepare(F, sh, mp, MP_LGLV(sh), MP_LGLV_M1(sh));
 #else
-        if (sh.band) mp_step_prepare(F, sh, mp, sh.lglv, sh.lglv_m1);
+        if (sh.band) mp_step_prepare(F, sh, mp, MP_LGLV(sh), MP_LGLV_M1(sh));
         else {
             const float L0 = sh.Ltab[0], L1 = sh.Ltab[1], q0 = sh.Q0, q1 = sh.Q1;
             float b = L1; b += q0; mp.s1_pre[0] = b;
@@ -1200,6 +1321,7 @@
     else if (tid == 64) {
         sh.cnt.bytes_mp += 4ull * D * (2 + mp.n) + 4ull * (1u << level);
         sh.cnt.n_mp++; sh.cnt.n_steps += mp.n;
+        if (tab_hit) sh.cnt.n_tab_hit++; else sh.cnt.n_tab_build++;
     }
 #endif
     if (fr.coop) {
diff --git a/fiasco_amd/csrc/hip/mp_reg.inc b/fiasco_amd/csrc/hip/mp_reg.inc
--- a/fiasco_amd/csrc/hip/mp_reg.inc
+++ b/fiasco_amd/csrc/hip/mp_reg.inc
@@ -235,7 +235,7 @@
                 for (int k = 0; k < MAXED; k++) ev.f[k] = 0;
                 const float i0 = ipk[0], i1 = NIP > 1 ? ipk[1 % NIP] : 0.0f;
                 const float i2 = NIP > 2 ? ipk[2 % NIP] : 0.0f, i3 = NIP > 3 ? ipk[3 % NIP] : 0.0f;
-                if (pass) full_eval<NIP>(F, sh, mp, sh.lglv, n, psk, state, numk, denk, i0, i1, i2, i3, ev);
+                if (pass) full_eval<NIP>(F, sh, mp, MP_LGLV(sh), n, psk, state, numk, denk, i0, i1, i2, i3, ev);
                 unsigned npass = (unsigned) __popcll(__ballot(pass));
                 int last = -1, win = -1;
                 for (;;) {
@@ -281,7 +281,7 @@
                 for (int k = 0; k < MAXED - 1; k++) if (k < n) mp.sel_ipdo[n][k] = rb.ip[k];
                 mp.row_state = bstate;
                 mp.n = n + 1;
-                if (mp.n < sh.par.max_elements) mp_step_prepare(F, sh, mp, sh.lglv, sh.lglv_m1);
+                if (mp.n < sh.par.max_elements) mp_step_prepare(F, sh, mp, MP_LGLV(sh), MP_LGLV_M1(sh));
             }
             mp.index = index;
         }
@@ -348,7 +348,7 @@
 #pragma unroll
             for (int k = 0; k < MAXED; k++) ev.f[k] = 0;
             if (pass)
-                full_eval<NIP>(F, sh, mp, sh.lglv, n, tid, st, num, den, ip[0], NIP > 1 ? ip[1 % NIP] : 0.0f,
+                full_eval<NIP>(F, sh, mp, MP_LGLV(sh), n, tid, st, num, den, ip[0], NIP > 1 ? ip[1 % NIP] : 0.0f,
                           NIP > 2 ? ip[2 % NIP] : 0.0f, NIP > 3 ? ip[3 % NIP] : 0.0f, ev);
             evals += (unsigned) __popcll(__ballot(pass));
             int last = -1, win = -1;
@@ -391,7 +391,7 @@
                 for (int k = 0; k < MAXED - 1; k++) if (k < n) mp.sel_ipdo[n][k] = rb.ip[k];
                 mp.row_state = bstate;
                 mp.n = n + 1;
-                if (mp.n < sh.par.max_elements) mp_step_prepare(F, sh, mp, sh.lglv, sh.lglv_m1);
+                if (mp.n < sh.par.max_elements) mp_step_prepare(F, sh, mp, MP_LGLV(sh), MP_LGLV_M1(sh));
             }
             mp.index = index;
         }
diff --git a/include/libfiasco_amd_hip.h b/include/libfiasco_amd_hip.h
--- a/include/libfiasco_amd_hip.h
+++ b/include/libfiasco_amd_hip.h
@@ -24,6 +24,7 @@
     unsigned long long decoder_frames, decoder_bytes, decoder_us;
     unsigned long long coop_frames, coop_workgroups;
     unsigned long long spec_app_rows, spec_app_wait;
+    unsigned long long tab_builds, tab_hits;
 } fiasco_amd_stats;
 
 void fiasco_amd_get_stats(fiasco_amd_stats *out);
```
